# ZijiaLewisLu/CVPR2025-DeCafNet

Hardware: AMD Instinct MI355X
Metric: clips/sec (grounding fwd, T=16384 D=1024) (higher is better)
Workload: dtype f32; 1 GPU; BASELINE configs[2]: T=16384 D=1024 full multi-scale pyramid + sidekick top-k 30% + expert path, NQ=1 queries/video, 24 independent videos per step: 3 forwards in flight on 3 HIP streams x 8 videos per forward, one replica of this per GPU; T=16384, vid_len=16384, D=1024, E=256, TE=256, levels=8, win=9, heads=4, fusion_layers=2, sn=60, msf=True, norm=True, Lq=32, nq=1, max_batch=8, forwards_in_flight=3

## Files before the change

### cvpr2025-decafnet_amd/_lib.py

```python
import ctypes
import os

_HERE = os.path.dirname(os.path.abspath(__file__))
SO_PATH = os.environ.get('DCF_LIB_PATH') or os.path.join(_HERE, 'libdecafnet_hip.so')
_LIB = None

c_f32p = ctypes.c_void_p
c_u8p = ctypes.c_void_p
c_i32p = ctypes.c_void_p
c_i64p = ctypes.c_void_p
i32, i64, f32, f64 = ctypes.c_int32, ctypes.c_int64, ctypes.c_float, ctypes.c_double
vp = ctypes.c_void_p


class DcfConfig(ctypes.Structure):
    _fields_ = [(n, i32) for n in ('D', 'E', 'TE', 'vid_heads', 'fusion_heads', 'fusion_layers', 'n_embd_convs',
                                   'n_stem', 'n_levels', 'win', 'head_layers', 'sn')] + \
               [('sratio', f32)] + [(n, i32) for n in ('msf', 'norm', 'use_abs_pe', 'max_batch', 'gemm_mode', 'model_kind', 'second_fusion',
                                                      'text_in', 'text_layers', 'text_heads', 'text_abs_pe', 'text_bkgd',
                                                      'scat', 'sfonly', 'text_kind', 'xattn_affine', 'vid_stride', 'pool_only', 'attn_mode')]


SIGNATURES = {
    'dcf_last_error': (ctypes.c_char_p, []),
    'dcf_abi_version': (i32, []),
    'dcf_model_create': (i32, [ctypes.POINTER(DcfConfig), ctypes.POINTER(vp)]),
    'dcf_model_destroy': (None, [vp]),
    'dcf_model_bind': (i32, [vp, ctypes.c_char_p, c_f32p, ctypes.POINTER(i64), i32]),
    'dcf_model_set_pe': (i32, [vp, c_f32p, i64]),
    'dcf_model_set_text_pe': (i32, [vp, c_f32p, i64]),
    'dcf_text_encode': (i32, [vp, c_f32p, c_u8p, i32, c_f32p, c_u8p, vp]),
    'dcf_model_finalize': (i32, [vp, vp]),
    'dcf_numerics_status': (i32, [vp, i32, vp]),
    'dcf_numerics_status_async': (i32, [vp, vp, vp]),
    'dcf_points_per_query': (i64, [vp, i64]),
    'dcf_forward_eval': (i32, [vp, c_f32p, c_f32p, c_u8p, i64, i32, ctypes.POINTER(vp), ctypes.POINTER(vp),
                               ctypes.POINTER(i32), c_f32p, c_f32p, c_f32p, c_u8p, vp]),
    'dcf_forward_eval_videos': (i32, [vp, i32, ctypes.POINTER(vp), ctypes.POINTER(vp), ctypes.POINTER(vp), i64, ctypes.POINTER(i32),
                                      ctypes.POINTER(vp), ctypes.POINTER(vp), ctypes.POINTER(i32), ctypes.POINTER(vp),
                                      c_f32p, c_f32p, c_u8p, vp]),
    'dcf_forward_train_videos': (i32, [vp, i32, ctypes.POINTER(vp), ctypes.POINTER(vp), ctypes.POINTER(vp), i64, ctypes.POINTER(i32),
                                       ctypes.POINTER(vp), ctypes.POINTER(vp), ctypes.POINTER(i32), ctypes.POINTER(vp),
                                       c_f32p, c_f32p, c_f32p, c_u8p, vp]),
    'dcf_model_set_dropout': (i32, [vp, f32, f32, f32, f32, f32, i64]),
    'dcf_debug_dropout_keep': (i32, [i64, i32, i64, i64, f32, c_u8p, vp]),
    'dcf_sigmoid_focal_loss': (i32, [c_f32p, c_f32p, c_u8p, i64, f32, f32, i32, c_f32p, c_f32p, c_i32p, vp]),
    'dcf_ctr_iou_loss': (i32, [c_f32p, c_f32p, c_u8p, i64, i32, f32, c_f32p, c_f32p, c_i32p, vp]),
    'dcf_annotate_points': (i32, [c_f32p, i32, i64, i32, f64, f64, i32, i64, i32, f64, c_u8p, c_f32p, c_u8p, c_u8p, vp]),
    'dcf_point_objective': (i32, [c_f32p, c_f32p, c_f32p, c_u8p, c_f32p, i32, i64, i32, f64, f64, i32, i64, i32, f64, f32, f64, i32, f32,
                                  c_f32p, f32, f32, c_f32p, c_f32p, vp]),
    'dcf_sigmoid_focal_loss_grad': (i32, [c_f32p, c_f32p, c_u8p, i64, f32, f32, i32, c_f32p, c_f32p, c_i32p, c_f32p, vp]),
    'dcf_ctr_iou_loss_grad': (i32, [c_f32p, c_f32p, c_u8p, i64, i32, f32, c_f32p, c_f32p, c_i32p, c_f32p, vp]),
    'dcf_point_objective_grad': (i32, [c_f32p, c_f32p, c_f32p, c_u8p, c_f32p, i32, i64, i32, f64, f64, i32, i64, i32, f64, f32, f64, i32, f32,
                                       c_f32p, f32, f32, c_f32p, c_f32p, c_f32p, c_f32p, c_f32p, i32, c_f32p, c_f32p, vp]),
    'dcf_forward_eval_gated': (i32, [vp, c_f32p, c_f32p, c_u8p, i64, i32, ctypes.POINTER(vp), ctypes.POINTER(vp),
                                     ctypes.POINTER(i32), c_f32p, c_f32p, c_f32p, c_u8p, vp]),
    'dcf_hybrid_phase1': (i32, [vp, i32, c_f32p, c_f32p, c_u8p, i64, i64, i32, ctypes.POINTER(vp), ctypes.POINTER(vp), ctypes.POINTER(i32),
                                c_f32p, c_f32p, vp]),
    'dcf_hybrid_phase2': (i32, [vp, c_f32p, c_u8p, i64, c_f32p, vp]),
    'dcf_hybrid_phase3': (i32, [vp, c_f32p, c_f32p, c_f32p, c_u8p, c_f32p, c_f32p, c_u8p, vp]),
    'dcf_debug_copy': (i32, [vp, i32, c_f32p, i64, vp]),
    'dcf_graph_active': (i32, [vp]),
    'dcf_debug_set_option': (i32, [ctypes.c_char_p, i32]),
    'dcf_calib_mfma_rate': (i32, [i32, i32, ctypes.POINTER(i32), ctypes.POINTER(f32)]),
    'dcf_model_set_graph_mode': (i32, [vp, i32]),
    'dcf_model_set_ln_carry': (i32, [vp, i32]),
    'dcf_profile_enable': (i32, [i32]),
    'dcf_profile_report': (i64, [ctypes.c_char_p, i64]),
    'dcf_collect_segments': (i32, [c_f32p, c_f32p, c_u8p, i32, i64, i32, f32, i32, f32, c_f32p, c_f32p, c_i32p, vp]),
    'dcf_collect_segments_ext': (i32, [c_f32p, c_f32p, c_u8p, c_f32p, i32, i64, i32, f32, i32, f32, c_f32p, c_f32p, c_i32p, vp]),
    'dcf_nms_1d': (i32, [c_f32p, c_f32p, c_i32p, i32, i32, i32, f32, c_i64p, c_i32p, vp]),
    'dcf_softnms_1d': (i32, [c_f32p, c_f32p, c_i32p, i32, i32, i32, f32, f32, f32, i32, i32, c_f32p, c_i64p, c_i32p, vp]),
    'dcf_segment_voting': (i32, [c_f32p, i32, c_i32p, i32, i32, c_f32p, c_f32p, c_i32p, i32, i32, f32, i32, c_f32p, vp]),
    'dcf_op_linear': (i32, [c_f32p, c_f32p, c_f32p, c_f32p, i32, i32, i32, i32, vp]),
    'dcf_op_linear_split': (i32, [c_f32p, c_f32p, c_f32p, c_f32p, i32, i32, i32, i32, i32, vp]),
    'dcf_op_linear_cm': (i32, [c_f32p, c_f32p, c_f32p, c_f32p, i32, i32, i32, vp]),
    'dcf_op_linear_ln': (i32, [c_f32p, c_f32p, c_f32p, c_f32p, c_f32p, c_f32p, c_f32p, i32, i32, i32, i32, i32, vp]),
    'dcf_op_linear_ln_carry': (i32, [c_f32p, c_f32p, c_f32p, c_f32p, c_f32p, c_f32p, c_f32p, c_f32p, c_f32p, c_f32p, i32, i32, i32, i32, i32, i32, vp]),
    'dcf_op_ffn': (i32, [c_f32p, c_f32p, c_f32p, c_f32p, c_f32p, c_f32p, c_f32p, c_f32p, c_u8p, c_f32p, c_f32p, i32, i32, i32, vp]),
    'dcf_op_linear_cm_split': (i32, [c_f32p, c_f32p, c_f32p, c_f32p, i32, i32, i32, i32, vp]),
    'dcf_op_head': (i32, [c_f32p, c_u8p, c_f32p, c_f32p, c_f32p, c_f32p, c_f32p, c_f32p, c_f32p, c_f32p, c_f32p, i32, i32, i32, i32, f32, i32, vp]),
    'dcf_op_conv3': (i32, [c_f32p, c_u8p, c_f32p, c_f32p, i32, i32, i32, i32, vp]),
    'dcf_op_conv3_split': (i32, [c_f32p, c_u8p, c_f32p, c_f32p, i32, i32, i32, i32, i32, vp]),
    'dcf_op_layernorm': (i32, [c_f32p, c_f32p, c_f32p, c_f32p, i32, i32, i32, vp]),
    'dcf_op_xattn': (i32, [c_f32p, c_f32p, c_f32p, c_u8p, c_f32p, i32, i32, i32, i32, i32, vp]),
    'dcf_op_local_attn': (i32, [c_f32p, c_f32p, c_f32p, c_u8p, c_f32p, i32, i32, i32, i32, i32, vp]),
    'dcf_op_sidekick': (i32, [c_f32p, c_f32p, c_f32p, i32, i32, i32, i32, vp]),
    'dcf_op_gate': (i32, [c_f32p, c_u8p, c_f32p, c_u8p, i32, i32, i32, f64, i32, vp]),
    'dcf_op_encoder': (i32, [vp, ctypes.c_char_p, c_f32p, c_u8p, i32, i32, i32, c_f32p, c_u8p, vp]),
    'dcf_op_enc_pre': (i32, [vp, ctypes.c_char_p, c_f32p, c_u8p, i32, i32, i32, c_f32p, c_f32p, c_f32p, c_f32p, vp]),
    'dcf_op_decoder': (i32, [vp, ctypes.c_char_p, c_f32p, c_u8p, i32, i32, ctypes.POINTER(vp), ctypes.POINTER(vp), ctypes.POINTER(i32), vp]),
    'dcf_op_tcn': (i32, [vp, ctypes.c_char_p, c_f32p, c_u8p, i32, i32, i32, i32, c_f32p, vp]),
}


def lib():
    global _LIB
    if _LIB is None:
        import torch
        if not os.path.exists(SO_PATH):
            raise RuntimeError(f'{SO_PATH} is missing: build it with __graft_entry__.build() '
                               f'(there is no CPU fallback for the grounding path)')
        h = ctypes.CDLL(SO_PATH, mode=ctypes.RTLD_GLOBAL)
        for name, (res, args) in SIGNATURES.items():
            fn = getattr(h, name)
            fn.restype = res
            fn.argtypes = args
        _LIB = h
    return _LIB


def check(rc, what=''):
    if rc != 0:
        msg = lib().dcf_last_error().decode(errors='replace')
        raise RuntimeError(f'decafnet_hip {what} failed: {msg}')


def ptr(t):
    return None if t is None else ctypes.c_void_p(t.data_ptr())


def current_stream():
    import torch
    return ctypes.c_void_p(torch.cuda.current_stream().cuda_stream)
```

### cvpr2025-decafnet_amd/csrc/dec_chain.h

```cpp
#pragma once
#include <hip/hip_runtime.h>
#include <stdint.h>

namespace dcf {

struct DecChainArgs {
  const float* X;
  int64_t ldx;
  const uint8_t* mask;
  const float* ln_q_w; const float* ln_q_b;
  const float* dw;
  const float* qn_w; const float* qn_b;
  const unsigned short* Wq;
  const float* bq;
  const unsigned short* KV;
  const float* kmask;
  const unsigned short* Wp;
  const float* bp;
  float* Q3;
  int64_t ldq;
  float* stats_out;
  int stats_w;
  int B, T;
  int affine;
  int lk2;
  unsigned* status;
  int attn_single;
};

bool dec_chain_supports(int E, int heads, int Lk);
int launch_dec_chain(const DecChainArgs& a, hipStream_t stream);

size_t chain1_image_halfs(int N, int K);
int launch_split_chain1(const float* W, unsigned short* img, int N, int K, hipStream_t stream, unsigned* overflow = nullptr);

size_t kv_image_halfs(int lk2);
int launch_kv_image(const float* K, const float* V, const uint8_t* kvmask, int B, int Lk, int lk2, unsigned short* img, float* kmask,
                    hipStream_t stream);

}
```

### cvpr2025-decafnet_amd/csrc/dec_chain.hip

```cpp
#include "dec_chain.h"

#include <type_traits>

#include "chain_common.h"
#include "common.h"

namespace dcf {

namespace {

using namespace chain;

constexpr int DE = 256, DHEADS = 4, DHD = 64;
constexpr int STAGE = 65536;
constexpr int WGROWS = 128;
constexpr int P_LNW = 0, P_LNB = 256, P_QNW = 512, P_QNB = 768, P_DW = 1024, P_BQ = 1792, P_BP = 2048, P_MS = 2560, P_END = 2624;
constexpr int X_LAST = P_END;
constexpr int X_FIRST = X_LAST + 5 * 256;
constexpr int LDS_FLOATS = X_FIRST + 5 * 256;
constexpr int LDS_BYTES = 2 * STAGE + LDS_FLOATS * (int)sizeof(float);
#ifdef DCF_DC_STAMP
__device__ unsigned long long dcf_dc_stamps[16];
#endif
}

__global__ void k_split_chain1(const float* __restrict__ W, unsigned short* __restrict__ img, int N, int K, unsigned* __restrict__ overflow) {
  const int i = blockIdx.x * blockDim.x + threadIdx.x;
  if (i >= N * (K / 2)) return;
  const int n = i / (K / 2), k = (i - n * (K / 2)) * 2;
  const float w0 = W[(size_t)n * K + k], w1 = W[(size_t)n * K + k + 1];
  unsigned hi, lo;
  split2_f16(w0, w1, SW, hi, lo);
  if (!(__builtin_fabsf(w0) * SW <= 65504.f) || !(__builtin_fabsf(w1) * SW <= 65504.f)) {
    if (overflow) atomicOr(overflow, 1u);
  }
  const int n32 = n >> 5, rr = n & 31, kk = k >> 4, kr = k & 15;
  const int a = kr >> 3, h = (kr >> 2) & 1, ii = kr & 3, j = 4 * a + ii;
  const size_t o = ((size_t)(n32 * (K / 16) + kk) * 2) * 512 + (size_t)(h * 32 + rr) * 8 + j;
  *reinterpret_cast<unsigned*>(img + o) = hi;
  *reinterpret_cast<unsigned*>(img + o + 512) = lo;
}

__global__ void k_kv_image(const float* __restrict__ K, const float* __restrict__ V, const uint8_t* __restrict__ kvmask, int B, int Lk,
                           int lk2, unsigned short* __restrict__ img, float* __restrict__ kmask) {
  const int per_head = 16 * lk2 * 256;
  const int i = blockIdx.x * blockDim.x + threadIdx.x;
  if (i < B * 64) {
    const int b = i / 64, key = i % 64;
    kmask[i] = (key < Lk && kvmask[(size_t)b * Lk + key]) ? 0.f : -INFINITY;
  }
  if (i >= B * DHEADS * per_head) return;
  const int b = i / (DHEADS * per_head), rem = i - b * (DHEADS * per_head);
  const int hd = rem / per_head, rem2 = rem - hd * per_head;
  const int piece = rem2 >> 8, lane = (rem2 >> 2) & 63, jp = rem2 & 3;
  const int h = lane >> 5, r = lane & 31, plane = piece & 1, j = 2 * jp;
  const float scale = 1.0f / sqrtf(sqrtf((float)DHD));
  float v0 = 0.f, v1 = 0.f;
  if (piece < 8 * lk2) {
    const int ks = (piece >> 1) & 3, kt = piece >> 3;
    const int key = 32 * kt + r, ch = DHD * hd + 16 * ks + 8 * (j >> 2) + 4 * h + (j & 3);
    if (key < Lk) { v0 = K[((size_t)b * Lk + key) * DE + ch] * scale; v1 = K[((size_t)b * Lk + key) * DE + ch + 1] * scale; }
  } else {
    const int pv = piece - 8 * lk2;
    const int q = (pv >> 1) & 1, kt = (pv >> 2) % lk2, ct = (pv >> 2) / lk2;
    const int ch = DHD * hd + 32 * ct + r, key = 32 * kt + 16 * q + 8 * (j >> 2) + 4 * h + (j & 3);
    if (key < Lk) v0 = V[((size_t)b * Lk + key) * DE + ch];
    if (key + 1 < Lk) v1 = V[((size_t)b * Lk + key + 1) * DE + ch];
  }
  const f16x2 hh = __builtin_convertvector(f32x2{v0, v1}, f16x2);
  const f16x2 ll = __builtin_convertvector(f32x2{v0 - (float)hh[0], v1 - (float)hh[1]}, f16x2);
  const size_t o = (((size_t)b * DHEADS + hd) * 16 * lk2 + piece) * 512 + (size_t)lane * 8 + j;
  *reinterpret_cast<unsigned*>(img + o) = __builtin_bit_cast(unsigned, plane == 0 ? hh : ll);
}

template <int LK2, bool SINGLE = false>
__global__ __launch_bounds__(256, 1) void k_dec_chain(DecChainArgs p) {
  extern __shared__ __attribute__((aligned(16))) unsigned char lds[];
  float* ldf = reinterpret_cast<float*>(lds + 2 * STAGE);
  const int tid = threadIdx.x, lane = tid & 63, r = lane & 31, h = lane >> 5;
  const int w = __builtin_amdgcn_readfirstlane(tid >> 6);
  const unsigned lane16 = (unsigned)lane * 16u;
  const int wins = (p.T + WGROWS - 1) / WGROWS;
  const int b = (int)blockIdx.x / wins, t0 = ((int)blockIdx.x - b * wins) * WGROWS;
  const int t = t0 + w * 32 + r;
  const bool inseq = t < p.T;
  const int64_t row = (int64_t)b * p.T + (inseq ? t : p.T - 1);
  constexpr int KVP = 16 * LK2;

  const unsigned short* kv_b = p.KV + (size_t)b * DHEADS * KVP * 512;
  auto issue_piece = [&](int s, int i) __attribute__((always_inline)) {
    const bool kv = s < 8 && (s & 1);
    const int np = kv ? KVP : 64;
    int pc = w + 4 * i;
    pc = pc < np ? pc : np - 1;
    const unsigned short* src = s >= 8 ? p.Wp + (size_t)(s - 8) * 64 * 512 : (kv ? kv_b + (size_t)(s >> 1) * KVP * 512 : p.Wq + (size_t)(s >> 1) * 64 * 512);
    glds16(src + (size_t)pc * 512, lane16, (unsigned)(s & 1) * STAGE + (unsigned)pc * 1024u);
  };
#ifdef DCF_DC_STAMP
  unsigned long long acc_[16] = {0, 0, 0, 0, 0, 0, 0, 0, 0, 0, 0, 0, 0, 0, 0, 0}, last_ = dc_stamp();
#endif

  const float* px = p.X + row * p.ldx + 4 * h;
  const bool valid = inseq && p.mask[row] != 0;
  f32x4 xv[32];
#pragma unroll
  for (int i = 0; i < 32; ++i) xv[i] = *reinterpret_cast<const f32x4*>(px + 32 * (i >> 2) + 8 * (i & 3));
  const int te = w == 0 ? t0 - 1 : t0 + WGROWS;
  const bool edge_wave = w == 0 || w == 3;
  const bool evalid = edge_wave && te >= 0 && te < p.T && p.mask[(int64_t)b * p.T + (te >= 0 && te < p.T ? te : 0)] != 0;
  f32x4 ev = f32x4{0.f, 0.f, 0.f, 0.f};
  if (evalid) ev = *reinterpret_cast<const f32x4*>(p.X + ((int64_t)b * p.T + te) * p.ldx + 4 * lane);
#pragma unroll
  for (int i = 0; i < 16; ++i) issue_piece(0, i);

  {
    ldf[P_LNW + tid] = p.ln_q_w[tid]; ldf[P_LNB + tid] = p.ln_q_b[tid];
    ldf[P_QNW + tid] = p.qn_w[tid]; ldf[P_QNB + tid] = p.qn_b[tid];
    ldf[P_DW + tid] = p.dw[tid]; ldf[P_DW + 256 + tid] = p.dw[256 + tid]; ldf[P_DW + 512 + tid] = p.dw[512 + tid];
    ldf[P_BQ + tid] = p.bq[tid];
    ldf[P_BP + tid] = p.bp[tid]; ldf[P_BP + 256 + tid] = p.bp[256 + tid];
    if (tid < 64) ldf[P_MS + tid] = p.kmask[(size_t)b * 64 + tid];
  }


  if (!valid) {
#pragma unroll
    for (int i = 0; i < 32; ++i) xv[i] = f32x4{0.f, 0.f, 0.f, 0.f};
  }
  float mean1, rstd1;
  row_stats<DE>(xv, mean1, rstd1);
  STAMP(0);
  __syncthreads();
#pragma unroll
  for (int i = 0; i < 32; ++i) {
    const int c = 32 * (i >> 2) + 8 * (i & 3) + 4 * h;
    const f32x4 g = *reinterpret_cast<const f32x4*>(ldf + P_LNW + c), bb = *reinterpret_cast<const f32x4*>(ldf + P_LNB + c);
    f32x4 y = (xv[i] - mean1) * rstd1 * g + bb;
    if (!valid) y = f32x4{0.f, 0.f, 0.f, 0.f};
    xv[i] = y;
  }
  if (r == 31) {
#pragma unroll
    for (int i = 0; i < 32; ++i) *reinterpret_cast<f32x4*>(ldf + X_LAST + (w + 1) * 256 + 32 * (i >> 2) + 8 * (i & 3) + 4 * h) = xv[i];
  }
  if (r == 0) {
#pragma unroll
    for (int i = 0; i < 32; ++i) *reinterpret_cast<f32x4*>(ldf + X_FIRST + w * 256 + 32 * (i >> 2) + 8 * (i & 3) + 4 * h) = xv[i];
  }
  if (edge_wave) {
    f32x4 y = f32x4{0.f, 0.f, 0.f, 0.f};
    const float s = wave_sum((ev.x + ev.y) + (ev.z + ev.w));
    const float mean = s * (1.0f / DE);
    const f32x4 d = ev - mean;
    const float var = wave_sum((d.x * d.x + d.y * d.y) + (d.z * d.z + d.w * d.w)) * (1.0f / DE);
    const float rs = 1.0f / sqrtf(var + 1e-5f);
    if (evalid) y = d * rs * *reinterpret_cast<const f32x4*>(ldf + P_LNW + 4 * lane) + *reinterpret_cast<const f32x4*>(ldf + P_LNB + 4 * lane);
    *reinterpret_cast<f32x4*>(ldf + (w == 0 ? X_LAST : X_FIRST + 4 * 256) + 4 * lane) = y;
  }
  STAMP(1);
  __syncthreads();
  STAMP(2);
  {
    const bool is32 = lane == 32, is31 = lane == 31;
#pragma unroll
    for (int i = 0; i < 32; ++i) {
      const int c = 32 * (i >> 2) + 8 * (i & 3) + 4 * h;
      const f32x4 lastv = *reinterpret_cast<const f32x4*>(ldf + X_LAST + w * 256 + c);
      const f32x4 firstv = *reinterpret_cast<const f32x4*>(ldf + X_FIRST + (w + 1) * 256 + c);
      const f32x4 w0 = *reinterpret_cast<const f32x4*>(ldf + P_DW + c), w1 = *reinterpret_cast<const f32x4*>(ldf + P_DW + 256 + c),
                  w2 = *reinterpret_cast<const f32x4*>(ldf + P_DW + 512 + c);
      f32x4 pv, nv;
#pragma unroll
      for (int e = 0; e < 4; ++e) {
        const float sp = shr1(xv[i][e], lastv[e]), sn = shl1(xv[i][e], firstv[e]);
        pv[e] = is32 ? lastv[e] : sp;
        nv[e] = is31 ? firstv[e] : sn;
      }
      xv[i] = w0 * pv + w1 * xv[i] + w2 * nv;
    }
  }
  f16x8 qh[16], ql[16];
  {
    float mean2, rstd2;
    row_stats<DE>(xv, mean2, rstd2);
#pragma unroll
    for (int kk = 0; kk < 16; ++kk) {
      float v8[8];
#pragma unroll
      for (int u = 0; u < 2; ++u) {
        const int i = 2 * kk + u, c = 32 * (i >> 2) + 8 * (i & 3) + 4 * h;
        const f32x4 g = *reinterpret_cast<const f32x4*>(ldf + P_QNW + c), bb = *reinterpret_cast<const f32x4*>(ldf + P_QNB + c);
        const f32x4 y = (xv[i] - mean2) * rstd2 * g + bb;
        v8[4 * u] = y.x; v8[4 * u + 1] = y.y; v8[4 * u + 2] = y.z; v8[4 * u + 3] = y.w;
      }
      split8(v8, SA, qh[kk], ql[kk]);
    }
  }

  STAMP(3);
  f16x8 cth[16], ctl[16];
  const float qscale = 1.0f / sqrtf(sqrtf((float)DHD));
  auto stage_begin = [&](int s) __attribute__((always_inline)) {
    asm volatile("s_waitcnt vmcnt(0)" ::: "memory");
    STAMP(4);
    __syncthreads();
    STAMP(5);
  };
  auto gemm2 = [&](const unsigned char* buf, const f16x8 (&bh)[16], const f16x8 (&bl)[16], f32x16 (&acc)[2], auto&& dma, auto&& side)
                   __attribute__((always_inline)) {
    f16x8 fr[2][4];
    auto frags = [&](int kk, int set) __attribute__((always_inline)) {
      fr[set][0] = *reinterpret_cast<const f16x8*>(buf + ((0 * 16 + kk) * 2) * 1024);
      fr[set][1] = *reinterpret_cast<const f16x8*>(buf + ((0 * 16 + kk) * 2 + 1) * 1024);
      fr[set][2] = *reinterpret_cast<const f16x8*>(buf + ((1 * 16 + kk) * 2) * 1024);
      fr[set][3] = *reinterpret_cast<const f16x8*>(buf + ((1 * 16 + kk) * 2 + 1) * 1024);
    };
    frags(0, 0);
#pragma unroll
    for (int kk = 0; kk < 16; ++kk) {
      const int set = kk & 1;
      if (kk + 1 < 16) frags(kk + 1, set ^ 1);
      acc[0] = mma(fr[set][1], bh[kk], acc[0]);
      acc[1] = mma(fr[set][3], bh[kk], acc[1]);
      __builtin_amdgcn_sched_barrier(0);
      side(kk, 0);
      __builtin_amdgcn_sched_barrier(0);
      acc[0] = mma(fr[set][0], bl[kk], acc[0]);
      acc[1] = mma(fr[set][2], bl[kk], acc[1]);
      __builtin_amdgcn_sched_barrier(0);
      side(kk, 1);
      dma(kk);
      __builtin_amdgcn_sched_barrier(0);
      acc[0] = mma(fr[set][0], bh[kk], acc[0]);
      acc[1] = mma(fr[set][2], bh[kk], acc[1]);
      __builtin_amdgcn_sched_barrier(0);
    }
  };
  f32x16 O[2];
  u32x4 cx_h, cx_l;
  auto ctx_piece = [&](int hd, int u) __attribute__((always_inline)) {
    const int ct = u >> 3, q = (u >> 2) & 1, i = u & 3;
    unsigned hi, lo;
    split2_f16(O[ct][8 * q + 2 * i], O[ct][8 * q + 2 * i + 1], SA, hi, lo);
    cx_h[i] = hi; cx_l[i] = lo;
    if (i == 3) {
      cth[2 * (2 * hd + ct) + q] = __builtin_bit_cast(f16x8, cx_h);
      ctl[2 * (2 * hd + ct) + q] = __builtin_bit_cast(f16x8, cx_l);
    }
  };
#pragma unroll
  for (int hd = 0; hd < DHEADS; ++hd) {
    f32x16 QA[2];
    {
      stage_begin(2 * hd);
      const unsigned char* buf = lds + ((2 * hd) & 1) * STAGE + lane16;
#pragma unroll
      for (int t2 = 0; t2 < 2; ++t2)
#pragma unroll
        for (int e = 0; e < 16; ++e) QA[t2][e] = 0.f;
      gemm2(buf, qh, ql, QA,
            [&](int kk) __attribute__((always_inline)) {
              if (kk < KVP / 4) issue_piece(2 * hd + 1, kk);
            },
            [&](int kk, int slot) __attribute__((always_inline)) { if (hd > 0 && slot == 0) ctx_piece(hd - 1, kk); });
    }
    STAMP(6);
    f16x8 sh_[4], sl_[4];
#pragma unroll
    for (int t2 = 0; t2 < 2; ++t2)
#pragma unroll
      for (int q = 0; q < 2; ++q) {
        float v8[8];
#pragma unroll
        for (int u = 0; u < 2; ++u) {
          const int g = 2 * q + u;
          const f32x4 bq = *reinterpret_cast<const f32x4*>(ldf + P_BQ + DHD * hd + 32 * t2 + 8 * g + 4 * h);
#pragma unroll
          for (int e = 0; e < 4; ++e) v8[4 * u + e] = __builtin_fmaf(QA[t2][4 * g + e], UNSCALE, bq[e]) * qscale;
        }
        split8(v8, 1.f, sh_[2 * t2 + q], sl_[2 * t2 + q]);
      }
    STAMP(7);
    {
      stage_begin(2 * hd + 1);
      const unsigned char* buf = lds + ((2 * hd + 1) & 1) * STAGE + lane16;
      f32x16 S[LK2];
#pragma unroll
      for (int kt = 0; kt < LK2; ++kt)
#pragma unroll
        for (int e = 0; e < 16; ++e) S[kt][e] = 0.f;
      f16x8 kf[2][LK2][2];
      auto kfrags = [&](int ks, int set) __attribute__((always_inline)) {
#pragma unroll
        for (int kt = 0; kt < LK2; ++kt) {
          kf[set][kt][0] = *reinterpret_cast<const f16x8*>(buf + ((kt * 4 + ks) * 2) * 1024);
          kf[set][kt][1] = *reinterpret_cast<const f16x8*>(buf + ((kt * 4 + ks) * 2 + 1) * 1024);
        }
      };
      kfrags(0, 0);
#pragma unroll
      for (int ks = 0; ks < 4; ++ks) {
        const int set = ks & 1;
        if (ks + 1 < 4) kfrags(ks + 1, set ^ 1);
        issue_piece(2 * hd + 2, 2 * ks);
        issue_piece(2 * hd + 2, 2 * ks + 1);
        if constexpr (!SINGLE) {
#pragma unroll
          for (int kt = 0; kt < LK2; ++kt) S[kt] = mma(kf[set][kt][0], sl_[ks], S[kt]);
#pragma unroll
          for (int kt = 0; kt < LK2; ++kt) S[kt] = mma(kf[set][kt][1], sh_[ks], S[kt]);
        }
#pragma unroll
        for (int kt = 0; kt < LK2; ++kt) S[kt] = mma(kf[set][kt][0], sh_[ks], S[kt]);
        __builtin_amdgcn_sched_barrier(0);
      }
      STAMP(8);
      f16x8 vf[2][2][2];
      auto vfrags = [&](int st_, int set) __attribute__((always_inline)) {
#pragma unroll
        for (int ct = 0; ct < 2; ++ct) {
          const int pc = 8 * LK2 + ((ct * LK2 + (st_ >> 1)) * 2 + (st_ & 1)) * 2;
          vf[set][ct][0] = *reinterpret_cast<const f16x8*>(buf + pc * 1024);
          vf[set][ct][1] = *reinterpret_cast<const f16x8*>(buf + (pc + 1) * 1024);
        }
      };
      vfrags(0, 0);
      float mx = -INFINITY;
#pragma unroll
      for (int kt = 0; kt < LK2; ++kt)
#pragma unroll
        for (int g = 0; g < 4; ++g) {
          const f32x4 mk = *reinterpret_cast<const f32x4*>(ldf + P_MS + 32 * kt + 8 * g + 4 * h);
#pragma unroll
          for (int e = 0; e < 4; ++e) { S[kt][4 * g + e] += mk[e]; mx = fmaxf(mx, S[kt][4 * g + e]); }
        }
      mx = xor32_max(mx);
      float sum = 0.f;
#pragma unroll
      for (int kt = 0; kt < LK2; ++kt)
#pragma unroll
        for (int e = 0; e < 16; ++e) { S[kt][e] = fast_exp(S[kt][e] - mx); sum += S[kt][e]; }
      const float inv = 1.0f / xor32_sum(sum);
      f16x8 ph[LK2][2], pl[LK2][2];
#pragma unroll
      for (int kt = 0; kt < LK2; ++kt)
#pragma unroll
        for (int q = 0; q < 2; ++q) {
          float v8[8];
#pragma unroll
          for (int e = 0; e < 8; ++e) v8[e] = S[kt][8 * q + e] * inv;
          split8(v8, 1.f, ph[kt][q], pl[kt][q]);
        }
      STAMP(9);
#pragma unroll
      for (int ct = 0; ct < 2; ++ct)
#pragma unroll
        for (int e = 0; e < 16; ++e) O[ct][e] = 0.f;
#pragma unroll
      for (int st_ = 0; st_ < 2 * LK2; ++st_) {
        const int set = st_ & 1, kt = st_ >> 1, q = st_ & 1;
        if (st_ + 1 < 2 * LK2) vfrags(st_ + 1, set ^ 1);
#pragma unroll
        for (int i = 0; i < 8 / (2 * LK2); ++i) issue_piece(2 * hd + 2, 8 + st_ * (8 / (2 * LK2)) + i);
        if constexpr (!SINGLE) {
#pragma unroll
          for (int ct = 0; ct < 2; ++ct) O[ct] = mma(vf[set][ct][0], pl[kt][q], O[ct]);
#pragma unroll
          for (int ct = 0; ct < 2; ++ct) O[ct] = mma(vf[set][ct][1], ph[kt][q], O[ct]);
        }
#pragma unroll
        for (int ct = 0; ct < 2; ++ct) O[ct] = mma(vf[set][ct][0], ph[kt][q], O[ct]);
        __builtin_amdgcn_sched_barrier(0);
      }
      STAMP(10);
    }
  }

  float ps = 0.f, pss = 0.f;
  float* qout = p.Q3 + row * p.ldq + 4 * h;
  f32x16 A2[2][2];
  f32x4 xr[2][4];
  auto load_xr = [&](int j) __attribute__((always_inline)) {
#pragma unroll
    for (int g = 0; g < 4; ++g) xr[j & 1][g] = *reinterpret_cast<const f32x4*>(px + 32 * j + 8 * g);
  };
  f32x4 ep_sc, ep_sf;
  auto epilogue = [&](int j, int g, int half) __attribute__((always_inline)) {
    if (half == 0) {
      const f32x4 bs = *reinterpret_cast<const f32x4*>(ldf + P_BP + 64 * j + 8 * g + 4 * h);
      const f32x4 bh = *reinterpret_cast<const f32x4*>(ldf + P_BP + 64 * j + 32 + 8 * g + 4 * h);
#pragma unroll
      for (int e = 0; e < 4; ++e) {
        ep_sc[e] = __builtin_fmaf(A2[j & 1][0][4 * g + e], UNSCALE, bs[e]);
        ep_sf[e] = __builtin_fmaf(A2[j & 1][1][4 * g + e], UNSCALE, bh[e]);
      }
    } else {
      f32x4 xa = valid ? xr[j & 1][g] : f32x4{0.f, 0.f, 0.f, 0.f};
      if (!p.affine) xa = (xa - mean1) * rstd1;
      const f32x4 o = xa * ep_sc + ep_sf;
      if (inseq) *reinterpret_cast<f32x4*>(qout + 32 * j + 8 * g) = o;
      ps += (o.x + o.y) + (o.z + o.w);
      pss += __builtin_fmaf(o.x, o.x, o.y * o.y) + __builtin_fmaf(o.z, o.z, o.w * o.w);
    }
  };
#pragma unroll
  for (int j = 0; j < 8; ++j) {
    stage_begin(8 + j);
    const unsigned char* buf = lds + (j & 1) * STAGE + lane16;
    if (j > 0) asm volatile("" : "+v"(xr[(j - 1) & 1][0]), "+v"(xr[(j - 1) & 1][1]), "+v"(xr[(j - 1) & 1][2]), "+v"(xr[(j - 1) & 1][3]));
    load_xr(j);
#pragma unroll
    for (int t2 = 0; t2 < 2; ++t2)
#pragma unroll
      for (int e = 0; e < 16; ++e) A2[j & 1][t2][e] = 0.f;
    if (j == 0) {
      gemm2(buf, cth, ctl, A2[0],
            [&](int kk) __attribute__((always_inline)) {
              issue_piece(9, kk);
            },
            [&](int kk, int slot) __attribute__((always_inline)) { if (kk < 8) ctx_piece(DHEADS - 1, 2 * kk + slot); });
    } else {
      gemm2(buf, cth, ctl, A2[j & 1],
            [&](int kk) __attribute__((always_inline)) {
              if (j + 1 < 8) issue_piece(8 + j + 1, kk);
            },
            [&](int kk, int slot) __attribute__((always_inline)) { if ((kk & 3) == 0) epilogue(j - 1, kk >> 2, slot); });
    }
    STAMP(11);
  }
  asm volatile("s_waitcnt vmcnt(0)" ::: "memory");
  asm volatile("" : "+v"(xr[1][0]), "+v"(xr[1][1]), "+v"(xr[1][2]), "+v"(xr[1][3]));
#pragma unroll
  for (int g = 0; g < 4; ++g) { epilogue(7, g, 0); epilogue(7, g, 1); }
  STAMP(12);
  const float s1 = xor32_sum(ps), s2 = xor32_sum(pss);
  if (p.stats_out && inseq && h == 0) {
    const int slots = DE / p.stats_w;
    float* o = p.stats_out + row * slots * 2;
    o[0] = s1; o[1] = s2;
    for (int k = 1; k < slots; ++k) { o[2 * k] = 0.f; o[2 * k + 1] = 0.f; }
  }
  const bool bad = !(__builtin_fabsf(s1) <= 3.4028234664e38f) && inseq;
  if (bad && p.status) {
    bool anykey = false;
#pragma unroll
    for (int k = 0; k < 64; ++k) anykey = anykey || ldf[P_MS + k] == 0.f;
    if (anykey) atomicOr(p.status, 1u);
  }
#ifdef DCF_DC_STAMP
  STAMP(13);
  if (blockIdx.x == 1 && tid == 0)
    for (int i = 0; i < 16; ++i) dcf_dc_stamps[i] = acc_[i];
#endif
}

#ifdef DCF_DC_STAMP
}
extern "C" int dcf_debug_dc_stamps(unsigned long long* out) {
  return hipMemcpyFromSymbol(out, HIP_SYMBOL(dcf::dcf_dc_stamps), 16 * sizeof(unsigned long long)) == hipSuccess ? 0 : -1;
}
namespace dcf {
#endif

bool dec_chain_supports(int E, int heads, int Lk) { return E == DE && heads == DHEADS && Lk >= 1 && Lk <= 64; }

size_t chain1_image_halfs(int N, int K) { return (size_t)N * K * 2; }

int launch_split_chain1(const float* W, unsigned short* img, int N, int K, hipStream_t stream, unsigned* overflow) {
  DCF_CHECK(N % 32 == 0 && K % 16 == 0, "launch_split_chain1: N = %d, K = %d", N, K);
  const int n = N * (K / 2);
  hipLaunchKernelGGL(k_split_chain1, dim3((n + 255) / 256), dim3(256), 0, stream, W, img, N, K, overflow);
  DCF_HIP(hipGetLastError());
  return 0;
}

size_t kv_image_halfs(int lk2) { return (size_t)DHEADS * 16 * lk2 * 512; }

int launch_kv_image(const float* K, const float* V, const uint8_t* kvmask, int B, int Lk, int lk2, unsigned short* img, float* kmask,
                    hipStream_t stream) {
  DCF_CHECK(B > 0 && Lk >= 1 && Lk <= 32 * lk2 && (lk2 == 1 || lk2 == 2), "launch_kv_image: Lk = %d, lk2 = %d", Lk, lk2);
  const int n = B * DHEADS * 16 * lk2 * 256;
  hipLaunchKernelGGL(k_kv_image, dim3((n + 255) / 256), dim3(256), 0, stream, K, V, kvmask, B, Lk, lk2, img, kmask);
  DCF_HIP(hipGetLastError());
  return 0;
}

int launch_dec_chain(const DecChainArgs& a, hipStream_t stream) {
  DCF_CHECK(a.B > 0 && a.T > 0 && a.X && a.mask && a.Wq && a.KV && a.kmask && a.Wp && a.Q3, "launch_dec_chain: null argument");
  DCF_CHECK(a.lk2 == 1 || a.lk2 == 2, "launch_dec_chain: lk2 = %d", a.lk2);
  DCF_CHECK(!a.stats_out || (a.stats_w > 0 && DE % a.stats_w == 0), "launch_dec_chain: stats_out needs a slot width dividing %d", DE);
  auto al16 = [](const void* q) { return (reinterpret_cast<uintptr_t>(q) & 15) == 0; };
  DCF_CHECK(al16(a.X) && al16(a.Q3) && al16(a.Wq) && al16(a.Wp) && al16(a.KV) && a.ldx % 4 == 0 && a.ldq % 4 == 0,
            "launch_dec_chain: operands must be 16-byte aligned with row pitches that are multiples of 4");
  static bool attr_set[64] = {};
  int dev = 0;
  DCF_HIP(hipGetDevice(&dev));
  if (dev >= 0 && dev < 64 && !attr_set[dev]) {
    DCF_HIP(hipFuncSetAttribute(reinterpret_cast<const void*>(&k_dec_chain<1>), hipFuncAttributeMaxDynamicSharedMemorySize, LDS_BYTES));
    DCF_HIP(hipFuncSetAttribute(reinterpret_cast<const void*>(&k_dec_chain<2>), hipFuncAttributeMaxDynamicSharedMemorySize, LDS_BYTES));
    DCF_HIP(hipFuncSetAttribute(reinterpret_cast<const void*>(&k_dec_chain<1, true>), hipFuncAttributeMaxDynamicSharedMemorySize, LDS_BYTES));
    DCF_HIP(hipFuncSetAttribute(reinterpret_cast<const void*>(&k_dec_chain<2, true>), hipFuncAttributeMaxDynamicSharedMemorySize, LDS_BYTES));
    attr_set[dev] = true;
  }
  const unsigned grid = (unsigned)(a.B * ((a.T + WGROWS - 1) / WGROWS));
  if (a.attn_single) {
    if (a.lk2 == 1) hipLaunchKernelGGL((k_dec_chain<1, true>), dim3(grid), dim3(256), LDS_BYTES, stream, a);
    else hipLaunchKernelGGL((k_dec_chain<2, true>), dim3(grid), dim3(256), LDS_BYTES, stream, a);
  } else if (a.lk2 == 1) hipLaunchKernelGGL(k_dec_chain<1>, dim3(grid), dim3(256), LDS_BYTES, stream, a);
  else hipLaunchKernelGGL(k_dec_chain<2>, dim3(grid), dim3(256), LDS_BYTES, stream, a);
  DCF_HIP(hipGetLastError());
  return 0;
}

}
```

### cvpr2025-decafnet_amd/csrc/engine.hip

```cpp
#include <cstdarg>
#include <cstdio>
#include <cstdlib>
#include <algorithm>
#include <cstring>
#include <string>
#include <atomic>
#include <mutex>
#include <unordered_map>
#include <vector>

#include "../../include/decafnet_hip.h"
#include "attn.h"
#include "common.h"
#include "dec_chain.h"
#include "dropout.h"
#include "enc_chain.h"
#include "ffn_chain.h"
#include "gemm.h"
#include "head_chain.h"
#include "heads.h"
#include "postproc.h"
#include "rowops.h"
#include "score.h"

namespace dcf {

static thread_local std::string g_err;
void set_error(const char* fmt, ...) {
  char buf[1024];
  va_list ap;
  va_start(ap, fmt);
  vsnprintf(buf, sizeof(buf), fmt, ap);
  va_end(ap);
  g_err = buf;
}

static std::unordered_map<std::string, int>& debug_options() {
  static std::unordered_map<std::string, int> o;
  return o;
}
static std::mutex& debug_options_mutex() {
  static std::mutex mu;
  return mu;
}
static std::atomic<int> g_option_epoch{0};
static int debug_option(const char* name, int dflt) {
  std::lock_guard<std::mutex> lock(debug_options_mutex());
  auto& o = debug_options();
  auto it = o.find(name);
  return it == o.end() ? dflt : it->second;
}

struct ProfRec { std::string name; hipEvent_t a, b; double flops, bytes; };
static bool g_prof_on = false;
static std::vector<ProfRec> g_recs;

ProfScope::ProfScope(const char* name, hipStream_t s, double flops, double bytes) : idx(-1), st(s) {
  if (!g_prof_on) return;
  ProfRec r{name, nullptr, nullptr, flops, bytes};
  if (hipEventCreate(&r.a) != hipSuccess || hipEventCreate(&r.b) != hipSuccess) return;
  (void)hipEventRecord(r.a, st);
  g_recs.push_back(r);
  idx = (int)g_recs.size() - 1;
}
ProfScope::~ProfScope() {
  if (idx >= 0) (void)hipEventRecord(g_recs[idx].b, st);
}

__global__ void k_permute3(const float* __restrict__ src, float* __restrict__ dst, int d0, int d1, int d2, int p0, int p1,
                           int p2) {
  const int n = d0 * d1 * d2;
  const int i = blockIdx.x * blockDim.x + threadIdx.x;
  if (i >= n) return;
  int idx[3];
  idx[0] = i / (d1 * d2);
  idx[1] = (i / d2) % d1;
  idx[2] = i % d2;
  const int dims[3] = {d0, d1, d2};
  const int perm[3] = {p0, p1, p2};
  const int o = (idx[perm[0]] * dims[perm[1]] + idx[perm[1]]) * dims[perm[2]] + idx[perm[2]];
  dst[o] = src[i];
}

__global__ void k_masks_out(const uint8_t* __restrict__ mask_all, uint8_t* __restrict__ out, const LevelTable* lt,
                            const unsigned* __restrict__ status, float* __restrict__ logits) {
  const int r = blockIdx.x * blockDim.x + threadIdx.x;
  const int total = lt->start[lt->n_levels];
  if (r >= total) return;
  int l = 0;
  while (l + 1 < lt->n_levels && r >= lt->start[l + 1]) ++l;
  const int rel = r - lt->start[l];
  const int b = rel / lt->T[l], t = rel - b * lt->T[l];
  const int64_t o = (int64_t)b * lt->S + lt->off[l] + t;
  out[o] = mask_all[r];
  if (status && (status[0] & 3u)) logits[o] = __uint_as_float(0x7fc00000u);
}

__global__ void k_points_out(const float* __restrict__ rows, float* __restrict__ out, const LevelTable* lt) {
  const int r = blockIdx.x * blockDim.x + threadIdx.x;
  const int total = lt->start[lt->n_levels];
  if (r >= total) return;
  int l = 0;
  while (l + 1 < lt->n_levels && r >= lt->start[l + 1]) ++l;
  const int rel = r - lt->start[l];
  const int b = rel / lt->T[l], t = rel - b * lt->T[l];
  out[(int64_t)b * lt->S + lt->off[l] + t] = rows[r];
}

__global__ void k_apply_gate(const float* __restrict__ gate_in, const uint8_t* __restrict__ vid_mask, float* __restrict__ gate,
                             uint8_t* __restrict__ mask_out, int T, int rows, int msf) {
  const int r = blockIdx.x * blockDim.x + threadIdx.x;
  if (r >= rows) return;
  const int t = r % T;
  const float g = gate_in[r];
  const bool m = vid_mask[t] != 0;
  gate[r] = g;
  mask_out[r] = msf ? m : (m && g != 0.f);
}

__global__ __launch_bounds__(64) void k_fold_ln(const float* __restrict__ W, const float* __restrict__ bias, const float* __restrict__ g,
                                                const float* __restrict__ beta, float* __restrict__ Wf, float* __restrict__ s,
                                                float* __restrict__ c, int K) {
  const int n = blockIdx.x, lane = threadIdx.x;
  float a1 = 0.f, a2 = 0.f;
  for (int k = lane; k < K; k += 64) {
    const float w = W[(int64_t)n * K + k];
    const float wf = w * g[k];
    Wf[(int64_t)n * K + k] = wf;
    a1 += wf;
    a2 += beta[k] * w;
  }
  a1 = wave_sum(a1);
  a2 = wave_sum(a2);
  if (lane == 0) { s[n] = a1; c[n] = (bias ? bias[n] : 0.f) + a2; }
}

struct Bound {
  const float* p = nullptr;
  std::vector<int64_t> shape;
  int64_t numel() const {
    int64_t n = 1;
    for (auto s : shape) n *= s;
    return n;
  }
};

struct EncW {
  const float *ln_attn_w, *ln_attn_b, *dw_q, *dw_k, *dw_v, *qn_w, *qn_b, *kn_w, *kn_b, *vn_w, *vn_b;
  const float *wq, *bq, *wk, *bk, *wv, *bv, *wp, *bp, *ls_attn;
  const float *ln_ffn_w, *ln_ffn_b, *fc_w, *fc_b, *pj_w, *pj_b, *ls_ffn;
  const float *fc_wf, *fc_s, *fc_c;
  const unsigned short* qkv_chain[3];
  const float *qkv_s[3], *qkv_c[3];
  const unsigned short* wp_chain;
};
struct DecW {
  const float *ln_q_w, *ln_q_b, *ln_kv_w, *ln_kv_b, *dw, *qn_w, *qn_b;
  const float *wq, *bq, *wk, *bk, *wv, *bv, *wp, *bp;
  const float *wp_il, *bp_il;
  const float *ln_ffn_w, *ln_ffn_b, *fc_w, *fc_b, *pj_w, *pj_b, *ls_ffn;
  const float *fc_wf, *fc_s, *fc_c;
  const unsigned short *wq_chain, *wp_chain;
};
struct TextEncW {
  const float *ln_attn_w, *ln_attn_b, *wq, *bq, *wk, *bk, *wv, *bv, *wp, *bp, *ls_attn;
  const float *ln_ffn_w, *ln_ffn_b, *fc_w, *fc_b, *pj_w, *pj_b, *ls_ffn;
};
struct HeadW {
  std::vector<const float*> conv;
  std::vector<const float*> ln_w, ln_b;
  const float* out_w;
  const float* out_b;
  const unsigned short* chain[2] = {nullptr, nullptr};
};

static inline int vid_stride_of(const dcf_config& c) { return c.vid_stride > 1 ? c.vid_stride : 1; }

struct Plan {
  int T0 = 0, B = 0, L = 0;
  LevelTable lt{};
  LevelTable* d_lt = nullptr;
};

}

using namespace dcf;

namespace dcf { struct HybridState; }
using dcf::HybridState;

struct dcf_model {
  dcf_config cfg{};
  std::unordered_map<std::string, Bound> bound;
  std::vector<float*> owned;
  std::unordered_map<const float*, const unsigned short*> wsplit;
  std::unordered_map<const float*, int64_t> wsplit_ldw;
  std::unordered_map<const float*, int> wsplit_terms;
  int gemm_terms = 16;
  bool force_x6 = false;
  bool no_ln_carry = false;
  int option_epoch = 0;
  unsigned* status = nullptr;
  bool finalized = false;
  const float* pe = nullptr;
  int64_t pe_T = 0;

  const float *vid_map_w = nullptr, *vid_map_b = nullptr;
  const float *vid_w1 = nullptr, *vid_w2 = nullptr, *vid_w3 = nullptr;
  int64_t vid_ldw = 0;
  std::vector<DecW> dec;
  const float *fus_out_w = nullptr, *fus_out_b = nullptr;
  const float *embd_fc_w = nullptr, *embd_fc_b = nullptr;
  const float *embd_fc_wf = nullptr, *embd_fc_s = nullptr, *embd_fc_c = nullptr;
  std::vector<const float*> embd_conv, embd_ln_w, embd_ln_b;
  std::vector<EncW> stem, branch;
  std::vector<const float*> pool_w;
  HeadW cls1, cls2, reg;
  std::vector<float> reg_scales;
  const float *tcn_in_w = nullptr, *tcn_in_b = nullptr, *tcn_out_w = nullptr, *tcn_out_b = nullptr;
  std::vector<const float*> tcn_wd, tcn_bd, tcn_wp, tcn_bp, tcn_lnw, tcn_lnb;
  std::vector<const unsigned short*> tcn_frag;
  const float *text_embd_w = nullptr, *text_embd_b = nullptr, *text_bkgd = nullptr;
  TextEncW text_pool{};
  std::vector<TextEncW> text_enc;
  const float* text_pe = nullptr;
  int64_t text_pe_L = 0;
  char* text_ws = nullptr;
  size_t text_ws_bytes = 0;

  char* arena = nullptr;
  size_t arena_bytes = 0;
  std::vector<Plan> plans;
  std::vector<uint64_t> last_key, graph_key;
  hipGraph_t graph = nullptr;
  hipGraphExec_t graph_exec = nullptr;
  bool capturing = false;
  int graph_mode = 0;
  std::vector<uint64_t> nocapture_key;
  int last_launch = 0;
  hipStream_t own = nullptr;
  hipEvent_t ev_in = nullptr, ev_out = nullptr;
  struct {
    float *correl = nullptr, *gate = nullptr, *vidmap = nullptr, *fused = nullptr, *F = nullptr;
    int nq = 0, T0 = 0, B = 0, S = 0;
  } dbg;
  struct HybridState* hyb = nullptr;
  int hyb_levels = 0;
  size_t hyb_extra = 0;
  char* hyb_extra_ptr = nullptr;
  float* hyb_feat_out = nullptr;
  float* dbg_vidmap = nullptr;
  float* dbg_fused = nullptr;
  int64_t dbg_cap = 0;
  bool keep_debug = false;
  struct DropState {
    float p[5] = {0.f, 0.f, 0.f, 0.f, 0.f};
    float scale[5] = {1.f, 1.f, 1.f, 1.f, 1.f};
    uint64_t seed = 0;
    bool active = false;
    int b0 = 0;
  } drop_state;
  DropState* drop = nullptr;
};

namespace dcf {

static void free_hybrid(dcf_model* m);

static void drop_graph(dcf_model* m, bool keep_last_key = false) {
  if (m->graph_exec) (void)hipGraphExecDestroy(m->graph_exec);
  if (m->graph) (void)hipGraphDestroy(m->graph);
  m->graph_exec = nullptr;
  m->graph = nullptr;
  m->graph_key.clear();
  if (!keep_last_key) m->last_key.clear();
}

static int free_model(dcf_model* m) {
  drop_graph(m);
  if (m->status) (void)hipFree(m->status);
  m->status = nullptr;
  for (float* p : m->owned) (void)hipFree(p);
  m->owned.clear();
  m->wsplit.clear();
  m->wsplit_ldw.clear();
  m->wsplit_terms.clear();
  for (auto& pl : m->plans) if (pl.d_lt) (void)hipFree(pl.d_lt);
  m->plans.clear();
  free_hybrid(m);
  if (m->arena) (void)hipFree(m->arena);
  if (m->text_ws) (void)hipFree(m->text_ws);
  if (m->ev_in) (void)hipEventDestroy(m->ev_in);
  if (m->ev_out) (void)hipEventDestroy(m->ev_out);
  if (m->own) (void)hipStreamDestroy(m->own);
  return 0;
}

static int get(dcf_model* m, const std::string& name, std::initializer_list<int64_t> shape, const float** out) {
  auto it = m->bound.find(name);
  DCF_CHECK(it != m->bound.end(), "parameter '%s' is not bound", name.c_str());
  const Bound& b = it->second;
  int64_t want = 1;
  for (auto s : shape) want *= s;
  DCF_CHECK(b.numel() == want, "parameter '%s' has %lld elements, expected %lld", name.c_str(), (long long)b.numel(),
            (long long)want);
  *out = b.p;
  return 0;
}

static int pack3(dcf_model* m, const float* src, int d0, int d1, int d2, int p0, int p1, int p2, hipStream_t st,
                 const float** out) {
  float* dst = nullptr;
  const size_t n = (size_t)d0 * d1 * d2;
  DCF_HIP(hipMalloc(&dst, n * sizeof(float)));
  m->owned.push_back(dst);
  hipLaunchKernelGGL(k_permute3, dim3((unsigned)((n + 255) / 256)), dim3(256), 0, st, src, dst, d0, d1, d2, p0, p1, p2);
  DCF_HIP(hipGetLastError());
  *out = dst;
  return 0;
}

static int split_weight(dcf_model* m, const float* W, int N, int K, hipStream_t st, int64_t ldw = 0, int terms = 0) {
  if (m->gemm_terms == 0 || m->wsplit.count(W)) return 0;
  if (!terms) terms = m->gemm_terms;
  unsigned short* planes = nullptr;
  DCF_HIP(hipMalloc(&planes, (size_t)3 * N * K * sizeof(unsigned short)));
  m->owned.push_back(reinterpret_cast<float*>(planes));
  if (launch_split_planes(W, planes, N, K, ldw ? ldw : K, st, terms, m->status ? m->status + 1 : nullptr)) return -1;
  m->wsplit[W] = planes;
  m->wsplit_ldw[W] = ldw ? ldw : K;
  m->wsplit_terms[W] = terms;
  return 0;
}
#define SPLIT(W, N, K) do { if (split_weight(m, (W), (N), (K), st)) return -1; } while (0)

static int fold_ln(dcf_model* m, const float* W, const float* bias, const float* g, const float* beta, int N, int K, hipStream_t st,
                   const float** wf, const float** s_out, const float** c_out) {
  float* buf = nullptr;
  DCF_HIP(hipMalloc(&buf, ((size_t)N * K + 2 * (size_t)N) * sizeof(float)));
  m->owned.push_back(buf);
  float* sv = buf + (size_t)N * K;
  hipLaunchKernelGGL(k_fold_ln, dim3(N), dim3(64), 0, st, W, bias, g, beta, buf, sv, sv + N, K);
  DCF_HIP(hipGetLastError());
  *wf = buf; *s_out = sv; *c_out = sv + N;
  return split_weight(m, buf, N, K, st);
}

#define GET(name, shape, dst) do { if (get(m, (name), shape, &(dst))) return -1; } while (0)
#define SH(...) std::initializer_list<int64_t>{__VA_ARGS__}

static int resolve_encoder(dcf_model* m, const std::string& p, int E, hipStream_t st, EncW& w) {
  const float* t;
  GET(p + ".ln_attn.weight", SH(E), w.ln_attn_w); GET(p + ".ln_attn.bias", SH(E), w.ln_attn_b);
  GET(p + ".attn.q_conv.conv.weight", SH(E, 3), t); if (pack3(m, t, 1, E, 3, 0, 2, 1, st, &w.dw_q)) return -1;
  GET(p + ".attn.k_conv.conv.weight", SH(E, 3), t); if (pack3(m, t, 1, E, 3, 0, 2, 1, st, &w.dw_k)) return -1;
  GET(p + ".attn.v_conv.conv.weight", SH(E, 3), t); if (pack3(m, t, 1, E, 3, 0, 2, 1, st, &w.dw_v)) return -1;
  GET(p + ".attn.q_norm.weight", SH(E), w.qn_w); GET(p + ".attn.q_norm.bias", SH(E), w.qn_b);
  GET(p + ".attn.k_norm.weight", SH(E), w.kn_w); GET(p + ".attn.k_norm.bias", SH(E), w.kn_b);
  GET(p + ".attn.v_norm.weight", SH(E), w.vn_w); GET(p + ".attn.v_norm.bias", SH(E), w.vn_b);
  GET(p + ".attn.attn.query.weight", SH(E, E), w.wq); GET(p + ".attn.attn.query.bias", SH(E), w.bq);
  GET(p + ".attn.attn.key.weight", SH(E, E), w.wk); GET(p + ".attn.attn.key.bias", SH(E), w.bk);
  GET(p + ".attn.attn.value.weight", SH(E, E), w.wv); GET(p + ".attn.attn.value.bias", SH(E), w.bv);
  GET(p + ".attn.attn.proj.weight", SH(E, E), w.wp); GET(p + ".attn.attn.proj.bias", SH(E), w.bp);
  GET(p + ".drop_path_attn.scale", SH(E), w.ls_attn);
  GET(p + ".ln_ffn.weight", SH(E), w.ln_ffn_w); GET(p + ".ln_ffn.bias", SH(E), w.ln_ffn_b);
  GET(p + ".ffn.fc.weight", SH(4 * E, E), w.fc_w); GET(p + ".ffn.fc.bias", SH(4 * E), w.fc_b);
  GET(p + ".ffn.proj.weight", SH(E, 4 * E), w.pj_w); GET(p + ".ffn.proj.bias", SH(E), w.pj_b);
  GET(p + ".drop_path_ffn.scale", SH(E), w.ls_ffn);
  SPLIT(w.wq, E, E); SPLIT(w.wk, E, E); SPLIT(w.wv, E, E); SPLIT(w.wp, E, E);
  SPLIT(w.fc_w, 4 * E, E); SPLIT(w.pj_w, E, 4 * E);
  w.fc_wf = w.fc_s = w.fc_c = nullptr;
  if (m->gemm_terms != 0 && E % 64 == 0 && fold_ln(m, w.fc_w, w.fc_b, w.ln_ffn_w, w.ln_ffn_b, 4 * E, E, st, &w.fc_wf, &w.fc_s, &w.fc_c)) return -1;
  for (int i = 0; i < 3; ++i) { w.qkv_chain[i] = nullptr; w.qkv_s[i] = w.qkv_c[i] = nullptr; }
  w.wp_chain = nullptr;
  if (m->gemm_terms == GEMM_F16X3 && enc_chain_supports(E, m->cfg.vid_heads, m->cfg.win > 0 ? m->cfg.win : 99)) {
    {
      unsigned short* img = nullptr;
      DCF_HIP(hipMalloc(&img, chain1_image_halfs(E, E) * sizeof(unsigned short)));
      m->owned.push_back(reinterpret_cast<float*>(img));
      if (launch_split_chain1(w.wp, img, E, E, st, nullptr)) return -1;
      w.wp_chain = img;
    }
    const float* W3[3] = {w.wq, w.wk, w.wv};
    const float* B3[3] = {w.bq, w.bk, w.bv};
    const float* G3[3] = {w.qn_w, w.kn_w, w.vn_w};
    const float* H3[3] = {w.qn_b, w.kn_b, w.vn_b};
    for (int i = 0; i < 3; ++i) {
      const float* wf;
      if (fold_ln(m, W3[i], B3[i], G3[i], H3[i], E, E, st, &wf, &w.qkv_s[i], &w.qkv_c[i])) return -1;
      unsigned short* img = nullptr;
      DCF_HIP(hipMalloc(&img, chain1_image_halfs(E, E) * sizeof(unsigned short)));
      m->owned.push_back(reinterpret_cast<float*>(img));
      if (launch_split_chain1(wf, img, E, E, st, m->status ? m->status + 1 : nullptr)) return -1;
      w.qkv_chain[i] = img;
    }
  }
  return 0;
}

static int resolve_decoder(dcf_model* m, const std::string& p, int E, int TE, hipStream_t st, DecW& w) {
  const float* t;
  GET(p + ".ln_xattn_q.weight", SH(E), w.ln_q_w); GET(p + ".ln_xattn_q.bias", SH(E), w.ln_q_b);
  GET(p + ".ln_xattn_kv.weight", SH(TE), w.ln_kv_w); GET(p + ".ln_xattn_kv.bias", SH(TE), w.ln_kv_b);
  GET(p + ".xattn.q_conv.conv.weight", SH(E, 3), t); if (pack3(m, t, 1, E, 3, 0, 2, 1, st, &w.dw)) return -1;
  GET(p + ".xattn.q_norm.weight", SH(E), w.qn_w); GET(p + ".xattn.q_norm.bias", SH(E), w.qn_b);
  GET(p + ".xattn.xattn.query.weight", SH(E, E), w.wq); GET(p + ".xattn.xattn.query.bias", SH(E), w.bq);
  GET(p + ".xattn.xattn.key.weight", SH(E, TE), w.wk); GET(p + ".xattn.xattn.key.bias", SH(E), w.bk);
  GET(p + ".xattn.xattn.value.weight", SH(E, TE), w.wv); GET(p + ".xattn.xattn.value.bias", SH(E), w.bv);
  GET(p + ".xattn.xattn.proj.weight", SH(2 * E, E), w.wp); GET(p + ".xattn.xattn.proj.bias", SH(2 * E), w.bp);
  GET(p + ".ln_ffn.weight", SH(E), w.ln_ffn_w); GET(p + ".ln_ffn.bias", SH(E), w.ln_ffn_b);
  GET(p + ".ffn.fc.weight", SH(4 * E, E), w.fc_w); GET(p + ".ffn.fc.bias", SH(4 * E), w.fc_b);
  GET(p + ".ffn.proj.weight", SH(E, 4 * E), w.pj_w); GET(p + ".ffn.proj.bias", SH(E), w.pj_b);
  GET(p + ".drop_path_ffn.scale", SH(E), w.ls_ffn);
  SPLIT(w.wq, E, E); SPLIT(w.wk, E, TE); SPLIT(w.wv, E, TE); SPLIT(w.wp, 2 * E, E);
  SPLIT(w.fc_w, 4 * E, E); SPLIT(w.pj_w, E, 4 * E);
  w.fc_wf = w.fc_s = w.fc_c = nullptr;
  if (m->gemm_terms != 0 && E % 128 == 0 && fold_ln(m, w.fc_w, w.fc_b, w.ln_ffn_w, w.ln_ffn_b, 4 * E, E, st, &w.fc_wf, &w.fc_s, &w.fc_c)) return -1;
  w.wp_il = w.bp_il = nullptr;
  if (E % 32 == 0) {
    if (pack3(m, w.wp, 2, E / 32, 32 * E, 1, 0, 2, st, &w.wp_il)) return -1;
    if (pack3(m, w.bp, 2, E / 32, 32, 1, 0, 2, st, &w.bp_il)) return -1;
    SPLIT(w.wp_il, 2 * E, E);
  }
  w.wq_chain = w.wp_chain = nullptr;
  if (m->gemm_terms == GEMM_F16X3 && w.wp_il && dec_chain_supports(E, m->cfg.fusion_heads, 1)) {
    unsigned short *iq = nullptr, *ip = nullptr;
    DCF_HIP(hipMalloc(&iq, chain1_image_halfs(E, E) * sizeof(unsigned short)));
    m->owned.push_back(reinterpret_cast<float*>(iq));
    DCF_HIP(hipMalloc(&ip, chain1_image_halfs(2 * E, E) * sizeof(unsigned short)));
    m->owned.push_back(reinterpret_cast<float*>(ip));
    if (launch_split_chain1(w.wq, iq, E, E, st, nullptr)) return -1;
    if (launch_split_chain1(w.wp_il, ip, 2 * E, E, st, nullptr)) return -1;
    w.wq_chain = iq; w.wp_chain = ip;
  }
  return 0;
}

static int resolve_tcn(dcf_model* m, const std::string& pre, int n_in, int n_layers, hipStream_t st) {
  const float* t;
  m->tcn_wd.clear(); m->tcn_bd.clear(); m->tcn_wp.clear(); m->tcn_bp.clear(); m->tcn_lnw.clear(); m->tcn_lnb.clear();
  GET(pre + ".conv_1x1.weight", SH(TCN_HID, n_in), t); if (pack3(m, t, 1, TCN_HID, n_in, 0, 2, 1, st, &m->tcn_in_w)) return -1;
  GET(pre + ".conv_1x1.bias", SH(TCN_HID), m->tcn_in_b);
  for (int i = 0; i < n_layers; ++i) {
    const std::string p = pre + ".layers." + std::to_string(i);
    const float* pk;
    GET(p + ".conv_dilated.weight", SH(TCN_HID, TCN_HID, 3), t);
    if (pack3(m, t, TCN_HID, TCN_HID, 3, 2, 1, 0, st, &pk)) return -1;
    m->tcn_wd.push_back(pk);
    GET(p + ".conv_dilated.bias", SH(TCN_HID), t); m->tcn_bd.push_back(t);
    GET(p + ".conv_1x1.weight", SH(TCN_HID, TCN_HID), t);
    if (pack3(m, t, 1, TCN_HID, TCN_HID, 0, 2, 1, st, &pk)) return -1;
    m->tcn_wp.push_back(pk);
    if (m->gemm_terms == GEMM_F16X3) {
      if (launch_f16_weight_range(m->tcn_wd.back(), 3 * TCN_HID * TCN_HID, m->status ? m->status + 1 : nullptr, st)) return -1;
      if (launch_f16_weight_range(m->tcn_wp.back(), TCN_HID * TCN_HID, m->status ? m->status + 1 : nullptr, st)) return -1;
    }
    GET(p + ".conv_1x1.bias", SH(TCN_HID), t); m->tcn_bp.push_back(t);
    GET(p + ".norm.weight", SH(TCN_HID), t); m->tcn_lnw.push_back(t);
    GET(p + ".norm.bias", SH(TCN_HID), t); m->tcn_lnb.push_back(t);
  }
  GET(pre + ".conv_out.weight", SH(TCN_HID, TCN_HID), t);
  if (pack3(m, t, 1, TCN_HID, TCN_HID, 0, 2, 1, st, &m->tcn_out_w)) return -1;
  if (m->gemm_terms == GEMM_F16X3 && launch_f16_weight_range(m->tcn_out_w, TCN_HID * TCN_HID, m->status ? m->status + 1 : nullptr, st)) return -1;
  GET(pre + ".conv_out.bias", SH(TCN_HID), m->tcn_out_b);
  m->tcn_frag.clear();
  if (m->gemm_terms == GEMM_F16X3) {
    for (int i = 0; i < n_layers; ++i) {
      unsigned short* img = nullptr;
      DCF_HIP(hipMalloc(&img, (size_t)TCN_FRAG_HALFS * sizeof(unsigned short)));
      m->owned.push_back(reinterpret_cast<float*>(img));
      if (launch_tcn_frag_image(m->tcn_wd[i], m->tcn_wp[i], i + 1 == n_layers ? m->tcn_out_w : nullptr, img, st)) return -1;
      m->tcn_frag.push_back(img);
    }
  }
  return 0;
}

static int init_gemm_mode(dcf_model* m, hipStream_t st) {
  const int gm = m->cfg.gemm_mode;
  DCF_CHECK(gm == 0 || gm == 1 || gm == 6 || gm == 16, "gemm_mode %d: use 0 / 16 (f16x3), 6 (bf16x6) or 1 (fp32); the bf16x3 mode was replaced by f16x3", gm);
  m->gemm_terms = gm == 1 ? 0 : (gm == 6 ? GEMM_BF16X6 : GEMM_F16X3);
  if (m->force_x6 && m->gemm_terms == GEMM_F16X3) m->gemm_terms = GEMM_BF16X6;
  if (!m->status) DCF_HIP(hipMalloc(&m->status, 2 * sizeof(unsigned)));
  DCF_HIP(hipMemsetAsync(m->status, 0, 2 * sizeof(unsigned), st));
  return 0;
}

static int resolve_head(dcf_model* m, const std::string& p, const std::string& out_name, int C, int NO, int layers,
                        hipStream_t st, HeadW& h) {
  const float* t;
  for (int i = 0; i < layers; ++i) {
    const std::string s = std::to_string(i);
    GET(p + ".convs." + s + ".conv.weight", SH(C, C, 3), t);
    const float* pk;
    if (pack3(m, t, C, C, 3, 0, 2, 1, st, &pk)) return -1;
    SPLIT(pk, C, 3 * C);
    h.conv.push_back(pk);
    const float *lw, *lb;
    GET(p + ".norms." + s + ".weight", SH(C), lw); GET(p + ".norms." + s + ".bias", SH(C), lb);
    h.ln_w.push_back(lw); h.ln_b.push_back(lb);
  }
  GET(p + "." + out_name + ".conv.weight", SH(NO, C, 3), t);
  if (pack3(m, t, NO, C, 3, 0, 2, 1, st, &h.out_w)) return -1;
  GET(p + "." + out_name + ".conv.bias", SH(NO), h.out_b);
  h.chain[0] = h.chain[1] = nullptr;
  if (m->gemm_terms == GEMM_F16X3 && layers == 2 && head_chain_supports(C, NO)) {
    for (int i = 0; i < 2; ++i) {
      unsigned short* img = nullptr;
      DCF_HIP(hipMalloc(&img, head_chain_image_halfs(C) * sizeof(unsigned short)));
      m->owned.push_back(reinterpret_cast<float*>(img));
      if (launch_split_chain3(h.conv[i], img, C, st, nullptr)) return -1;
      h.chain[i] = img;
    }
  }
  return 0;
}

static inline bool vidmap_sfonly(const dcf_config& c) { return c.model_kind == 0 && c.msf && c.sfonly; }
static inline int vidmap_in_dim(const dcf_config& c) {
  return ((c.msf && !vidmap_sfonly(c)) ? 2 * c.D : c.D) + (c.scat ? 1 : 0);
}

static int finalize(dcf_model* m, hipStream_t st) {
  const dcf_config& c = m->cfg;
  const int E = c.E, D = c.D, TE = c.TE, L = c.n_levels;
  const bool sfonly = vidmap_sfonly(c);
  const int Din = vidmap_in_dim(c);
  for (float* p : m->owned) (void)hipFree(p);
  m->owned.clear();
  m->wsplit.clear();
  m->wsplit_ldw.clear();
  m->wsplit_terms.clear();
  if (init_gemm_mode(m, st)) return -1;
  m->dec.clear(); m->stem.clear(); m->branch.clear();
  m->embd_conv.clear(); m->embd_ln_w.clear(); m->embd_ln_b.clear();
  m->cls1 = HeadW(); m->cls2 = HeadW(); m->reg = HeadW();
  m->tcn_wd.clear(); m->tcn_bd.clear(); m->tcn_wp.clear(); m->tcn_bp.clear(); m->tcn_lnw.clear(); m->tcn_lnb.clear();
  const float* t;

  m->text_enc.clear();
  m->text_embd_w = m->text_embd_b = m->text_bkgd = nullptr;
  m->text_pool = TextEncW();
  if (c.text_kind == 1) {
    DCF_CHECK(c.text_in > 0 && c.text_heads >= 1 && TE % c.text_heads == 0, "text_net (identity): in_dim=%d heads=%d do not fit TE=%d", c.text_in, c.text_heads, TE);
    if (m->bound.count("text_net.embd_fc.conv.weight")) {
      GET("text_net.embd_fc.conv.weight", SH(TE, c.text_in), m->text_embd_w); GET("text_net.embd_fc.conv.bias", SH(TE), m->text_embd_b);
    } else {
      DCF_CHECK(c.text_in == TE, "text_net (identity) without embd_fc needs in_dim == embd_dim (%d vs %d)", c.text_in, TE);
    }
    if (c.text_bkgd) {
      TextEncW& w = m->text_pool;
      const std::string p = "text_net.attn_pool.attn";
      GET(p + ".query.weight", SH(TE, TE), w.wq); GET(p + ".query.bias", SH(TE), w.bq);
      GET(p + ".key.weight", SH(TE, TE), w.wk); GET(p + ".key.bias", SH(TE), w.bk);
      GET(p + ".value.weight", SH(TE, TE), w.wv); GET(p + ".value.bias", SH(TE), w.bv);
      GET(p + ".proj.weight", SH(TE, TE), w.wp); GET(p + ".proj.bias", SH(TE), w.bp);
      SPLIT(w.wq, TE, TE); SPLIT(w.wk, TE, TE); SPLIT(w.wv, TE, TE); SPLIT(w.wp, TE, TE);
    }
  } else
  if (c.text_layers > 0 || c.text_in > 0) {
    DCF_CHECK(c.text_in > 0 && c.text_layers >= 0 && c.text_heads >= 1 && TE % c.text_heads == 0,
              "text_net: in_dim=%d layers=%d heads=%d do not fit TE=%d", c.text_in, c.text_layers, c.text_heads, TE);
    GET("text_net.embd_fc.conv.weight", SH(TE, c.text_in), m->text_embd_w); GET("text_net.embd_fc.conv.bias", SH(TE), m->text_embd_b);
    if (c.text_bkgd) GET("text_net.bkgd_token", SH(TE), m->text_bkgd);
    for (int i = 0; i < c.text_layers; ++i) {
      const std::string p = "text_net.transformer." + std::to_string(i);
      TextEncW w{};
      GET(p + ".ln_attn.weight", SH(TE), w.ln_attn_w); GET(p + ".ln_attn.bias", SH(TE), w.ln_attn_b);
      GET(p + ".attn.attn.query.weight", SH(TE, TE), w.wq); GET(p + ".attn.attn.query.bias", SH(TE), w.bq);
      GET(p + ".attn.attn.key.weight", SH(TE, TE), w.wk); GET(p + ".attn.attn.key.bias", SH(TE), w.bk);
      GET(p + ".attn.attn.value.weight", SH(TE, TE), w.wv); GET(p + ".attn.attn.value.bias", SH(TE), w.bv);
      GET(p + ".attn.attn.proj.weight", SH(TE, TE), w.wp); GET(p + ".attn.attn.proj.bias", SH(TE), w.bp);
      GET(p + ".drop_path_attn.scale", SH(TE), w.ls_attn);
      GET(p + ".ln_ffn.weight", SH(TE), w.ln_ffn_w); GET(p + ".ln_ffn.bias", SH(TE), w.ln_ffn_b);
      GET(p + ".ffn.fc.weight", SH(4 * TE, TE), w.fc_w); GET(p + ".ffn.fc.bias", SH(4 * TE), w.fc_b);
      GET(p + ".ffn.proj.weight", SH(TE, 4 * TE), w.pj_w); GET(p + ".ffn.proj.bias", SH(TE), w.pj_b);
      GET(p + ".drop_path_ffn.scale", SH(TE), w.ls_ffn);
      SPLIT(w.wq, TE, TE); SPLIT(w.wk, TE, TE); SPLIT(w.wv, TE, TE); SPLIT(w.wp, TE, TE);
      SPLIT(w.fc_w, 4 * TE, TE); SPLIT(w.pj_w, TE, 4 * TE);
      m->text_enc.push_back(w);
    }
  }

  if (c.model_kind == 1) {
    GET("vid_net.embd_fc.conv.weight", SH(E, Din), m->vid_map_w); GET("vid_net.embd_fc.conv.bias", SH(E), m->vid_map_b);
  } else {
    GET("vid_map.conv.weight", SH(E, Din), m->vid_map_w); GET("vid_map.conv.bias", SH(E), m->vid_map_b);
  }
  m->vid_w1 = (c.msf && sfonly) ? nullptr : m->vid_map_w;
  m->vid_w2 = c.msf ? (sfonly ? m->vid_map_w : m->vid_map_w + D) : nullptr;
  m->vid_w3 = nullptr;
  m->vid_ldw = Din;
  if (c.scat) {
    float* blk[3] = {nullptr, nullptr, nullptr};
    const float* src[3] = {m->vid_w1, m->vid_w2, m->vid_map_w + (Din - 1)};
    const int wid[3] = {D, D, 1};
    for (int i = 0; i < 3; ++i) {
      if (!src[i]) continue;
      DCF_HIP(hipMalloc(&blk[i], (size_t)E * wid[i] * sizeof(float)));
      m->owned.push_back(blk[i]);
      DCF_HIP(hipMemcpy2DAsync(blk[i], (size_t)wid[i] * 4, src[i], (size_t)Din * 4, (size_t)wid[i] * 4, E, hipMemcpyDeviceToDevice, st));
    }
    m->vid_w1 = blk[0]; m->vid_w2 = blk[1]; m->vid_w3 = blk[2];
    m->vid_ldw = D;
  }
  if (D % 32 == 0 && E % 32 == 0) {
    if (m->vid_w1 && split_weight(m, m->vid_w1, E, D, st, m->vid_ldw)) return -1;
    if (m->vid_w2 && split_weight(m, m->vid_w2, E, D, st, m->vid_ldw)) return -1;
  }
  for (int i = 0; i < c.fusion_layers; ++i) {
    DecW w{};
    if (resolve_decoder(m, "fusion.layers." + std::to_string(i), E, TE, st, w)) return -1;
    m->dec.push_back(w);
  }
  GET("fusion.ln_out.weight", SH(E), m->fus_out_w); GET("fusion.ln_out.bias", SH(E), m->fus_out_b);
  if (c.model_kind != 1) {
    GET("vid_net.embd_fc.conv.weight", SH(E, E), m->embd_fc_w); GET("vid_net.embd_fc.conv.bias", SH(E), m->embd_fc_b);
    SPLIT(m->embd_fc_w, E, E);
    m->embd_fc_wf = m->embd_fc_s = m->embd_fc_c = nullptr;
    if (m->gemm_terms != 0 && E % 64 == 0 && c.fusion_layers > 0 &&
        fold_ln(m, m->embd_fc_w, m->embd_fc_b, m->fus_out_w, m->fus_out_b, E, E, st, &m->embd_fc_wf, &m->embd_fc_s, &m->embd_fc_c)) return -1;
  }
  for (int i = 0, sv = vid_stride_of(c); i < c.n_embd_convs; ++i, sv = std::max(sv / 2, 1)) {
    const std::string s = std::to_string(i);
    const int taps = sv > 1 ? 5 : 3;
    GET("vid_net.embd_convs." + s + ".conv.weight", SH(E, E, taps), t);
    const float* pk;
    if (pack3(m, t, E, E, taps, 0, 2, 1, st, &pk)) return -1;
    SPLIT(pk, E, taps * E);
    m->embd_conv.push_back(pk);
    const float *lw, *lb;
    GET("vid_net.embd_norms." + s + ".weight", SH(E), lw); GET("vid_net.embd_norms." + s + ".bias", SH(E), lb);
    m->embd_ln_w.push_back(lw); m->embd_ln_b.push_back(lb);
  }
  for (int i = 0; i < c.n_stem; ++i) {
    EncW w{};
    if (resolve_encoder(m, "vid_net.stem." + std::to_string(i), E, st, w)) return -1;
    m->stem.push_back(w);
  }
  m->pool_w.clear();
  for (int i = 0; i < L; ++i) {
    if (c.pool_only) {
      const float* pk;
      GET("vid_net.branch." + std::to_string(i) + ".conv.weight", SH(E, 3), t);
      if (pack3(m, t, 1, E, 3, 0, 2, 1, st, &pk)) return -1;
      m->pool_w.push_back(pk);
      continue;
    }
    EncW w{};
    if (resolve_encoder(m, "vid_net.branch." + std::to_string(i), E, st, w)) return -1;
    m->branch.push_back(w);
  }
  if (resolve_head(m, "cls_head", "cls_head", E, 1, c.head_layers, st, m->cls1)) return -1;
  const int EH = c.model_kind == 0 ? E + TCN_HID : E;
  if (c.model_kind == 0 && resolve_head(m, "cls_head2", "cls_head", EH, 1, c.head_layers, st, m->cls2)) return -1;
  if (resolve_head(m, "reg_head", "reg_head", EH, 2, c.head_layers, st, m->reg)) return -1;
  m->reg_scales.assign(L, 1.f);
  for (int l = 0; l < L; ++l) {
    GET("reg_head.scales." + std::to_string(l) + ".scale", SH(1), t);
    DCF_HIP(hipMemcpyAsync(&m->reg_scales[l], t, sizeof(float), hipMemcpyDeviceToHost, st));
  }
  if (c.model_kind == 0 && resolve_tcn(m, "refine", L, L, st)) return -1;
  DCF_HIP(hipStreamSynchronize(st));
  for (auto& pl : m->plans) if (pl.d_lt) (void)hipFree(pl.d_lt);
  m->plans.clear();
  free_hybrid(m);
  drop_graph(m);
  if (m->gemm_terms == GEMM_F16X3) {
    unsigned flags[2] = {0u, 0u};
    DCF_HIP(hipMemcpyAsync(flags, m->status, sizeof(flags), hipMemcpyDeviceToHost, st));
    DCF_HIP(hipStreamSynchronize(st));
    if (flags[1]) {
      m->force_x6 = true;
      return finalize(m, st);
    }
  }
  m->finalized = true;
  return 0;
}

struct Arena {
  char* base;
  size_t off = 0, cap;
  bool dry;
  template <typename T>
  T* take(size_t n) {
    off = (off + 255) & ~(size_t)255;
    T* p = dry ? nullptr : reinterpret_cast<T*>(base + off);
    off += n * sizeof(T);
    return p;
  }
};

struct Buffers {
  float *P1, *P2, *tn, *partial, *correl, *gate;
  uint8_t *mask_all, *nbr_all, *kvmask, *maskv;
  uint8_t* tile_flags;
  uint8_t *mask_pre, *nbr_pre;
  float* col5;
  float *X, *R[7], *H2, *HID, *F, *HA, *HB, *HC, *HD, *logits1, *tcnA, *tcnB, *kvn, *Kt, *Vt;
  unsigned short* kvimg;
  float* kmadd;
  float* stats;
  float* hstats[2];
};

static void carve(Arena& a, const dcf_config& c, int T0, int B, int nq, int S, int Lk, int nvid, Buffers& b) {
  const size_t rows0 = (size_t)B * T0, rowsAll = (size_t)B * S;
  const size_t rowsF = std::max(rows0, (c.model_kind == 1 || c.second_fusion) ? rowsAll : (size_t)0);
  const bool strided = vid_stride_of(c) > 1;
  const int E = c.E, EH = c.E + TCN_HID;
  b.P1 = a.take<float>((size_t)nvid * T0 * E);
  b.P2 = a.take<float>((size_t)nvid * T0 * E);
  b.maskv = a.take<uint8_t>(nvid > 1 ? (size_t)nvid * T0 : 0);
  b.tn = a.take<float>((size_t)nq * c.D);
  b.partial = a.take<float>((size_t)SCORE_SLICES * (nq + nvid) * T0);
  b.correl = a.take<float>((size_t)nq * T0);
  b.gate = a.take<float>(rows0);
  b.tile_flags = a.take<uint8_t>((size_t)B * ((T0 + 63) / 64));
  b.mask_all = a.take<uint8_t>(rowsAll);
  b.nbr_all = a.take<uint8_t>(rowsAll);
  b.mask_pre = a.take<uint8_t>(strided ? 2 * rows0 : 0);
  b.nbr_pre = a.take<uint8_t>(strided ? 2 * rows0 : 0);
  b.col5 = a.take<float>(strided ? rows0 / 2 * 5 * E : 0);
  b.kvmask = a.take<uint8_t>((size_t)B * Lk);
  b.X = a.take<float>(rows0 * E);
  for (int i = 0; i < 7; ++i) b.R[i] = a.take<float>((i < 3 ? rowsF : rows0) * E);
  b.stats = a.take<float>(rowsF * (size_t)((E + 63) / 64) * 2);
  for (int i = 0; i < 2; ++i) b.hstats[i] = a.take<float>(rowsAll * (size_t)((EH + 63) / 64) * 2);
  b.H2 = a.take<float>(rowsF * 2 * E);
  b.HID = a.take<float>(rowsF * 4 * E);
  b.F = a.take<float>(rowsAll * EH);
  b.HA = a.take<float>(rowsAll * EH);
  b.HB = a.take<float>(rowsAll * EH);
  b.HC = a.take<float>(rowsAll * EH);
  b.HD = a.take<float>(rowsAll * EH);
  b.logits1 = a.take<float>(rowsAll);
  b.tcnA = a.take<float>(rows0 * TCN_HID);
  b.tcnB = a.take<float>(rows0 * TCN_HID);
  b.kvn = a.take<float>((size_t)B * Lk * c.TE);
  b.Kt = a.take<float>((size_t)B * Lk * E);
  b.Vt = a.take<float>((size_t)B * Lk * E);
  b.kvimg = a.take<unsigned short>((size_t)B * kv_image_halfs(2));
  b.kmadd = a.take<float>((size_t)B * 64);
}

static int get_plan(dcf_model* m, int T0, int B, int L, hipStream_t st, Plan** out) {
  for (auto& p : m->plans)
    if (p.T0 == T0 && p.B == B && p.L == L) { *out = &p; return 0; }
  Plan p;
  p.T0 = T0; p.B = B; p.L = L;
  LevelTable& lt = p.lt;
  lt.n_levels = L; lt.B = B;
  int acc = 0;
  for (int l = 0; l < lt.n_levels; ++l) {
    lt.T[l] = T0 >> l;
    lt.off[l] = acc;
    lt.start[l] = B * acc;
    lt.scale[l] = m->reg_scales[l];
    acc += lt.T[l];
  }
  lt.S = acc;
  lt.start[lt.n_levels] = B * acc;
  DCF_HIP(hipMalloc(&p.d_lt, sizeof(LevelTable)));
  DCF_HIP(hipMemcpyAsync(p.d_lt, &p.lt, sizeof(LevelTable), hipMemcpyHostToDevice, st));
  DCF_HIP(hipStreamSynchronize(st));
  m->plans.push_back(p);
  *out = &m->plans.back();
  return 0;
}

static GemmArgs gemm(const float* A, int64_t lda, const float* W, const float* bias, float* C, int64_t ldc, int M, int N,
                     int K) {
  GemmArgs g{};
  g.A = A; g.lda = lda; g.W = W; g.ldw = 0; g.bias = bias; g.C = C; g.ldc = ldc; g.M = M; g.N = N; g.K = K;
  return g;
}

#define TRY(x) do { if ((x) != 0) return -1; } while (0)

static int run_gemm(dcf_model* m, GemmArgs* g, int count, GemmAMode mode, hipStream_t st) {
  bool split = m->gemm_terms != 0;
  int terms = 0;
  for (int i = 0; i < count && split; ++i) {
    auto it = m->wsplit.find(g[i].W);
    if (it == m->wsplit.end() || (g[i].ldw ? g[i].ldw : g[i].K) != m->wsplit_ldw[g[i].W]) { split = false; break; }
    const int t = m->wsplit_terms[g[i].W];
    if (terms && t != terms) { split = false; break; }
    terms = t;
    g[i].Ws = it->second;
    g[i].status = m->status;
  }
  if (split && mode == A_CHANMAJOR && (g[0].N % 128 != 0 || g[0].M % 4 != 0)) split = false;
  for (int i = 0; i < count; ++i) DCF_CHECK(split || !(g[i].flags & G_ADALN), "internal: G_ADALN needs the split-operand GEMM");
  for (int i = 0; i < count; ++i) DCF_CHECK(split || !g[i].score_out, "internal: scores on the side need the split-operand GEMM");
  return split ? launch_gemm_split(g, count, mode, terms, st) : launch_gemm(g, count, mode, st);
}

constexpr int STATS_W = 64;
constexpr int FFN_CHAIN_MIN_ROWS = 16384;
static bool g_no_ffn_chain();
static bool can_chain_ffn_rows(dcf_model* m, int rows, int E) {
  return !g_no_ffn_chain() && E == 256 && rows >= FFN_CHAIN_MIN_ROWS && m->gemm_terms == GEMM_F16X3;
}
static bool g_no_ffn_chain() {
  static const bool off = getenv("DCF_NO_FFN_CHAIN") != nullptr;
  return off;
}
static bool can_chain_ffn(dcf_model* m, const float* fc_w, const GemmArgs& go, int rows, int E) {
  if (g_no_ffn_chain() || E != 256 || rows < FFN_CHAIN_MIN_ROWS || m->gemm_terms != GEMM_F16X3) return false;
  if (!m->wsplit.count(fc_w) || !m->wsplit.count(go.W) || m->wsplit_terms[fc_w] != GEMM_F16X3 || m->wsplit_terms[go.W] != GEMM_F16X3) return false;
  if (m->wsplit_ldw[fc_w] != E || m->wsplit_ldw[go.W] != 4 * E) return false;
  if (go.ln_w || !(go.flags & G_RES) || (go.flags & ~(G_RES | G_OUT_MASK)) || !go.R || !go.bias || go.a_scale > 0.f) return false;
  return true;
}
static int run_ffn_chain(dcf_model* m, const float* X, const float* fc_w, const float* fc_b, const GemmArgs& go, int rows, int E,
                         hipStream_t st, const float* stats, const float* ln_s) {
  FfnChainArgs a{};
  a.X = X; a.ldx = E; a.W1s = m->wsplit[fc_w]; a.b1 = fc_b; a.ln_s = ln_s; a.stats = stats; a.stats_slots = E / 64;
  a.W2s = m->wsplit[go.W]; a.b2 = go.bias; a.ls = go.ls; a.R = go.R; a.ldr = go.ldr;
  a.rowmask = (go.flags & G_OUT_MASK) ? go.rowmask : nullptr; a.C = go.C; a.ldc = go.ldc;
  a.stats_out = go.stats_out; a.stats_w = go.stats_w; a.status = m->status; a.M = rows;
  ProfScope prof("gemm_f16x3<ffn_chain>", st, 2.0 * rows * E * 4.0 * E * 2.0, (double)rows * E * 4.0 * 3.0);
  return launch_ffn_chain(a, st);
}

static int run_ffn(dcf_model* m, const float* X, const float* fc_w, const float* fc_b, GemmArgs go, float* HID, int rows, int E,
                   hipStream_t st, const float* stats = nullptr, const float* ln_s = nullptr) {
  if (can_chain_ffn(m, fc_w, go, rows, E)) return run_ffn_chain(m, X, fc_w, fc_b, go, rows, E, st, stats, ln_s);
  GemmArgs gf = gemm(X, E, fc_w, fc_b, HID, 4 * E, rows, 4 * E, E);
  gf.flags = G_GELU;
  if (stats) { gf.stats_in = stats; gf.ln_s = ln_s; gf.stats_slots = E / STATS_W; gf.stats_w = STATS_W; }
  TRY(run_gemm(m, &gf, 1, A_ROWS, st));
  return run_gemm(m, &go, 1, A_ROWS, st);
}

static bool g_no_carry_env() {
  static const bool off = getenv("DCF_NO_LN_CARRY") != nullptr;
  return off;
}
#define g_no_carry() (g_no_carry_env() || m->no_ln_carry)
static bool can_carry_ln(dcf_model* m, const float* prod_w, const float* fc_wf, int rows, int n_prod, int k_prod, int E) {
  if (g_no_carry() || !fc_wf || !prod_w || m->gemm_terms == 0 || !m->wsplit.count(fc_wf) || !m->wsplit.count(prod_w)) return false;
  return gemm_can_carry_stats(rows, n_prod, k_prod, 1, m->wsplit_terms[prod_w]) &&
         gemm_can_carry_stats(rows, 4 * E, E, 1, m->wsplit_terms[fc_wf]);
}

static bool can_fuse_ln(dcf_model* m, const float* W, int M, int N, int K, GemmAMode mode) {
  if (M >= 65536) return false;
  return m->gemm_terms != 0 && m->wsplit.count(W) && m->wsplit_ldw[W] == K && K >= 512 && gemm_can_fuse_ln(M, N, K, mode);
}

static bool can_norm_a(dcf_model* m, const float* W1, const float* W2, int M, int C, int* stats_w) {
  if (g_no_carry() || m->gemm_terms == 0 || !m->wsplit.count(W1) || !m->wsplit.count(W2)) return false;
  const int t1 = m->wsplit_terms[W1], t2 = m->wsplit_terms[W2];
  return t1 == t2 && gemm_can_norm_a(M, C, 3 * C, t1, stats_w) && !can_fuse_ln(m, W1, M, C, 3 * C, A_ROWS_TAP3);
}
static void norm_a(GemmArgs& g, const float* stats, int C, int stats_w, const float* ln_g, const float* ln_b) {
  g.a_stats = stats; g.a_stats_slots = C / stats_w; g.a_ln_g = ln_g; g.a_ln_b = ln_b;
}

static int enc_chain_min_rows() {
  const int o = debug_option("enc_chain_min_rows", -1);
  if (o >= 0) return o;
  static const int v = getenv("DCF_ENC_CHAIN_MIN_ROWS") ? atoi(getenv("DCF_ENC_CHAIN_MIN_ROWS")) : 32768;
  return v;
}
static bool can_chain_enc(dcf_model* m, const EncW& w, int rows, int stride, int64_t ldx) {
  static const bool off = getenv("DCF_NO_ENC_CHAIN") != nullptr;
  const dcf_config& c = m->cfg;
  return !off && !m->no_ln_carry && m->gemm_terms == GEMM_F16X3 && w.qkv_chain[0] && w.qkv_chain[1] && w.qkv_chain[2] && stride == 1 &&
         enc_chain_supports(c.E, c.vid_heads, c.win > 0 ? c.win : 99) && rows >= enc_chain_min_rows() && ldx % 4 == 0;
}

static bool fuse_scores_on() {
  static const bool off = getenv("DCF_NO_FUSE_SCORES") != nullptr;
  return !off && debug_option("fuse_scores", 1) != 0;
}
static int enc_attn_min_rows() {
  const int o = debug_option("enc_attn_min_rows", -1);
  if (o >= 0) return o;
  static const int v = getenv("DCF_ENC_ATTN_MIN_ROWS") ? atoi(getenv("DCF_ENC_ATTN_MIN_ROWS")) : 32768;
  return v;
}
static bool can_chain_enc_attn(dcf_model* m, const EncW& w, int rows, int64_t ldr) {
  static const bool off = getenv("DCF_NO_ENC_ATTN") != nullptr;
  const dcf_config& c = m->cfg;
  return !off && m->gemm_terms == GEMM_F16X3 && w.wp_chain && c.win > 0 && (c.win & 1) && enc_chain_supports(c.E, c.vid_heads, c.win) &&
         rows >= enc_attn_min_rows() && ldr % 4 == 0;
}

static int run_encoder(dcf_model* m, const EncW& w, Buffers& b, const float* Xin, int64_t ldx, const uint8_t* mask_in,
                       const uint8_t* mask_out, int B, int T_in, int stride, float* Xout, int64_t ldo, hipStream_t st) {
  const dcf_config& c = m->cfg;
  const int E = c.E, To = T_in / stride, rows = B * To;
  if (can_chain_enc(m, w, rows, stride, ldx)) {
    EncQkvArgs ea{};
    ea.X = Xin; ea.ldx = ldx; ea.mask_in = mask_in; ea.ln_w = w.ln_attn_w; ea.ln_b = w.ln_attn_b;
    ea.dw[0] = w.dw_q; ea.dw[1] = w.dw_k; ea.dw[2] = w.dw_v;
    for (int i = 0; i < 3; ++i) { ea.W[i] = w.qkv_chain[i]; ea.fs[i] = w.qkv_s[i]; ea.fc[i] = w.qkv_c[i]; ea.out[i] = b.R[4 + i]; }
    ea.B = B; ea.T_in = T_in; ea.status = m->status;
    ProfScope prof("gemm_f16x3<enc_qkv>", st, 2.0 * rows * E * 3.0 * E, (double)rows * E * 4.0 * 4.0);
    TRY(launch_enc_qkv(ea, st));
  } else {
  EncPreArgs ep{};
  ep.X = Xin; ep.ldx = ldx; ep.mask_in = mask_in; ep.ln_w = w.ln_attn_w; ep.ln_b = w.ln_attn_b;
  ep.dw_q = w.dw_q; ep.dw_k = w.dw_k; ep.dw_v = w.dw_v;
  ep.qn_w = w.qn_w; ep.qn_b = w.qn_b; ep.kn_w = w.kn_w; ep.kn_b = w.kn_b; ep.vn_w = w.vn_w; ep.vn_b = w.vn_b;
  ep.Qc = b.R[0]; ep.Kc = b.R[1]; ep.Vc = b.R[2]; ep.Skip = stride == 2 ? b.R[3] : nullptr;
  ep.B = B; ep.T_in = T_in; ep.C = E;
  TRY(launch_enc_pre(ep, stride, st));
  GemmArgs g3[3] = {gemm(b.R[0], E, w.wq, w.bq, b.R[4], E, rows, E, E), gemm(b.R[1], E, w.wk, w.bk, b.R[5], E, rows, E, E),
                    gemm(b.R[2], E, w.wv, w.bv, b.R[6], E, rows, E, E)};
  TRY(run_gemm(m, g3, 3, A_ROWS, st));
  }
  if (can_chain_enc_attn(m, w, rows, stride == 2 ? (int64_t)E : ldx)) {
    const bool carry = w.fc_wf && m->wsplit.count(w.fc_wf) && !g_no_carry() &&
                       (can_chain_ffn_rows(m, rows, E) || gemm_can_carry_stats(rows, 4 * E, E, 1, m->wsplit_terms[w.fc_wf]));
    EncAttnArgs aa{};
    aa.Q = b.R[4]; aa.K = b.R[5]; aa.V = b.R[6]; aa.mask = mask_out; aa.Wp = w.wp_chain; aa.bp = w.bp; aa.ls = w.ls_attn;
    if (stride == 2) { aa.R = b.R[3]; aa.ldr = E; } else { aa.R = Xin; aa.ldr = ldx; }
    aa.Y = b.R[1]; aa.ldy = E; aa.stats_out = carry ? b.stats : nullptr; aa.stats_w = STATS_W; aa.B = B; aa.T = To; aa.win = c.win; aa.status = m->status; aa.attn_single = c.attn_mode == 1;
    {
      ProfScope prof("gemm_f16x3<enc_attn>", st, 2.0 * rows * E * E + 4.0 * rows * E * c.win, (double)rows * E * 4.0 * 5.0);
      TRY(launch_enc_attn(aa, st));
    }
    GemmArgs go = gemm(b.HID, 4 * E, w.pj_w, w.pj_b, Xout, ldo, rows, E, 4 * E);
    go.flags = G_RES | G_OUT_MASK; go.rowmask = mask_out; go.ls = w.ls_ffn; go.R = b.R[1]; go.ldr = E;
    if (carry) return run_ffn(m, b.R[1], w.fc_wf, w.fc_c, go, b.HID, rows, E, st, b.stats, w.fc_s);
    LnArgs ln{}; ln.X = b.R[1]; ln.ldx = E; ln.Y = b.R[2]; ln.ldy = E; ln.w = w.ln_ffn_w; ln.b = w.ln_ffn_b; ln.rows = rows; ln.C = E;
    TRY(launch_ln(ln, st));
    return run_ffn(m, b.R[2], w.fc_w, w.fc_b, go, b.HID, rows, E, st);
  }
  if (c.win > 0) {
    LocalAttnArgs la{b.R[4], b.R[5], b.R[6], mask_out, b.R[0], B, To, E, c.vid_heads, c.win};
    TRY(launch_local_attn(la, st));
  } else {
    GlobalAttnArgs ga{b.R[4], b.R[5], b.R[6], mask_out, b.R[0], B, To, E, c.vid_heads};
    TRY(launch_global_attn(ga, st));
  }
  GemmArgs gp = gemm(b.R[0], E, w.wp, w.bp, b.R[1], E, rows, E, E);
  gp.flags = G_RES | G_RES_MASK; gp.rowmask = mask_out; gp.ls = w.ls_attn;
  if (stride == 2) { gp.R = b.R[3]; gp.ldr = E; } else { gp.R = Xin; gp.ldr = ldx; }
  GemmArgs go = gemm(b.HID, 4 * E, w.pj_w, w.pj_b, Xout, ldo, rows, E, 4 * E);
  go.flags = G_RES | G_OUT_MASK; go.rowmask = mask_out; go.ls = w.ls_ffn; go.R = b.R[1]; go.ldr = E;
  if (can_fuse_ln(m, w.wp, rows, E, E, A_ROWS)) {
    gp.ln_w = w.ln_ffn_w; gp.ln_b = w.ln_ffn_b; gp.Y = b.R[2]; gp.ldy = E;
    TRY(run_gemm(m, &gp, 1, A_ROWS, st));
  } else if (can_carry_ln(m, w.wp, w.fc_wf, rows, E, E, E)) {
    gp.stats_out = b.stats; gp.stats_w = STATS_W;
    TRY(run_gemm(m, &gp, 1, A_ROWS, st));
    return run_ffn(m, b.R[1], w.fc_wf, w.fc_c, go, b.HID, rows, E, st, b.stats, w.fc_s);
  } else {
    TRY(run_gemm(m, &gp, 1, A_ROWS, st));
    LnArgs ln{}; ln.X = b.R[1]; ln.ldx = E; ln.Y = b.R[2]; ln.ldy = E; ln.w = w.ln_ffn_w; ln.b = w.ln_ffn_b; ln.rows = rows; ln.C = E;
    TRY(launch_ln(ln, st));
  }
  TRY(run_ffn(m, b.R[2], w.fc_w, w.fc_b, go, b.HID, rows, E, st));
  return 0;
}

static int head_chain_min_rows() {
  static const int v = getenv("DCF_HEAD_CHAIN_MIN_ROWS") ? atoi(getenv("DCF_HEAD_CHAIN_MIN_ROWS")) : 30000;
  return v;
}
static bool g_no_head_chain() {
  static const bool off = getenv("DCF_NO_HEAD_CHAIN") != nullptr;
  return off;
}
static bool can_chain_head(dcf_model* m, const HeadW& h, int rows, int Cin, int NO) {
  if (g_no_head_chain() || rows < head_chain_min_rows() || m->gemm_terms != GEMM_F16X3 || !h.chain[0] || !h.chain[1]) return false;
  if (h.conv.size() != 2 || !head_chain_supports(Cin, NO)) return false;
  for (int i = 0; i < 2; ++i)
    if (!m->wsplit.count(h.conv[i]) || m->wsplit_terms[h.conv[i]] != GEMM_F16X3) return false;
  return true;
}
static HeadChainArgs head_chain_args(dcf_model* m, const HeadW& h, Buffers& b, const Plan& pl, int NO, int mode, int query_major, float* out) {
  HeadChainArgs a{};
  a.X = b.F; a.ldx = m->cfg.E + TCN_HID; a.nbr = b.nbr_all; a.W1c = h.chain[0]; a.W2c = h.chain[1];
  a.ln1_w = h.ln_w[0]; a.ln1_b = h.ln_b[0]; a.ln2_w = h.ln_w[1]; a.ln2_b = h.ln_b[1];
  a.Wout = h.out_w; a.bout = h.out_b; a.lt = pl.d_lt; a.out = out; a.rows = pl.B * pl.lt.S; a.NO = NO; a.mode = mode;
  a.query_major = query_major; a.status = m->status;
  return a;
}
static int run_head_chain(dcf_model* m, const HeadChainArgs* a, int count, int Cin, hipStream_t st) {
  double flops = 0., bytes = 0.;
  for (int i = 0; i < count; ++i) {
    flops += 2.0 * a[i].rows * Cin * 3.0 * Cin * 2.0 + 2.0 * a[i].rows * 3.0 * Cin * a[i].NO;
    bytes += (double)a[i].rows * (Cin + a[i].NO) * 4.0;
  }
  ProfScope prof("gemm_f16x3<head_chain>", st, flops, bytes);
  return launch_head_chain(a, count, Cin, st);
}

static int run_head(dcf_model* m, const HeadW& h, Buffers& b, const Plan& pl, int Cin, int NO, int mode, int query_major,
                    float* out, hipStream_t st, int row0 = 0, int rows = -1) {
  if (row0 == 0 && rows < 0 && can_chain_head(m, h, pl.B * pl.lt.S, Cin, NO)) {
    const HeadChainArgs a = head_chain_args(m, h, b, pl, NO, mode, query_major, out);
    return run_head_chain(m, &a, 1, Cin, st);
  }
  const int rowsAll = rows >= 0 ? rows : pl.B * pl.lt.S;
  const int ldf = m->cfg.E + TCN_HID;
  const float* in = b.F + (int64_t)row0 * ldf;
  int64_t ldin = ldf;
  float* HA = b.HA + (int64_t)row0 * Cin;
  float* HB = b.HB + (int64_t)row0 * Cin;
  const uint8_t* nbr = b.nbr_all + row0;
  const float *last_ln_w = nullptr, *last_ln_b = nullptr;
  float* hst = b.hstats[0] + (int64_t)row0 * ((Cin + 63) / 64) * 2;
  int pending = -1, pend_w = 0;
  for (size_t i = 0; i < h.conv.size(); ++i) {
    GemmArgs g = gemm(in, ldin, h.conv[i], nullptr, HA, Cin, rowsAll, Cin, 3 * Cin);
    g.cin = Cin; g.nbr = nbr;
    float* outp = (in == HB) ? HA : HB;
    if (pending >= 0) { norm_a(g, hst, Cin, pend_w, h.ln_w[pending], h.ln_b[pending]); pending = -1; }
    int sw = 0;
    if (can_fuse_ln(m, h.conv[i], rowsAll, Cin, 3 * Cin, A_ROWS_TAP3) && !g.a_stats) {
      g.C = nullptr; g.ln_w = h.ln_w[i]; g.ln_b = h.ln_b[i]; g.Y = outp; g.ldy = Cin; g.ln_relu = 1;
      TRY(run_gemm(m, &g, 1, A_ROWS_TAP3, st));
    } else if (i + 1 < h.conv.size() && !g.a_stats && can_norm_a(m, h.conv[i], h.conv[i + 1], rowsAll, Cin, &sw)) {
      g.C = outp; g.stats_out = hst; g.stats_w = sw;
      TRY(run_gemm(m, &g, 1, A_ROWS_TAP3, st));
      pending = (int)i; pend_w = sw;
    } else {
      g.C = outp;
      TRY(run_gemm(m, &g, 1, A_ROWS_TAP3, st));
      if (i + 1 == h.conv.size()) {
        last_ln_w = h.ln_w[i]; last_ln_b = h.ln_b[i];
      } else {
        LnArgs ln{}; ln.X = outp; ln.ldx = Cin; ln.Y = outp; ln.ldy = Cin; ln.w = h.ln_w[i]; ln.b = h.ln_b[i];
        ln.rows = rowsAll; ln.C = Cin; ln.relu = 1;
        TRY(launch_ln(ln, st));
      }
    }
    in = outp; ldin = Cin;
  }
  ConvOutArgs co{};
  co.ln_w = last_ln_w; co.ln_b = last_ln_b;
  co.X = in; co.ldx = ldin; co.nbr = nbr; co.W = h.out_w; co.bias = h.out_b; co.lt = pl.d_lt;
  co.out = query_major ? out : out + row0;
  co.rows = rowsAll; co.C = Cin; co.NO = NO; co.row0 = row0; co.mode = mode; co.query_major = query_major;
  TRY(launch_conv_out(co, st));
  return 0;
}

static int run_head_pair(dcf_model* m, const HeadW& h1, const HeadW& h2, Buffers& b, const Plan& pl, int Cin, int NO1, int mode1,
                         float* out1, int NO2, int mode2, float* out2, hipStream_t st) {
  const int rowsAll = pl.B * pl.lt.S;
  if (can_chain_head(m, h1, rowsAll, Cin, NO1) && can_chain_head(m, h2, rowsAll, Cin, NO2)) {
    const HeadChainArgs a[2] = {head_chain_args(m, h1, b, pl, NO1, mode1, 1, out1), head_chain_args(m, h2, b, pl, NO2, mode2, 1, out2)};
    return run_head_chain(m, a, 2, Cin, st);
  }
  bool pair = h1.conv.size() == h2.conv.size() && !h1.conv.empty() && m->gemm_terms != 0;
  for (size_t i = 0; pair && i < h1.conv.size(); ++i)
    pair = !can_fuse_ln(m, h1.conv[i], rowsAll, Cin, 3 * Cin, A_ROWS_TAP3) && m->wsplit.count(h1.conv[i]) && m->wsplit.count(h2.conv[i]);
  if (!pair) {
    TRY(run_head(m, h1, b, pl, Cin, NO1, mode1, 1, out1, st));
    return run_head(m, h2, b, pl, Cin, NO2, mode2, 1, out2, st);
  }
  const int ldf = m->cfg.E + TCN_HID;
  const float* in[2] = {b.F, b.F};
  int64_t ldin = ldf;
  float* buf[2][2] = {{b.HA, b.HB}, {b.HC, b.HD}};
  const HeadW* hs[2] = {&h1, &h2};
  int pending = -1, pend_w = 0;
  for (size_t i = 0; i < h1.conv.size(); ++i) {
    float* outp[2] = {buf[0][i & 1], buf[1][i & 1]};
    GemmArgs g[2];
    for (int k = 0; k < 2; ++k) {
      g[k] = gemm(in[k], ldin, hs[k]->conv[i], nullptr, outp[k], Cin, rowsAll, Cin, 3 * Cin);
      g[k].cin = Cin; g[k].nbr = b.nbr_all;
      if (pending >= 0) norm_a(g[k], b.hstats[k], Cin, pend_w, hs[k]->ln_w[pending], hs[k]->ln_b[pending]);
    }
    const bool was_pending = pending >= 0;
    pending = -1;
    int sw = 0;
    const bool carry = !was_pending && i + 1 < h1.conv.size() && can_norm_a(m, h1.conv[i], h1.conv[i + 1], rowsAll, Cin, &sw) &&
                       can_norm_a(m, h2.conv[i], h2.conv[i + 1], rowsAll, Cin, &sw);
    if (carry)
      for (int k = 0; k < 2; ++k) { g[k].stats_out = b.hstats[k]; g[k].stats_w = sw; }
    TRY(run_gemm(m, g, 2, A_ROWS_TAP3, st));
    if (carry) { pending = (int)i; pend_w = sw; }
    for (int k = 0; k < 2; ++k) {
      if (i + 1 < h1.conv.size() && !carry) {
        LnArgs ln{}; ln.X = outp[k]; ln.ldx = Cin; ln.Y = outp[k]; ln.ldy = Cin; ln.w = hs[k]->ln_w[i]; ln.b = hs[k]->ln_b[i];
        ln.rows = rowsAll; ln.C = Cin; ln.relu = 1;
        TRY(launch_ln(ln, st));
      }
      in[k] = outp[k];
    }
    ldin = Cin;
  }
  const int NOs[2] = {NO1, NO2}, modes[2] = {mode1, mode2};
  float* outs[2] = {out1, out2};
  for (int k = 0; k < 2; ++k) {
    ConvOutArgs co{};
    co.X = in[k]; co.ldx = ldin; co.nbr = b.nbr_all; co.W = hs[k]->out_w; co.bias = hs[k]->out_b; co.lt = pl.d_lt;
    co.out = outs[k]; co.rows = rowsAll; co.C = Cin; co.NO = NOs[k]; co.row0 = 0; co.mode = modes[k]; co.query_major = 1;
    co.ln_w = hs[k]->ln_w.back(); co.ln_b = hs[k]->ln_b.back();
    TRY(launch_conv_out(co, st));
  }
  return 0;
}

static int dec_chain_min_rows() {
  const int o = debug_option("dec_chain_min_rows", -1);
  if (o >= 0) return o;
  static const int v = getenv("DCF_DEC_CHAIN_MIN_ROWS") ? atoi(getenv("DCF_DEC_CHAIN_MIN_ROWS")) : 16384;
  return v;
}
static bool can_chain_dec(dcf_model* m, const DecW& w, const LevelTable* lt, int rows, int64_t ldx, int Lk) {
  static const bool off = getenv("DCF_NO_DEC_CHAIN") != nullptr;
  const dcf_config& c = m->cfg;
  return !off && !lt && m->gemm_terms == GEMM_F16X3 && w.wq_chain && w.wp_chain && dec_chain_supports(c.E, c.fusion_heads, Lk) &&
         c.TE % 32 == 0 && rows >= dec_chain_min_rows() && ldx % 4 == 0;
}

static int run_fusion(dcf_model* m, Buffers& b, float* X, int64_t ldx, int B, int T, const LevelTable* lt, const uint8_t* mask,
                      const uint8_t* nbr, const TextMeta* dm, int Lk, float* out, int64_t ld_out, hipStream_t st,
                      bool* carry_out = nullptr) {
  if (carry_out) *carry_out = false;
  const dcf_config& c = m->cfg;
  const int E = c.E;
  const int rows = lt ? lt->start[lt->n_levels] : B * T;
  for (size_t li = 0; li < m->dec.size(); ++li) {
    const DecW& w = m->dec[li];
    bool carry = false;
    const bool chain = can_chain_dec(m, w, lt, rows, ldx, Lk);
    TextLnArgs tl{*dm, b.kvn, b.kvmask, w.ln_kv_w, w.ln_kv_b, Lk, c.TE};
    TRY(launch_text_ln(tl, B, st));
    GemmArgs gkv[2] = {gemm(b.kvn, c.TE, w.wk, w.bk, b.Kt, E, B * Lk, E, c.TE), gemm(b.kvn, c.TE, w.wv, w.bv, b.Vt, E, B * Lk, E, c.TE)};
    TRY(run_gemm(m, gkv, 2, A_ROWS, st));
    if (chain) {
      const int lk2 = Lk <= 32 ? 1 : 2;
      TRY(launch_kv_image(b.Kt, b.Vt, b.kvmask, B, Lk, lk2, b.kvimg, b.kmadd, st));
      carry = !g_no_carry() && w.fc_wf && m->wsplit.count(w.fc_wf) &&
              (can_chain_ffn_rows(m, rows, E) || gemm_can_carry_stats(rows, 4 * E, E, 1, m->wsplit_terms[w.fc_wf]));
      DecChainArgs da{};
      da.X = X; da.ldx = ldx; da.mask = mask; da.ln_q_w = w.ln_q_w; da.ln_q_b = w.ln_q_b; da.dw = w.dw; da.qn_w = w.qn_w; da.qn_b = w.qn_b;
      da.Wq = w.wq_chain; da.bq = w.bq; da.KV = b.kvimg; da.kmask = b.kmadd; da.Wp = w.wp_chain; da.bp = w.bp_il;
      da.Q3 = b.R[2]; da.ldq = E; da.stats_out = carry ? b.stats : nullptr; da.stats_w = STATS_W;
      da.B = B; da.T = T; da.affine = c.xattn_affine; da.lk2 = lk2; da.status = m->status; da.attn_single = c.attn_mode == 1;
      {
        ProfScope prof("gemm_f16x3<dec_chain>", st, 2.0 * rows * E * 3.0 * E + 4.0 * rows * E * Lk, (double)rows * E * 4.0 * 2.0);
        TRY(launch_dec_chain(da, st));
      }
      if (!carry) {
        LnArgs ln{}; ln.X = b.R[2]; ln.ldx = E; ln.Y = b.R[0]; ln.ldy = E; ln.w = w.ln_ffn_w; ln.b = w.ln_ffn_b; ln.rows = rows; ln.C = E;
        TRY(launch_ln(ln, st));
      }
    } else {
    DecPreArgs dp{X, ldx, mask, w.ln_q_w, w.ln_q_b, w.dw, w.qn_w, w.qn_b, b.R[0], b.R[1], lt ? 1 : B, lt ? rows : T, E};
    dp.nbr = lt ? nbr : nullptr;
    dp.affine = c.xattn_affine;
    TRY(launch_dec_pre(dp, st));
    GemmArgs gq = gemm(b.R[0], E, w.wq, w.bq, b.R[2], E, rows, E, E);
    TRY(run_gemm(m, &gq, 1, A_ROWS, st));
    if (lt) {
      for (int l = 0; l < lt->n_levels; ++l) {
        XAttnArgs xa{b.R[2] + (int64_t)lt->start[l] * E, b.Kt, b.Vt, b.kvmask, b.R[0] + (int64_t)lt->start[l] * E, B, lt->T[l], Lk, E, c.fusion_heads, m->status, c.attn_mode == 1};
        TRY(launch_xattn(xa, st));
      }
    } else {
      XAttnArgs xa{b.R[2], b.Kt, b.Vt, b.kvmask, b.R[0], B, T, Lk, E, c.fusion_heads, m->status, c.attn_mode == 1};
      TRY(launch_xattn(xa, st));
    }
    if (m->gemm_terms != 0 && w.wp_il && m->wsplit.count(w.wp_il) && gemm_can_fuse_adaln(rows, 2 * E, E)) {
      GemmArgs gh = gemm(b.R[0], E, w.wp_il, w.bp_il, b.R[2], E, rows, 2 * E, E);
      gh.flags = G_ADALN; gh.R = b.R[1]; gh.ldr = E;
      carry = can_carry_ln(m, w.wp_il, w.fc_wf, rows, 2 * E, E, E);
      if (carry) { gh.stats_out = b.stats; gh.stats_w = STATS_W; }
      TRY(run_gemm(m, &gh, 1, A_ROWS, st));
      if (!carry) {
        LnArgs ln{}; ln.X = b.R[2]; ln.ldx = E; ln.Y = b.R[0]; ln.ldy = E; ln.w = w.ln_ffn_w; ln.b = w.ln_ffn_b; ln.rows = rows; ln.C = E;
        TRY(launch_ln(ln, st));
      }
    } else {
      GemmArgs gh = gemm(b.R[0], E, w.wp, w.bp, b.H2, 2 * E, rows, 2 * E, E);
      TRY(run_gemm(m, &gh, 1, A_ROWS, st));
      TRY(launch_dec_mid(b.R[1], b.H2, w.ln_ffn_w, w.ln_ffn_b, b.R[2], b.R[0], rows, E, st));
    }
    }
    GemmArgs go = gemm(b.HID, 4 * E, w.pj_w, w.pj_b, X, ldx, rows, E, 4 * E);
    go.flags = G_RES | G_OUT_MASK; go.rowmask = mask; go.ls = w.ls_ffn; go.R = b.R[2]; go.ldr = E;
    const float* fc_in = carry ? b.R[2] : b.R[0];
    const float *fc_w = carry ? w.fc_wf : w.fc_w, *fc_b = carry ? w.fc_c : w.fc_b;
    if (li + 1 == m->dec.size() && m->fus_out_w && can_fuse_ln(m, w.pj_w, rows, E, 4 * E, A_ROWS)) {
      GemmArgs gf = gemm(fc_in, E, fc_w, fc_b, b.HID, 4 * E, rows, 4 * E, E);
      gf.flags = G_GELU;
      if (carry) { gf.stats_in = b.stats; gf.ln_s = w.fc_s; gf.stats_slots = E / STATS_W; gf.stats_w = STATS_W; }
      TRY(run_gemm(m, &gf, 1, A_ROWS, st));
      go.C = nullptr; go.ln_w = m->fus_out_w; go.ln_b = m->fus_out_b; go.Y = out; go.ldy = ld_out;
      TRY(run_gemm(m, &go, 1, A_ROWS, st));
      return 0;
    }
    if (li + 1 == m->dec.size() && carry_out && m->fus_out_w && ldx == E &&
        m->embd_fc_wf && m->wsplit.count(m->embd_fc_wf) && !g_no_carry() &&
        m->wsplit.count(w.pj_w) && gemm_can_carry_stats(rows, E, 4 * E, 1, m->wsplit_terms[w.pj_w]) &&
        gemm_can_carry_stats(rows, E, E, 1, m->wsplit_terms[m->embd_fc_wf])) {
      go.stats_out = b.stats; go.stats_w = STATS_W;
      TRY(run_ffn(m, fc_in, fc_w, fc_b, go, b.HID, rows, E, st, carry ? b.stats : nullptr, w.fc_s));
      *carry_out = true;
      return 0;
    }
    TRY(run_ffn(m, fc_in, fc_w, fc_b, go, b.HID, rows, E, st, carry ? b.stats : nullptr, w.fc_s));
  }
  if (!m->fus_out_w) return 0;
  LnArgs ln{}; ln.X = X; ln.ldx = ldx; ln.Y = out; ln.ldy = ld_out; ln.w = m->fus_out_w; ln.b = m->fus_out_b; ln.rows = rows; ln.C = E;
  TRY(launch_ln(ln, st));
  return 0;
}

enum { DROP_R_VPROJ = 0, DROP_R_VPATH, DROP_R_FPROJ, DROP_R_FPATH, DROP_R_REFINE };
static DropSite drop_at(const dcf_model* m, int rate, uint32_t site) {
  DropSite d;
  d.site = site; d.p = m->drop->p[rate]; d.scale = m->drop->scale[rate];
  return d;
}

static int run_encoder_drop(dcf_model* m, const EncW& w, Buffers& b, const float* Xin, int64_t ldx, const uint8_t* mask_in,
                            const uint8_t* mask_out, int B, int T_in, int stride, float* Xout, int64_t ldo, uint32_t site0,
                            hipStream_t st) {
  const dcf_config& c = m->cfg;
  const int E = c.E, To = T_in / stride, rows = B * To;
  const auto& d = *m->drop;
  EncPreArgs ep{};
  ep.X = Xin; ep.ldx = ldx; ep.mask_in = mask_in; ep.ln_w = w.ln_attn_w; ep.ln_b = w.ln_attn_b;
  ep.dw_q = w.dw_q; ep.dw_k = w.dw_k; ep.dw_v = w.dw_v;
  ep.qn_w = w.qn_w; ep.qn_b = w.qn_b; ep.kn_w = w.kn_w; ep.kn_b = w.kn_b; ep.vn_w = w.vn_w; ep.vn_b = w.vn_b;
  ep.Qc = b.R[0]; ep.Kc = b.R[1]; ep.Vc = b.R[2]; ep.Skip = stride == 2 ? b.R[3] : nullptr;
  ep.B = B; ep.T_in = T_in; ep.C = E;
  TRY(launch_enc_pre(ep, stride, st));
  GemmArgs g3[3] = {gemm(b.R[0], E, w.wq, w.bq, b.R[4], E, rows, E, E), gemm(b.R[1], E, w.wk, w.bk, b.R[5], E, rows, E, E),
                    gemm(b.R[2], E, w.wv, w.bv, b.R[6], E, rows, E, E)};
  TRY(run_gemm(m, g3, 3, A_ROWS, st));
  if (c.win > 0) {
    LocalAttnArgs la{b.R[4], b.R[5], b.R[6], mask_out, b.R[0], B, To, E, c.vid_heads, c.win};
    TRY(launch_local_attn(la, st));
  } else {
    GlobalAttnArgs ga{b.R[4], b.R[5], b.R[6], mask_out, b.R[0], B, To, E, c.vid_heads};
    TRY(launch_global_attn(ga, st));
  }
  GemmArgs gp = gemm(b.R[0], E, w.wp, w.bp, b.R[4], E, rows, E, E);
  TRY(run_gemm(m, &gp, 1, A_ROWS, st));
  DropResArgs ra{};
  ra.out = b.R[1]; ra.ldo = E;
  if (stride == 2) { ra.R = b.R[3]; ra.ldr = E; } else { ra.R = Xin; ra.ldr = ldx; }
  ra.H = b.R[4]; ra.ldh = E; ra.rowmask = mask_out; ra.res_mask = 1; ra.out_mask = 0; ra.ls = w.ls_attn;
  ra.rows = rows; ra.C = E; ra.T = To; ra.b0 = d.b0; ra.seed = d.seed;
  ra.drop = drop_at(m, DROP_R_VPROJ, site0 | DROP_PROJ); ra.path = drop_at(m, DROP_R_VPATH, site0 | DROP_PATH_ATTN);
  TRY(launch_drop_residual(ra, st));
  LnArgs ln{}; ln.X = b.R[1]; ln.ldx = E; ln.Y = b.R[2]; ln.ldy = E; ln.w = w.ln_ffn_w; ln.b = w.ln_ffn_b; ln.rows = rows; ln.C = E;
  TRY(launch_ln(ln, st));
  GemmArgs gf = gemm(b.R[2], E, w.fc_w, w.fc_b, b.HID, 4 * E, rows, 4 * E, E);
  gf.flags = G_GELU;
  TRY(run_gemm(m, &gf, 1, A_ROWS, st));
  TRY(launch_dropout(b.HID, 4 * E, rows, 4 * E, To, d.b0, d.seed, drop_at(m, DROP_R_VPROJ, site0 | DROP_FFN_HID), st));
  GemmArgs go = gemm(b.HID, 4 * E, w.pj_w, w.pj_b, b.R[4], E, rows, E, 4 * E);
  TRY(run_gemm(m, &go, 1, A_ROWS, st));
  ra.out = Xout; ra.ldo = ldo; ra.R = b.R[1]; ra.ldr = E; ra.res_mask = 0; ra.out_mask = 1; ra.ls = w.ls_ffn;
  ra.drop = drop_at(m, DROP_R_VPROJ, site0 | DROP_FFN_OUT); ra.path = drop_at(m, DROP_R_VPATH, site0 | DROP_PATH_FFN);
  return launch_drop_residual(ra, st);
}

static int run_fusion_drop(dcf_model* m, Buffers& b, float* X, int64_t ldx, int B, int T, const uint8_t* mask, const TextMeta* dm,
                           int Lk, float* out, int64_t ld_out, hipStream_t st) {
  const dcf_config& c = m->cfg;
  const int E = c.E, rows = B * T;
  const auto& d = *m->drop;
  for (size_t li = 0; li < m->dec.size(); ++li) {
    const DecW& w = m->dec[li];
    const uint32_t site0 = drop_site(DROP_G_FUSION, (uint32_t)li, 0);
    TextLnArgs tl{*dm, b.kvn, b.kvmask, w.ln_kv_w, w.ln_kv_b, Lk, c.TE};
    TRY(launch_text_ln(tl, B, st));
    GemmArgs gkv[2] = {gemm(b.kvn, c.TE, w.wk, w.bk, b.Kt, E, B * Lk, E, c.TE), gemm(b.kvn, c.TE, w.wv, w.bv, b.Vt, E, B * Lk, E, c.TE)};
    TRY(run_gemm(m, gkv, 2, A_ROWS, st));
    DecPreArgs dp{X, ldx, mask, w.ln_q_w, w.ln_q_b, w.dw, w.qn_w, w.qn_b, b.R[0], b.R[1], B, T, E};
    dp.nbr = nullptr;
    dp.affine = c.xattn_affine;
    TRY(launch_dec_pre(dp, st));
    GemmArgs gq = gemm(b.R[0], E, w.wq, w.bq, b.R[2], E, rows, E, E);
    TRY(run_gemm(m, &gq, 1, A_ROWS, st));
    XAttnArgs xa{b.R[2], b.Kt, b.Vt, b.kvmask, b.R[0], B, T, Lk, E, c.fusion_heads, m->status, c.attn_mode == 1};
    TRY(launch_xattn(xa, st));
    GemmArgs gh = gemm(b.R[0], E, w.wp, w.bp, b.H2, 2 * E, rows, 2 * E, E);
    TRY(run_gemm(m, &gh, 1, A_ROWS, st));
    TRY(launch_dropout(b.H2, 2 * E, rows, 2 * E, T, d.b0, d.seed, drop_at(m, DROP_R_FPROJ, site0 | DROP_PROJ), st));
    TRY(launch_dec_mid(b.R[1], b.H2, w.ln_ffn_w, w.ln_ffn_b, b.R[2], b.R[0], rows, E, st));
    GemmArgs gf = gemm(b.R[0], E, w.fc_w, w.fc_b, b.HID, 4 * E, rows, 4 * E, E);
    gf.flags = G_GELU;
    TRY(run_gemm(m, &gf, 1, A_ROWS, st));
    TRY(launch_dropout(b.HID, 4 * E, rows, 4 * E, T, d.b0, d.seed, drop_at(m, DROP_R_FPROJ, site0 | DROP_FFN_HID), st));
    GemmArgs go = gemm(b.HID, 4 * E, w.pj_w, w.pj_b, b.R[1], E, rows, E, 4 * E);
    TRY(run_gemm(m, &go, 1, A_ROWS, st));
    DropResArgs ra{};
    ra.out = X; ra.ldo = ldx; ra.R = b.R[2]; ra.ldr = E; ra.H = b.R[1]; ra.ldh = E; ra.rowmask = mask; ra.res_mask = 0; ra.out_mask = 1;
    ra.ls = w.ls_ffn; ra.rows = rows; ra.C = E; ra.T = T; ra.b0 = d.b0; ra.seed = d.seed;
    ra.drop = drop_at(m, DROP_R_FPROJ, site0 | DROP_FFN_OUT); ra.path = drop_at(m, DROP_R_FPATH, site0 | DROP_PATH_FFN);
    TRY(launch_drop_residual(ra, st));
  }
  LnArgs ln{}; ln.X = X; ln.ldx = ldx; ln.Y = out; ln.ldy = ld_out; ln.w = m->fus_out_w; ln.b = m->fus_out_b; ln.rows = rows; ln.C = E;
  return launch_ln(ln, st);
}

constexpr int DCF_MAX_VIDEOS = 16;
struct VideoSet {
  int nvid = 0;
  const float* vid[DCF_MAX_VIDEOS];
  const float* shallow[DCF_MAX_VIDEOS];
  const uint8_t* mask[DCF_MAX_VIDEOS];
  const float* text_cls[DCF_MAX_VIDEOS];
  int nq[DCF_MAX_VIDEOS];
  float* logits1_out = nullptr;
};

struct MaskPtrs { const uint8_t* p[DCF_MAX_VIDEOS]; };
__global__ void k_gather_masks(MaskPtrs mp, uint8_t* __restrict__ dst, int T0) {
  const int t = blockIdx.x * blockDim.x + threadIdx.x;
  if (t < T0) dst[(size_t)blockIdx.y * T0 + t] = mp.p[blockIdx.y][t];
}


struct HybridState {
  bool valid = false;
  int k = 0, Tn = 0, Tc = 0, B = 0, Lk = 0;
  Buffers bn{};
  Plan pn{}, pc{}, pch{};
  float *Fc = nullptr, *logits1c = nullptr, *stacked = nullptr;
  uint8_t *maskc = nullptr, *nbrc = nullptr;
};

static void free_hybrid(dcf_model* m) {
  if (!m->hyb) return;
  for (Plan* p : {&m->hyb->pn, &m->hyb->pc, &m->hyb->pch}) if (p->d_lt) (void)hipFree(p->d_lt);
  delete m->hyb;
  m->hyb = nullptr;
}

static int make_plan(dcf_model* m, Plan& p, const int* Tl, int n, int B, const float* scales, hipStream_t st) {
  p.T0 = Tl[0]; p.B = B; p.L = n;
  LevelTable& lt = p.lt;
  lt = LevelTable{};
  lt.n_levels = n; lt.B = B;
  int acc = 0;
  for (int l = 0; l < n; ++l) {
    lt.T[l] = Tl[l]; lt.off[l] = acc; lt.start[l] = B * acc; lt.scale[l] = scales ? scales[l] : 1.f;
    acc += Tl[l];
  }
  lt.S = acc; lt.start[n] = B * acc;
  if (!p.d_lt) DCF_HIP(hipMalloc(&p.d_lt, sizeof(LevelTable)));
  DCF_HIP(hipMemcpyAsync(p.d_lt, &p.lt, sizeof(LevelTable), hipMemcpyHostToDevice, st));
  DCF_HIP(hipStreamSynchronize(st));
  (void)m;
  return 0;
}

static size_t hybrid_extra_bytes(const dcf_config& c, int B, int Tc, int LC, int Tn, int L) {
  size_t rows = 0;
  for (int j = 0; j < LC; ++j) rows += (size_t)B * (Tc >> j);
  const size_t EH = c.E + TCN_HID;
  return rows * EH * 4 + 2 * (rows + 256) + rows * 4 + (size_t)B * Tn * L * 4 + 8 * 256;
}

static int hybrid_take(dcf_model* m, const Buffers& b, const Plan& pl, int B, int Lk, hipStream_t st) {
  HybridState& h = *m->hyb;
  const dcf_config& c = m->cfg;
  const int E = c.E, ldf = E + TCN_HID, k = h.k;
  h.bn = b; h.B = B; h.Lk = Lk;
  h.pn.lt = pl.lt; h.pn.T0 = pl.T0; h.pn.B = pl.B; h.pn.L = pl.L;
  if (!h.pn.d_lt) DCF_HIP(hipMalloc(&h.pn.d_lt, sizeof(LevelTable)));
  DCF_HIP(hipMemcpyAsync(h.pn.d_lt, pl.d_lt, sizeof(LevelTable), hipMemcpyDeviceToDevice, st));
  const int LC = c.n_levels - k;
  Arena a{m->hyb_extra_ptr, 0, m->hyb_extra, false};
  size_t rows = 0;
  for (int j = 0; j < LC; ++j) rows += (size_t)B * (h.Tc >> j);
  h.Fc = a.take<float>(rows * ldf);
  h.maskc = a.take<uint8_t>(rows);
  h.nbrc = a.take<uint8_t>(rows);
  h.logits1c = a.take<float>(rows);
  h.stacked = a.take<float>((size_t)B * h.Tn * c.n_levels);
  DCF_CHECK(a.off <= m->hyb_extra, "internal: hybrid workspace");
  DCF_HIP(hipMemcpy2DAsync(m->hyb_feat_out, (size_t)E * 4, b.F + (int64_t)pl.lt.start[k] * ldf, (size_t)ldf * 4, (size_t)E * 4,
                           (size_t)B * pl.lt.T[k], hipMemcpyDeviceToDevice, st));
  h.valid = true;
  return 0;
}

__global__ void k_hybrid_stack(const float* __restrict__ l1n, const LevelTable* __restrict__ ltn, const float* __restrict__ l1c,
                               const LevelTable* __restrict__ ltc, const uint8_t* __restrict__ mask0, float* __restrict__ out,
                               int B, int Tn, int k, int L, int off_k) {
  const int r = blockIdx.x * blockDim.x + threadIdx.x;
  if (r >= B * Tn) return;
  const int b = r / Tn, t = r - b * Tn;
  const float m0 = mask0[r] ? 1.f : 0.f;
  for (int l = 0; l < L; ++l) {
    float u;
    if (l <= k) u = l1n[ltn->start[l] + b * ltn->T[l] + (t >> l)];
    else {
      const int j = l - k - 1;
      int i = ((t >> k) + off_k) >> (j + 1);
      i = i < 0 ? 0 : (i < ltc->T[j] ? i : ltc->T[j] - 1);
      u = l1c[ltc->start[j] + b * ltc->T[j] + i];
    }
    out[(int64_t)r * L + l] = l > 0 ? u * m0 : u;
  }
}

static int tcn_stack_env() {
  static const int v = getenv("DCF_TCN_STACK") ? atoi(getenv("DCF_TCN_STACK")) : -1;
  return v;
}
static RefineArgs refine_args(dcf_model* m) {
  RefineArgs ra{};
  ra.w_in = m->tcn_in_w; ra.b_in = m->tcn_in_b;
  ra.host_w_dil = m->tcn_wd.data(); ra.host_b_dil = m->tcn_bd.data(); ra.host_w_pw = m->tcn_wp.data();
  ra.host_b_pw = m->tcn_bp.data(); ra.host_ln_w = m->tcn_lnw.data(); ra.host_ln_b = m->tcn_lnb.data();
  ra.w_out = m->tcn_out_w; ra.b_out = m->tcn_out_b;
  ra.host_frag = (!m->tcn_frag.empty() && debug_option("tcn_frag", 1) != 0) ? m->tcn_frag.data() : nullptr;
  ra.stack_layers = debug_option("tcn_stack", tcn_stack_env());
  ra.f16 = m->gemm_terms == GEMM_F16X3; ra.status = m->status;
  return ra;
}

static Buffers hybrid_coarse_heads(const HybridState& h, int ldf) {
  Buffers bc = h.bn;
  const int s1 = h.pc.lt.start[1];
  bc.F = h.Fc + (int64_t)s1 * ldf; bc.mask_all = h.maskc + s1; bc.nbr_all = h.nbrc + s1; bc.logits1 = h.logits1c;
  return bc;
}

static int hybrid_phase2(dcf_model* m, const float* featk_c, const uint8_t* maskk_c, int off_k, float* refk_out, hipStream_t st) {
  HybridState& h = *m->hyb;
  const dcf_config& c = m->cfg;
  const int E = c.E, ldf = E + TCN_HID, k = h.k, L = c.n_levels, LC = L - k, B = h.B;
  DCF_HIP(hipMemcpy2DAsync(h.Fc, (size_t)ldf * 4, featk_c, (size_t)E * 4, (size_t)E * 4, (size_t)B * h.Tc, hipMemcpyDeviceToDevice, st));
  for (int b = 0; b < B; ++b) DCF_HIP(hipMemcpyAsync(h.maskc + (size_t)b * h.Tc, maskk_c, (size_t)h.Tc, hipMemcpyDeviceToDevice, st));
  TRY(launch_pyramid_masks(h.maskc, h.nbrc, B, h.Tc, LC, h.pc.lt.start[LC], st));
  const LevelTable& lc = h.pc.lt;
  for (int j = 1; j < LC; ++j) {
    const float* xin = h.Fc + (int64_t)lc.start[j - 1] * ldf;
    float* xo = h.Fc + (int64_t)lc.start[j] * ldf;
    if (c.pool_only) TRY(launch_dwconv3(xin, ldf, h.maskc + lc.start[j - 1], m->pool_w[k + j], xo, ldf, B, lc.T[j - 1], 2, E, st));
    else TRY(run_encoder(m, m->branch[k + j], h.bn, xin, ldf, h.maskc + lc.start[j - 1], h.maskc + lc.start[j], B, lc.T[j - 1], 2, xo, ldf, st));
  }
  TRY(run_head(m, m->cls1, h.bn, h.pn, E, 1, 0, 0, h.bn.logits1, st));
  Buffers bc = hybrid_coarse_heads(h, ldf);
  if (LC > 1) TRY(run_head(m, m->cls1, bc, h.pch, E, 1, 0, 0, h.logits1c, st));
// ... 926 lines not shown
  dcf::VotingArgs a{nms_segs, nms_ld, n1_counts, n1_max, n1_stride, all_segs, all_scores, n2_counts, n2_max, n2_stride,
                    iou_thresh, out};
  return dcf::launch_voting(a, nq, (hipStream_t)stream);
}

int dcf_op_linear(const float* A, const float* W, const float* bias, float* C, int32_t M, int32_t N, int32_t K,
                  int32_t act, void* stream) {
  dcf::GemmArgs g = dcf::gemm(A, K, W, bias, C, N, M, N, K);
  g.flags = act == 1 ? dcf::G_GELU : act == 2 ? dcf::G_RELU : 0;
  return dcf::launch_gemm(&g, 1, dcf::A_ROWS, (hipStream_t)stream);
}

int dcf_op_linear_split(const float* A, const float* W, const float* bias, float* C, int32_t M, int32_t N, int32_t K,
                        int32_t act, int32_t nterms, void* stream) {
  hipStream_t st = (hipStream_t)stream;
  unsigned short* planes = nullptr;
  DCF_HIP(hipMallocAsync((void**)&planes, (size_t)3 * N * K * sizeof(unsigned short), st));
  int rc = dcf::launch_split_planes(W, planes, N, K, K, st, nterms);
  if (rc == 0) {
    dcf::GemmArgs g = dcf::gemm(A, K, W, bias, C, N, M, N, K);
    g.Ws = planes;
    g.flags = act == 1 ? dcf::G_GELU : act == 2 ? dcf::G_RELU : 0;
    rc = dcf::launch_gemm_split(&g, 1, dcf::A_ROWS, nterms, st);
  }
  DCF_HIP(hipFreeAsync(planes, st));
  return rc;
}

int dcf_op_linear_cm(const float* A_cm, const float* W, const float* bias, float* C, int32_t M, int32_t N, int32_t K,
                     void* stream) {
  dcf::GemmArgs g = dcf::gemm(A_cm, M, W, bias, C, N, M, N, K);
  return dcf::launch_gemm(&g, 1, dcf::A_CHANMAJOR, (hipStream_t)stream);
}

int dcf_op_linear_ln(const float* A, const float* W, const float* bias, const float* ln_w, const float* ln_b, float* C, float* Y,
                     int32_t M, int32_t N, int32_t K, int32_t relu, int32_t nterms, void* stream) {
  hipStream_t st = (hipStream_t)stream;
  DCF_CHECK(dcf::gemm_can_fuse_ln(M, N, K, dcf::A_ROWS), "dcf_op_linear_ln: %dx%dx%d cannot carry a fused LayerNorm (N = 256, M >= 28672)", M, N, K);
  unsigned short* planes = nullptr;
  DCF_HIP(hipMallocAsync((void**)&planes, (size_t)3 * N * K * sizeof(unsigned short), st));
  int rc = dcf::launch_split_planes(W, planes, N, K, K, st, nterms);
  if (rc == 0) {
    dcf::GemmArgs g = dcf::gemm(A, K, W, bias, C, N, M, N, K);
    g.Ws = planes;
    g.ln_w = ln_w; g.ln_b = ln_b; g.Y = Y; g.ldy = N; g.ln_relu = relu;
    rc = dcf::launch_gemm_split(&g, 1, dcf::A_ROWS, nterms, st);
  }
  DCF_HIP(hipFreeAsync(planes, st));
  return rc;
}

int dcf_op_linear_ln_carry(const float* A, const float* W1, const float* b1, const float* R, const float* ln_w, const float* ln_b,
                           const float* W2, const float* b2, float* X, float* Y, int32_t M, int32_t N1, int32_t K1, int32_t N2,
                           int32_t gelu, int32_t nterms, void* stream) {
  hipStream_t st = (hipStream_t)stream;
  DCF_CHECK(A && W1 && ln_w && ln_b && W2 && X && Y, "dcf_op_linear_ln_carry: null argument");
  DCF_CHECK(N1 % 64 == 0 && dcf::gemm_can_carry_stats(M, N1, K1, 1, nterms) && dcf::gemm_can_carry_stats(M, N2, N1, 1, nterms),
            "dcf_op_linear_ln_carry: %dx%dx%d -> %d runs on the k-sliced kernel (no row statistics there)", M, N1, K1, N2);
  unsigned short *p1 = nullptr, *p2 = nullptr;
  float *wf = nullptr, *stats = nullptr;
  DCF_HIP(hipMallocAsync((void**)&p1, (size_t)3 * N1 * K1 * sizeof(unsigned short), st));
  DCF_HIP(hipMallocAsync((void**)&p2, (size_t)3 * N2 * N1 * sizeof(unsigned short), st));
  DCF_HIP(hipMallocAsync((void**)&wf, ((size_t)N2 * N1 + 2 * (size_t)N2) * sizeof(float), st));
  DCF_HIP(hipMallocAsync((void**)&stats, (size_t)M * (N1 / 64) * 2 * sizeof(float), st));
  float* sv = wf + (size_t)N2 * N1;
  hipLaunchKernelGGL(dcf::k_fold_ln, dim3(N2), dim3(64), 0, st, W2, b2, ln_w, ln_b, wf, sv, sv + N2, N1);
  int rc = dcf::launch_split_planes(W1, p1, N1, K1, K1, st, nterms);
  if (rc == 0) rc = dcf::launch_split_planes(wf, p2, N2, N1, N1, st, nterms);
  if (rc == 0) {
    dcf::GemmArgs g = dcf::gemm(A, K1, W1, b1, X, N1, M, N1, K1);
    g.Ws = p1; g.stats_out = stats; g.stats_w = 64;
    if (R) { g.flags = dcf::G_RES; g.R = R; g.ldr = N1; }
    rc = dcf::launch_gemm_split(&g, 1, dcf::A_ROWS, nterms, st);
  }
  if (rc == 0) {
    dcf::GemmArgs g = dcf::gemm(X, N1, wf, sv + N2, Y, N2, M, N2, N1);
    g.Ws = p2; g.flags = gelu ? dcf::G_GELU : 0;
    g.stats_in = stats; g.ln_s = sv; g.stats_slots = N1 / 64; g.stats_w = 64;
    rc = dcf::launch_gemm_split(&g, 1, dcf::A_ROWS, nterms, st);
  }
  DCF_HIP(hipFreeAsync(p1, st)); DCF_HIP(hipFreeAsync(p2, st)); DCF_HIP(hipFreeAsync(wf, st)); DCF_HIP(hipFreeAsync(stats, st));
  return rc;
}

int dcf_op_ffn(const float* X, const float* ln_w, const float* ln_b, const float* W1, const float* b1, const float* W2, const float* b2,
               const float* ls, const uint8_t* mask, float* C, float* stats_out, int32_t M, int32_t E, int32_t chain, void* stream) {
  hipStream_t st = (hipStream_t)stream;
  DCF_CHECK(X && W1 && b1 && W2 && b2 && C && M > 0 && E % 64 == 0, "dcf_op_ffn: bad argument");
  DCF_CHECK(!chain || E == 256, "dcf_op_ffn: the one-kernel form exists for E = 256 only");
  DCF_CHECK(chain >= 0 && chain <= 3, "dcf_op_ffn: chain = %d (0 .. 3)", chain);
  DCF_CHECK(C != X, "dcf_op_ffn: C must not alias X");
  DCF_CHECK(!stats_out || chain || dcf::gemm_can_carry_stats(M, E, 4 * E, 1, dcf::GEMM_F16X3), "dcf_op_ffn: %d rows run on a kernel without row statistics", M);
  const int H = 4 * E, nterms = dcf::GEMM_F16X3;
  unsigned short *p1 = nullptr, *p2 = nullptr;
  float *wf = nullptr, *stats = nullptr, *xn = nullptr, *hid = nullptr;
  DCF_HIP(hipMallocAsync((void**)&p1, (size_t)3 * H * E * sizeof(unsigned short), st));
  DCF_HIP(hipMallocAsync((void**)&p2, (size_t)3 * H * E * sizeof(unsigned short), st));
  const float *fc_w = W1, *fc_b = b1, *fc_s = nullptr, *fc_in = X;
  int rc = 0;
  if (ln_w && chain) {
    DCF_HIP(hipMallocAsync((void**)&wf, ((size_t)H * E + 2 * (size_t)H) * sizeof(float), st));
    DCF_HIP(hipMallocAsync((void**)&stats, (size_t)M * (E / 64) * 2 * sizeof(float), st));
    float* sv = wf + (size_t)H * E;
    hipLaunchKernelGGL(dcf::k_fold_ln, dim3(H), dim3(64), 0, st, W1, b1, ln_w, ln_b, wf, sv, sv + H, E);
    rc = dcf::launch_row_stats(X, E, stats, M, E, 64, st);
    fc_w = wf; fc_s = sv; fc_b = sv + H;
  } else if (ln_w) {
    DCF_HIP(hipMallocAsync((void**)&xn, (size_t)M * E * sizeof(float), st));
    dcf::LnArgs ln{}; ln.X = X; ln.ldx = E; ln.Y = xn; ln.ldy = E; ln.w = ln_w; ln.b = ln_b; ln.rows = M; ln.C = E;
    rc = dcf::launch_ln(ln, st);
    fc_in = xn;
  }
  if (rc == 0) rc = dcf::launch_split_planes(fc_w, p1, H, E, E, st, nterms);
  if (rc == 0) rc = dcf::launch_split_planes(W2, p2, E, H, H, st, nterms);
  if (rc == 0 && chain) {
    dcf::FfnChainArgs a{};
    a.X = X; a.ldx = E; a.W1s = p1; a.b1 = fc_b; a.ln_s = fc_s; a.stats = stats; a.stats_slots = E / 64; a.W2s = p2; a.b2 = b2; a.ls = ls;
    a.R = X; a.ldr = E; a.rowmask = mask; a.C = C; a.ldc = E; a.stats_out = stats_out; a.stats_w = 64; a.M = M;
    a.variant = chain == 1 ? 0 : chain - 1;
    unsigned* word = nullptr;
    unsigned flag = 0u;
    if (ln_w) {
      if (hipMallocAsync((void**)&word, sizeof(unsigned), st) != hipSuccess) { word = nullptr; rc = -1; dcf::set_error("dcf_op_ffn: hipMallocAsync failed"); }
      if (rc == 0 && hipMemsetAsync(word, 0, sizeof(unsigned), st) != hipSuccess) { rc = -1; dcf::set_error("dcf_op_ffn: hipMemsetAsync failed"); }
    }
    a.status = word;
    if (rc == 0) rc = dcf::launch_ffn_chain(a, st);
    if (rc == 0 && word) {
      if (hipMemcpyAsync(&flag, word, sizeof(flag), hipMemcpyDeviceToHost, st) != hipSuccess || hipStreamSynchronize(st) != hipSuccess) {
        rc = -1; dcf::set_error("dcf_op_ffn: reading the numerics word failed");
      }
    }
    if (word) (void)hipFreeAsync(word, st);
    if (rc == 0 && ln_w && (flag & 2u)) {
      DCF_HIP(hipMallocAsync((void**)&xn, (size_t)M * E * sizeof(float), st));
      dcf::LnArgs ln{}; ln.X = X; ln.ldx = E; ln.Y = xn; ln.ldy = E; ln.w = ln_w; ln.b = ln_b; ln.rows = M; ln.C = E;
      rc = dcf::launch_ln(ln, st);
      if (rc == 0) rc = dcf::launch_split_planes(W1, p1, H, E, E, st, nterms);
      a.X = xn; a.b1 = b1; a.ln_s = nullptr; a.stats = nullptr; a.status = nullptr;
      if (rc == 0) rc = dcf::launch_ffn_chain(a, st);
    }
  } else if (rc == 0) {
    DCF_HIP(hipMallocAsync((void**)&hid, (size_t)M * H * sizeof(float), st));
    dcf::GemmArgs gf = dcf::gemm(fc_in, E, fc_w, fc_b, hid, H, M, H, E);
    gf.Ws = p1; gf.flags = dcf::G_GELU;
    rc = dcf::launch_gemm_split(&gf, 1, dcf::A_ROWS, nterms, st);
    if (rc == 0) {
      dcf::GemmArgs go = dcf::gemm(hid, H, W2, b2, C, E, M, E, H);
      go.Ws = p2; go.flags = dcf::G_RES | (mask ? dcf::G_OUT_MASK : 0); go.rowmask = mask; go.ls = ls; go.R = X; go.ldr = E;
      if (stats_out) { go.stats_out = stats_out; go.stats_w = 64; }
      rc = dcf::launch_gemm_split(&go, 1, dcf::A_ROWS, nterms, st);
    }
  }
  DCF_HIP(hipFreeAsync(p1, st)); DCF_HIP(hipFreeAsync(p2, st));
  if (wf) DCF_HIP(hipFreeAsync(wf, st));
  if (stats) DCF_HIP(hipFreeAsync(stats, st));
  if (xn) DCF_HIP(hipFreeAsync(xn, st));
  if (hid) DCF_HIP(hipFreeAsync(hid, st));
  return rc;
}

int dcf_op_linear_cm_split(const float* A_cm, const float* W, const float* bias, float* C, int32_t M, int32_t N, int32_t K,
                           int32_t nterms, void* stream) {
  hipStream_t st = (hipStream_t)stream;
  unsigned short* planes = nullptr;
  DCF_HIP(hipMallocAsync((void**)&planes, (size_t)3 * N * K * sizeof(unsigned short), st));
  int rc = dcf::launch_split_planes(W, planes, N, K, K, st, nterms);
  if (rc == 0) {
    dcf::GemmArgs g = dcf::gemm(A_cm, M, W, bias, C, N, M, N, K);
    g.Ws = planes;
    rc = dcf::launch_gemm_split(&g, 1, dcf::A_CHANMAJOR, nterms, st);
  }
  DCF_HIP(hipFreeAsync(planes, st));
  return rc;
}

int dcf_op_conv3(const float* X, const uint8_t* mask, const float* W_ock, float* Y, int32_t B, int32_t T, int32_t Cin,
                 int32_t N, void* stream) {
  hipStream_t st = (hipStream_t)stream;
  const int rows = B * T;
  float* wp = nullptr;
  uint8_t* nbr = nullptr;
  DCF_HIP(hipMallocAsync((void**)&wp, (size_t)N * Cin * 3 * sizeof(float), st));
  DCF_HIP(hipMallocAsync((void**)&nbr, (size_t)rows, st));
  const int n = N * Cin * 3;
  hipLaunchKernelGGL(dcf::k_permute3, dim3((n + 255) / 256), dim3(256), 0, st, W_ock, wp, N, Cin, 3, 0, 2, 1);
  int rc = dcf::launch_rowflags(mask, nbr, T, rows, st);
  if (rc == 0) {
    dcf::GemmArgs g = dcf::gemm(X, Cin, wp, nullptr, Y, N, rows, N, 3 * Cin);
    g.cin = Cin; g.nbr = nbr;
    rc = dcf::launch_gemm(&g, 1, dcf::A_ROWS_TAP3, st);
  }
  DCF_HIP(hipFreeAsync(wp, st));
  DCF_HIP(hipFreeAsync(nbr, st));
  return rc;
}

int dcf_op_conv3_split(const float* X, const uint8_t* mask, const float* W_ock, float* Y, int32_t B, int32_t T, int32_t Cin,
                       int32_t N, int32_t nterms, void* stream) {
  hipStream_t st = (hipStream_t)stream;
  const int rows = B * T;
  float* wp = nullptr;
  uint8_t* nbr = nullptr;
  unsigned short* planes = nullptr;
  DCF_HIP(hipMallocAsync((void**)&wp, (size_t)N * Cin * 3 * sizeof(float), st));
  DCF_HIP(hipMallocAsync((void**)&nbr, (size_t)rows, st));
  DCF_HIP(hipMallocAsync((void**)&planes, (size_t)3 * N * Cin * 3 * sizeof(unsigned short), st));
  const int n = N * Cin * 3;
  hipLaunchKernelGGL(dcf::k_permute3, dim3((n + 255) / 256), dim3(256), 0, st, W_ock, wp, N, Cin, 3, 0, 2, 1);
  int rc = dcf::launch_rowflags(mask, nbr, T, rows, st);
  if (rc == 0) rc = dcf::launch_split_planes(wp, planes, N, 3 * Cin, 3 * Cin, st, nterms);
  if (rc == 0) {
    dcf::GemmArgs g = dcf::gemm(X, Cin, wp, nullptr, Y, N, rows, N, 3 * Cin);
    g.cin = Cin; g.nbr = nbr; g.Ws = planes;
    rc = dcf::launch_gemm_split(&g, 1, dcf::A_ROWS_TAP3, nterms, st);
  }
  DCF_HIP(hipFreeAsync(wp, st));
  DCF_HIP(hipFreeAsync(nbr, st));
  DCF_HIP(hipFreeAsync(planes, st));
  return rc;
}

int dcf_op_head(const float* X, const uint8_t* mask, const float* W1, const float* ln1_w, const float* ln1_b, const float* W2,
                const float* ln2_w, const float* ln2_b, const float* Wout, const float* bout, float* out, int32_t B, int32_t T,
                int32_t C, int32_t NO, float scale, int32_t chain, void* stream) {
  hipStream_t st = (hipStream_t)stream;
  DCF_CHECK(X && mask && W1 && ln1_w && ln1_b && W2 && ln2_w && ln2_b && Wout && bout && out && B > 0 && T > 0, "dcf_op_head: null argument");
  DCF_CHECK((NO == 1 || NO == 2) && C % 32 == 0, "dcf_op_head: NO = %d, C = %d", NO, C);
  DCF_CHECK(!chain || dcf::head_chain_supports(C, NO), "dcf_op_head: the one-kernel form exists for C = 256 / 288 only");
  const int rows = B * T, nterms = dcf::GEMM_F16X3;
  float *wp[2] = {nullptr, nullptr}, *wo = nullptr, *ha = nullptr, *hb = nullptr;
  uint8_t* nbr = nullptr;
  unsigned short* img[2] = {nullptr, nullptr};
  dcf::LevelTable lt{}, *d_lt = nullptr;
  lt.n_levels = 1; lt.B = B; lt.S = T; lt.T[0] = T; lt.start[0] = 0; lt.start[1] = rows; lt.off[0] = 0; lt.scale[0] = scale;
  DCF_HIP(hipMallocAsync((void**)&d_lt, sizeof(lt), st));
  DCF_HIP(hipMemcpyAsync(d_lt, &lt, sizeof(lt), hipMemcpyHostToDevice, st));
  DCF_HIP(hipStreamSynchronize(st));
  DCF_HIP(hipMallocAsync((void**)&nbr, (size_t)rows, st));
  DCF_HIP(hipMallocAsync((void**)&wo, (size_t)NO * C * 3 * sizeof(float), st));
  const size_t img_halfs = chain ? dcf::head_chain_image_halfs(C) : (size_t)3 * C * C * 3;
  const float* Ws[2] = {W1, W2};
  int rc = dcf::launch_rowflags(mask, nbr, T, rows, st);
  for (int i = 0; i < 2 && rc == 0; ++i) {
    DCF_HIP(hipMallocAsync((void**)&wp[i], (size_t)C * C * 3 * sizeof(float), st));
    DCF_HIP(hipMallocAsync((void**)&img[i], img_halfs * sizeof(unsigned short), st));
    const int n = C * C * 3;
    hipLaunchKernelGGL(dcf::k_permute3, dim3((n + 255) / 256), dim3(256), 0, st, Ws[i], wp[i], C, C, 3, 0, 2, 1);
    rc = chain ? dcf::launch_split_chain3(wp[i], img[i], C, st) : dcf::launch_split_planes(wp[i], img[i], C, 3 * C, 3 * C, st, nterms);
  }
  {
    const int n = NO * C * 3;
    hipLaunchKernelGGL(dcf::k_permute3, dim3((n + 255) / 256), dim3(256), 0, st, Wout, wo, NO, C, 3, 0, 2, 1);
  }
  const int mode = scale != 0.f ? 1 : 0;
  if (rc == 0 && chain) {
    dcf::HeadChainArgs a{};
    a.X = X; a.ldx = C; a.nbr = nbr; a.W1c = img[0]; a.W2c = img[1]; a.ln1_w = ln1_w; a.ln1_b = ln1_b; a.ln2_w = ln2_w; a.ln2_b = ln2_b;
    a.Wout = wo; a.bout = bout; a.lt = d_lt; a.out = out; a.rows = rows; a.NO = NO; a.mode = mode; a.query_major = 0;
    rc = dcf::launch_head_chain(&a, 1, C, st);
  } else if (rc == 0) {
    DCF_HIP(hipMallocAsync((void**)&ha, (size_t)rows * C * sizeof(float), st));
    DCF_HIP(hipMallocAsync((void**)&hb, (size_t)rows * C * sizeof(float), st));
    const float* in = X;
    float* bufs[2] = {ha, hb};
    const float *lw[2] = {ln1_w, ln2_w}, *lb[2] = {ln1_b, ln2_b};
    for (int i = 0; i < 2 && rc == 0; ++i) {
      dcf::GemmArgs g = dcf::gemm(in, C, wp[i], nullptr, bufs[i], C, rows, C, 3 * C);
      g.cin = C; g.nbr = nbr; g.Ws = img[i];
      rc = dcf::launch_gemm_split(&g, 1, dcf::A_ROWS_TAP3, nterms, st);
      if (rc == 0) {
        dcf::LnArgs ln{}; ln.X = bufs[i]; ln.ldx = C; ln.Y = bufs[i]; ln.ldy = C; ln.w = lw[i]; ln.b = lb[i]; ln.rows = rows; ln.C = C; ln.relu = 1;
        rc = dcf::launch_ln(ln, st);
      }
      in = bufs[i];
    }
    if (rc == 0) {
      dcf::ConvOutArgs co{};
      co.X = in; co.ldx = C; co.nbr = nbr; co.W = wo; co.bias = bout; co.lt = d_lt; co.out = out; co.rows = rows; co.C = C; co.NO = NO;
      co.row0 = 0; co.mode = mode; co.query_major = 0;
      rc = dcf::launch_conv_out(co, st);
    }
  }
  for (int i = 0; i < 2; ++i) { if (wp[i]) DCF_HIP(hipFreeAsync(wp[i], st)); if (img[i]) DCF_HIP(hipFreeAsync(img[i], st)); }
  if (ha) DCF_HIP(hipFreeAsync(ha, st));
  if (hb) DCF_HIP(hipFreeAsync(hb, st));
  DCF_HIP(hipFreeAsync(wo, st)); DCF_HIP(hipFreeAsync(nbr, st)); DCF_HIP(hipFreeAsync(d_lt, st));
  return rc;
}

int dcf_op_layernorm(const float* X, const float* w, const float* b, float* Y, int32_t rows, int32_t C, int32_t relu,
                     void* stream) {
  dcf::LnArgs a{};
  a.X = X; a.ldx = C; a.Y = Y; a.ldy = C; a.w = w; a.b = b; a.rows = rows; a.C = C; a.relu = relu;
  return dcf::launch_ln(a, (hipStream_t)stream);
}

int dcf_op_xattn(const float* Q, const float* K, const float* V, const uint8_t* kvmask, float* O, int32_t B, int32_t T,
                 int32_t Lk, int32_t C, int32_t heads, void* stream) {
  dcf::XAttnArgs a{Q, K, V, kvmask, O, B, T, Lk, C, heads};
  return dcf::launch_xattn(a, (hipStream_t)stream);
}

int dcf_op_local_attn(const float* Q, const float* K, const float* V, const uint8_t* mask, float* O, int32_t B, int32_t T,
                      int32_t C, int32_t heads, int32_t window, void* stream) {
  if (window == 0) {
    dcf::GlobalAttnArgs g{Q, K, V, mask, O, B, T, C, heads};
    return dcf::launch_global_attn(g, (hipStream_t)stream);
  }
  dcf::LocalAttnArgs a{Q, K, V, mask, O, B, T, C, heads, window};
  return dcf::launch_local_attn(a, (hipStream_t)stream);
}

int dcf_op_sidekick(const float* shallow, const float* text_cls, float* correl, int32_t D, int32_t T, int32_t nq,
                    int32_t norm, void* stream) {
  hipStream_t st = (hipStream_t)stream;
  float *tn = nullptr, *partial = nullptr;
  DCF_HIP(hipMallocAsync((void**)&tn, (size_t)nq * D * sizeof(float), st));
  DCF_HIP(hipMallocAsync((void**)&partial, (size_t)dcf::SCORE_SLICES * (nq + 1) * T * sizeof(float), st));
  int rc = dcf::launch_sidekick(dcf::score_args(shallow, text_cls, tn, partial, correl, D, T, nq, norm), st);
  DCF_HIP(hipFreeAsync(tn, st));
  DCF_HIP(hipFreeAsync(partial, st));
  return rc;
}

int dcf_op_gate(const float* correl, const uint8_t* vid_mask, float* gate, uint8_t* mask_out, int32_t T, int32_t nq,
                int32_t sn, double sratio, int32_t msf, void* stream) {
  dcf::GateArgs a{correl, vid_mask, gate, mask_out, T, nq, 0, sn, msf, sratio};
  return dcf::launch_gate(a, (hipStream_t)stream);
}

namespace dcf {
static int scratch_begin(dcf_model* m, const char* what, hipStream_t st) {
  DCF_CHECK(m && !m->finalized, "%s: needs a scratch model (dcf_model_create + dcf_model_bind of the block's parameters, not finalized)", what);
  return init_gemm_mode(m, st);
}
static int scratch_end(dcf_model* m, hipStream_t st, int rc) {
  (void)hipStreamSynchronize(st);
  for (float* p : m->owned) (void)hipFree(p);
  m->owned.clear();
  m->wsplit.clear(); m->wsplit_ldw.clear(); m->wsplit_terms.clear();
  m->dec.clear();
  m->fus_out_w = m->fus_out_b = nullptr;
  return rc;
}
struct ScratchArena {
  char* base = nullptr;
  ~ScratchArena() { if (base) (void)hipFree(base); }
};
}

int dcf_op_encoder(dcf_model* m, const char* prefix, const float* X, const uint8_t* mask, int32_t B, int32_t T, int32_t stride,
                   float* Y, uint8_t* mask_out, void* stream) {
  using namespace dcf;
  hipStream_t st = (hipStream_t)stream;
  DCF_CHECK(prefix && X && mask && Y && mask_out && B >= 1 && T >= 1 && (stride == 1 || stride == 2) && T % stride == 0, "dcf_op_encoder: bad arguments");
  if (scratch_begin(m, "dcf_op_encoder", st)) return -1;
  const dcf_config& c = m->cfg;
  const int half = c.win / 2;
  DCF_CHECK(half == 0 || (T / stride) % half == 0, "dcf_op_encoder: T / stride = %d must be a multiple of win//2 = %d (blocks.py:216)", T / stride, half);
  EncW w{};
  int rc = resolve_encoder(m, prefix, c.E, st, w);
  ScratchArena sa;
  if (rc == 0) {
    Buffers b{};
    Arena dry{nullptr, 0, 0, true};
    carve(dry, c, T, B, B, T, 1, 1, b);
    if (hipMalloc(&sa.base, dry.off) != hipSuccess) { set_error("dcf_op_encoder: out of memory"); rc = -1; }
    if (rc == 0) {
      Arena real{sa.base, 0, dry.off, false};
      carve(real, c, T, B, B, T, 1, 1, b);
      if (stride == 2) rc = launch_mask_down(mask, mask_out, B * T / 2, st);
      else if (hipMemcpyAsync(mask_out, mask, (size_t)B * T, hipMemcpyDeviceToDevice, st) != hipSuccess) rc = -1;
      if (rc == 0) rc = run_encoder(m, w, b, X, c.E, mask, mask_out, B, T, stride, Y, c.E, st);
    }
  }
  return scratch_end(m, st, rc);
}

int dcf_op_enc_pre(dcf_model* m, const char* prefix, const float* X, const uint8_t* mask, int32_t B, int32_t T, int32_t stride,
                   float* Qc, float* Kc, float* Vc, float* Skip, void* stream) {
  using namespace dcf;
  hipStream_t st = (hipStream_t)stream;
  DCF_CHECK(prefix && X && mask && Qc && Kc && Vc && B >= 1 && T >= 1 && (stride == 1 || (stride == 2 && Skip)) && T % stride == 0, "dcf_op_enc_pre: bad arguments");
  if (scratch_begin(m, "dcf_op_enc_pre", st)) return -1;
  EncW w{};
  int rc = resolve_encoder(m, prefix, m->cfg.E, st, w);
  if (rc == 0) {
    EncPreArgs ep{};
    ep.X = X; ep.ldx = m->cfg.E; ep.mask_in = mask; ep.ln_w = w.ln_attn_w; ep.ln_b = w.ln_attn_b;
    ep.dw_q = w.dw_q; ep.dw_k = w.dw_k; ep.dw_v = w.dw_v;
    ep.qn_w = w.qn_w; ep.qn_b = w.qn_b; ep.kn_w = w.kn_w; ep.kn_b = w.kn_b; ep.vn_w = w.vn_w; ep.vn_b = w.vn_b;
    ep.Qc = Qc; ep.Kc = Kc; ep.Vc = Vc; ep.Skip = stride == 2 ? Skip : nullptr;
    ep.B = B; ep.T_in = T; ep.C = m->cfg.E;
    rc = launch_enc_pre(ep, stride, st);
  }
  return scratch_end(m, st, rc);
}

int dcf_op_decoder(dcf_model* m, const char* prefix, float* X, const uint8_t* mask, int32_t B, int32_t T,
                   const float* const* text, const uint8_t* const* text_mask, const int32_t* text_len, void* stream) {
  using namespace dcf;
  hipStream_t st = (hipStream_t)stream;
  DCF_CHECK(prefix && X && mask && text && text_len && B >= 1 && B <= DCF_MAX_BATCH && T >= 1, "dcf_op_decoder: bad arguments");
  if (scratch_begin(m, "dcf_op_decoder", st)) return -1;
  const dcf_config& c = m->cfg;
  DecW w{};
  int rc = resolve_decoder(m, prefix, c.E, c.TE, st, w);
  ScratchArena sa;
  if (rc == 0) {
    m->dec.assign(1, w);
    m->fus_out_w = m->fus_out_b = nullptr;
    int Lk = 1;
    TextMeta tm{};
    for (int i = 0; i < B; ++i) {
      tm.text[i] = text[i]; tm.text_mask[i] = text_mask ? text_mask[i] : nullptr; tm.len[i] = text_len[i];
      Lk = std::max(Lk, (int)text_len[i]);
    }
    Buffers b{};
    Arena dry{nullptr, 0, 0, true};
    carve(dry, c, T, B, B, T, Lk, 1, b);
    if (hipMalloc(&sa.base, dry.off) != hipSuccess) { set_error("dcf_op_decoder: out of memory"); rc = -1; }
    if (rc == 0) {
      Arena real{sa.base, 0, dry.off, false};
      carve(real, c, T, B, B, T, Lk, 1, b);
      rc = run_fusion(m, b, X, c.E, B, T, nullptr, mask, nullptr, &tm, Lk, X, c.E, st);
    }
  }
  return scratch_end(m, st, rc);
}

int dcf_op_tcn(dcf_model* m, const char* prefix, const float* x, const uint8_t* mask, int32_t B, int32_t T, int32_t n_in,
               int32_t n_layers, float* Y, void* stream) {
  using namespace dcf;
  hipStream_t st = (hipStream_t)stream;
  DCF_CHECK(prefix && x && mask && Y && B >= 1 && T >= 1 && n_in >= 1 && n_in <= DCF_MAX_LEVELS && n_layers >= 0, "dcf_op_tcn: bad arguments");
  if (scratch_begin(m, "dcf_op_tcn", st)) return -1;
  int rc = resolve_tcn(m, prefix, n_in, n_layers, st);
  float* buf = nullptr;
  if (rc == 0 && hipMalloc(&buf, (size_t)2 * B * T * TCN_HID * sizeof(float)) != hipSuccess) { set_error("dcf_op_tcn: out of memory"); rc = -1; }
  if (rc == 0) {
    LevelTable lt{};
    lt.n_levels = n_in; lt.B = B; lt.T[0] = T; lt.S = T;
    RefineArgs ra{};
    ra.stacked = x; ra.mask_all = mask;
    ra.w_in = m->tcn_in_w; ra.b_in = m->tcn_in_b;
    ra.host_w_dil = m->tcn_wd.data(); ra.host_b_dil = m->tcn_bd.data(); ra.host_w_pw = m->tcn_wp.data();
    ra.host_b_pw = m->tcn_bp.data(); ra.host_ln_w = m->tcn_lnw.data(); ra.host_ln_b = m->tcn_lnb.data();
    ra.w_out = m->tcn_out_w; ra.b_out = m->tcn_out_b;
    ra.host_frag = (!m->tcn_frag.empty() && dcf::debug_option("tcn_frag", 1) != 0) ? m->tcn_frag.data() : nullptr;
    ra.stack_layers = dcf::debug_option("tcn_stack", tcn_stack_env());
    ra.bufA = buf; ra.bufB = buf + (size_t)B * T * TCN_HID; ra.F = Y; ra.ldf = TCN_HID; ra.E = 0;
    ra.B = B; ra.T0 = T; ra.n_levels = n_in; ra.n_layers = n_layers;
    ra.f16 = m->gemm_terms == GEMM_F16X3; ra.status = m->status;
    rc = launch_refine(ra, lt, st);
  }
  rc = scratch_end(m, st, rc);
  if (buf) (void)hipFree(buf);
  return rc;
}

}
```

### include/decafnet_hip.h

```cpp
#ifndef DECAFNET_HIP_H
#define DECAFNET_HIP_H

#include <stdint.h>

#ifdef __cplusplus
extern "C" {
#endif

const char* dcf_last_error(void);
int dcf_abi_version(void);

typedef struct dcf_model dcf_model;

typedef struct dcf_config {
  int32_t D;
  int32_t E;
  int32_t TE;
  int32_t vid_heads;
  int32_t fusion_heads;
  int32_t fusion_layers;
  int32_t n_embd_convs;
  int32_t n_stem;
  int32_t n_levels;
  int32_t win;
  int32_t head_layers;
  int32_t sn;
  float sratio;
  int32_t msf;
  int32_t norm;
  int32_t use_abs_pe;
  int32_t max_batch;
  int32_t gemm_mode;
  int32_t model_kind;
  int32_t second_fusion;
  int32_t text_in;
  int32_t text_layers;
  int32_t text_heads;
  int32_t text_abs_pe;
  int32_t text_bkgd;
  int32_t scat;
  int32_t sfonly;
  int32_t text_kind;
  int32_t xattn_affine;
  int32_t vid_stride;
  int32_t pool_only;
  int32_t attn_mode;
} dcf_config;

int dcf_model_create(const dcf_config* cfg, dcf_model** out);
void dcf_model_destroy(dcf_model* m);

int dcf_model_bind(dcf_model* m, const char* name, const float* data, const int64_t* shape, int32_t ndim);

int dcf_numerics_status(dcf_model* m, int32_t reset, void* stream);
int dcf_numerics_status_async(dcf_model* m, int32_t* host_dst, void* stream);
int dcf_model_set_ln_carry(dcf_model* m, int32_t on);

int dcf_model_set_pe(dcf_model* m, const float* pe_tokens, int64_t T);

int dcf_model_set_text_pe(dcf_model* m, const float* pe_tokens, int64_t L);

int dcf_text_encode(dcf_model* m, const float* tokens, const uint8_t* token_mask, int32_t Lq, float* text_out,
                    uint8_t* mask_out, void* stream);

int dcf_model_finalize(dcf_model* m, void* stream);

int64_t dcf_points_per_query(const dcf_model* m, int64_t T);

int dcf_forward_eval(dcf_model* m, const float* vid, const float* shallow_vid, const uint8_t* vid_mask, int64_t T,
                     int32_t nq, const float* const* text, const uint8_t* const* text_mask, const int32_t* text_len,
                     const float* text_cls, float* logits_out, float* offsets_out, uint8_t* masks_out, void* stream);

int dcf_forward_eval_gated(dcf_model* m, const float* vid, const float* shallow_vid, const uint8_t* vid_mask, int64_t T,
                           int32_t nq, const float* const* text, const uint8_t* const* text_mask, const int32_t* text_len,
                           const float* gate, float* logits_out, float* offsets_out, uint8_t* masks_out, void* stream);

int dcf_forward_train_videos(dcf_model* m, int32_t nvid, const float* const* vid, const float* const* shallow_vid,
                             const uint8_t* const* vid_mask, int64_t T, const int32_t* nq_per_video, const float* const* text,
                             const uint8_t* const* text_mask, const int32_t* text_len, const float* const* text_cls,
                             float* logits1_out, float* logits2_out, float* offsets_out, uint8_t* masks_out, void* stream);

int dcf_model_set_dropout(dcf_model* m, float vid_proj_p, float vid_path_p, float fus_proj_p, float fus_path_p, float refine_p,
                          int64_t seed);
int dcf_debug_dropout_keep(int64_t seed, int32_t site, int64_t e0, int64_t n, float p, uint8_t* out, void* stream);

int dcf_sigmoid_focal_loss(const float* inputs, const float* targets, const uint8_t* select, int64_t n, float alpha, float gamma,
                           int32_t smoothing, float* elem_out, float* sum_out, int32_t* count_out, void* stream);
int dcf_ctr_iou_loss(const float* input_offsets, const float* target_offsets, const uint8_t* select, int64_t n, int32_t kind,
                     float eps, float* elem_out, float* sum_out, int32_t* count_out, void* stream);

int dcf_annotate_points(const float* targets, int32_t nrows, int64_t T, int32_t L, double regression_range, double sigma, int32_t use_offset,
                        int64_t max_seq_len, int32_t center_sampling, double radius, uint8_t* labels_out, float* offsets_out,
                        uint8_t* in_window_out, uint8_t* in_range_out, void* stream);
int dcf_point_objective(const float* logits1, const float* logits2, const float* offsets, const uint8_t* masks, const float* targets,
                        int32_t nrows, int64_t T, int32_t L, double regression_range, double sigma, int32_t use_offset, int64_t max_seq_len,
                        int32_t center_sampling, double radius, float alpha, double smoothing, int32_t iou_kind, float eps,
                        const float* loss_norm_dev, float world_size, float loss_weight, float* rows_out, float* out4, void* stream);

int dcf_sigmoid_focal_loss_grad(const float* inputs, const float* targets, const uint8_t* select, int64_t n, float alpha, float gamma,
                                int32_t smoothing, const float* grad_elem, const float* grad_scalar, const int32_t* count_dev,
                                float* grad_out, void* stream);
int dcf_ctr_iou_loss_grad(const float* input_offsets, const float* target_offsets, const uint8_t* select, int64_t n, int32_t kind,
                          float eps, const float* grad_elem, const float* grad_scalar, const int32_t* count_dev, float* grad_out,
                          void* stream);
int dcf_point_objective_grad(const float* logits1, const float* logits2, const float* offsets, const uint8_t* masks, const float* targets,
                             int32_t nrows, int64_t T, int32_t L, double regression_range, double sigma, int32_t use_offset, int64_t max_seq_len,
                             int32_t center_sampling, double radius, float alpha, double smoothing, int32_t iou_kind, float eps,
                             const float* loss_norm_dev, float world_size, float loss_weight, const float* grad_total_dev,
                             const float* grad_parts_dev, float* g_logits1, float* g_logits2, float* g_offsets, int32_t accumulate,
                             float* rows_out, float* out4, void* stream);

int dcf_forward_eval_videos(dcf_model* m, int32_t nvid, const float* const* vid, const float* const* shallow_vid,
                            const uint8_t* const* vid_mask, int64_t T, const int32_t* nq_per_video, const float* const* text,
                            const uint8_t* const* text_mask, const int32_t* text_len, const float* const* text_cls,
                            float* logits_out, float* offsets_out, uint8_t* masks_out, void* stream);

int dcf_debug_copy(dcf_model* m, int32_t what, float* dst, int64_t max_floats, void* stream);

int dcf_hybrid_phase1(dcf_model* m, int32_t k, const float* vid_w, const float* shallow_w, const uint8_t* mask_w, int64_t Tn, int64_t Tc,
                      int32_t nq, const float* const* text, const uint8_t* const* text_mask, const int32_t* text_len, const float* gate_w,
                      float* featk_out, void* stream);
int dcf_hybrid_phase2(dcf_model* m, const float* featk_c, const uint8_t* maskk_c, int64_t off_k, float* refk_out, void* stream);
int dcf_hybrid_phase3(dcf_model* m, const float* refk_c, float* logits_n, float* offsets_n, uint8_t* masks_n, float* logits_c,
                      float* offsets_c, uint8_t* masks_c, void* stream);

int dcf_graph_active(const dcf_model* m);
int dcf_model_set_graph_mode(dcf_model* m, int32_t mode);
int dcf_debug_set_option(const char* name, int32_t value);
int dcf_calib_mfma_rate(int32_t shape, int32_t mfmas_per_wave, int32_t* n_cus, float* ns_per_mfma);

int dcf_collect_segments(const float* logits, const float* offsets, const uint8_t* masks, int32_t nq, int64_t T,
                         int32_t n_levels, float pre_nms_thresh, int32_t pre_nms_topk, float seg_len_thresh,
                         float* segs_out, float* scores_out, int32_t* counts_out, void* stream);

int dcf_collect_segments_ext(const float* logits, const float* offsets, const uint8_t* masks, const float* ext_scores,
                             int32_t nq, int64_t T, int32_t n_levels, float pre_nms_thresh, int32_t pre_nms_topk,
                             float seg_len_thresh, float* segs_out, float* scores_out, int32_t* counts_out, void* stream);

int dcf_nms_1d(const float* segs, const float* scores, const int32_t* counts, int32_t nq, int32_t n_max,
               int32_t stride, float iou_thresh, int64_t* keep_out, int32_t* keep_counts_out, void* stream);
int dcf_softnms_1d(const float* segs, const float* scores, const int32_t* counts, int32_t nq, int32_t n_max,
                   int32_t stride, float iou_thresh, float sigma, float min_score, int32_t method,
                   int32_t max_iters, float* dets_out, int64_t* inds_out, int32_t* out_counts, void* stream);
int dcf_segment_voting(const float* nms_segs, int32_t nms_ld, const int32_t* n1_counts, int32_t n1_max,
                       int32_t n1_stride, const float* all_segs, const float* all_scores,
                       const int32_t* n2_counts, int32_t n2_max, int32_t n2_stride, float iou_thresh,
                       int32_t nq, float* out, void* stream);

int dcf_profile_enable(int32_t on);
int64_t dcf_profile_report(char* buf, int64_t cap);

int dcf_op_linear(const float* A, const float* W, const float* bias, float* C, int32_t M, int32_t N, int32_t K,
                  int32_t act, void* stream);
int dcf_op_linear_split(const float* A, const float* W, const float* bias, float* C, int32_t M, int32_t N, int32_t K,
                        int32_t act, int32_t nterms, void* stream);
int dcf_op_linear_cm(const float* A_cm, const float* W, const float* bias, float* C, int32_t M, int32_t N, int32_t K,
                     void* stream);
int dcf_op_linear_ln(const float* A, const float* W, const float* bias, const float* ln_w, const float* ln_b, float* C, float* Y,
                     int32_t M, int32_t N, int32_t K, int32_t relu, int32_t nterms, void* stream);

int dcf_op_linear_ln_carry(const float* A, const float* W1, const float* b1, const float* R, const float* ln_w, const float* ln_b,
                           const float* W2, const float* b2, float* X, float* Y, int32_t M, int32_t N1, int32_t K1, int32_t N2,
                           int32_t gelu, int32_t nterms, void* stream);

int dcf_op_ffn(const float* X, const float* ln_w, const float* ln_b, const float* W1, const float* b1, const float* W2, const float* b2,
               const float* ls, const uint8_t* mask, float* C, float* stats_out, int32_t M, int32_t E, int32_t chain, void* stream);

int dcf_op_linear_cm_split(const float* A_cm, const float* W, const float* bias, float* C, int32_t M, int32_t N, int32_t K,
                           int32_t nterms, void* stream);
int dcf_op_head(const float* X, const uint8_t* mask, const float* W1, const float* ln1_w, const float* ln1_b, const float* W2,
                const float* ln2_w, const float* ln2_b, const float* Wout, const float* bout, float* out, int32_t B, int32_t T,
                int32_t C, int32_t NO, float scale, int32_t chain, void* stream);

int dcf_op_conv3(const float* X, const uint8_t* mask, const float* W_ock, float* Y, int32_t B, int32_t T, int32_t Cin,
                 int32_t N, void* stream);
int dcf_op_conv3_split(const float* X, const uint8_t* mask, const float* W_ock, float* Y, int32_t B, int32_t T, int32_t Cin,
                       int32_t N, int32_t nterms, void* stream);
int dcf_op_layernorm(const float* X, const float* w, const float* b, float* Y, int32_t rows, int32_t C, int32_t relu,
                     void* stream);
int dcf_op_xattn(const float* Q, const float* K, const float* V, const uint8_t* kvmask, float* O, int32_t B, int32_t T,
                 int32_t Lk, int32_t C, int32_t heads, void* stream);
int dcf_op_local_attn(const float* Q, const float* K, const float* V, const uint8_t* mask, float* O, int32_t B, int32_t T,
                      int32_t C, int32_t heads, int32_t window, void* stream);
int dcf_op_sidekick(const float* shallow, const float* text_cls, float* correl, int32_t D, int32_t T, int32_t nq,
                    int32_t norm, void* stream);
int dcf_op_gate(const float* correl, const uint8_t* vid_mask, float* gate, uint8_t* mask_out, int32_t T, int32_t nq,
                int32_t sn, double sratio, int32_t msf, void* stream);

int dcf_op_encoder(dcf_model* m, const char* prefix, const float* X, const uint8_t* mask, int32_t B, int32_t T, int32_t stride,
                   float* Y, uint8_t* mask_out, void* stream);
int dcf_op_enc_pre(dcf_model* m, const char* prefix, const float* X, const uint8_t* mask, int32_t B, int32_t T, int32_t stride,
                   float* Qc, float* Kc, float* Vc, float* Skip, void* stream);
int dcf_op_decoder(dcf_model* m, const char* prefix, float* X, const uint8_t* mask, int32_t B, int32_t T,
                   const float* const* text, const uint8_t* const* text_mask, const int32_t* text_len, void* stream);
int dcf_op_tcn(dcf_model* m, const char* prefix, const float* x, const uint8_t* mask, int32_t B, int32_t T, int32_t n_in,
               int32_t n_layers, float* Y, void* stream);

#ifdef __cplusplus
}
#endif
#endif
```

Baseline: 21.64 million clips/s.

## Fold query and output projections into per-video key/value images for decoder cross-attention

Precomputes per-batch matrices M = Wq^T K (scaled) and N = Wp V per head, plus a bias-times-key mask term, in a new fold-image kernel. The fused decoder chain then computes attention scores directly from the normalized input against M and applies N to the softmax probabilities, skipping the separate Q projection and output projection GEMMs. It also skips N pieces for key slots beyond Lk. This trades E×E per-row GEMMs for work proportional to Lk (32 here), at the cost of an extra per-video precompute kernel and an overflow check on the split-f16 images.

```diff
diff --git a/cvpr2025-decafnet_amd/_lib.py b/cvpr2025-decafnet_amd/_lib.py
--- a/cvpr2025-decafnet_amd/_lib.py
+++ b/cvpr2025-decafnet_amd/_lib.py
@@ -84,6 +84,7 @@
     'dcf_op_conv3_split': (i32, [c_f32p, c_u8p, c_f32p, c_f32p, i32, i32, i32, i32, i32, vp]),
     'dcf_op_layernorm': (i32, [c_f32p, c_f32p, c_f32p, c_f32p, i32, i32, i32, vp]),
     'dcf_op_xattn': (i32, [c_f32p, c_f32p, c_f32p, c_u8p, c_f32p, i32, i32, i32, i32, i32, vp]),
+    'dcf_op_dec_fold_image': (i32, [c_f32p, c_f32p, c_u8p, c_f32p, c_f32p, c_f32p, i32, i32, vp, vp, c_f32p, vp, vp]),
     'dcf_op_local_attn': (i32, [c_f32p, c_f32p, c_f32p, c_u8p, c_f32p, i32, i32, i32, i32, i32, vp]),
     'dcf_op_sidekick': (i32, [c_f32p, c_f32p, c_f32p, i32, i32, i32, i32, vp]),
     'dcf_op_gate': (i32, [c_f32p, c_u8p, c_f32p, c_u8p, i32, i32, i32, f64, i32, vp]),
diff --git a/cvpr2025-decafnet_amd/csrc/dec_chain.h b/cvpr2025-decafnet_amd/csrc/dec_chain.h
--- a/cvpr2025-decafnet_amd/csrc/dec_chain.h
+++ b/cvpr2025-decafnet_amd/csrc/dec_chain.h
@@ -11,11 +11,9 @@
   const float* ln_q_w; const float* ln_q_b;
   const float* dw;
   const float* qn_w; const float* qn_b;
-  const unsigned short* Wq;
-  const float* bq;
-  const unsigned short* KV;
-  const float* kmask;
-  const unsigned short* Wp;
+  const unsigned short* Mimg;
+  const unsigned short* Nimg;
+  const float* cmask;
   const float* bp;
   float* Q3;
   int64_t ldq;
@@ -24,6 +22,7 @@
   int B, T;
   int affine;
   int lk2;
+  int Lk;
   unsigned* status;
   int attn_single;
 };
@@ -34,8 +33,8 @@
 size_t chain1_image_halfs(int N, int K);
 int launch_split_chain1(const float* W, unsigned short* img, int N, int K, hipStream_t stream, unsigned* overflow = nullptr);
 
-size_t kv_image_halfs(int lk2);
-int launch_kv_image(const float* K, const float* V, const uint8_t* kvmask, int B, int Lk, int lk2, unsigned short* img, float* kmask,
-                    hipStream_t stream);
+size_t fold_image_halfs(int lk2, bool n);
+int launch_fold_image(const float* K, const float* V, const uint8_t* kvmask, const float* Wq, const float* bq, const float* Wp, int B, int Lk,
+                      int lk2, unsigned short* Mimg, unsigned short* Nimg, float* cmask, hipStream_t stream, unsigned* overflow = nullptr);
 
 }
diff --git a/cvpr2025-decafnet_amd/csrc/dec_chain.hip b/cvpr2025-decafnet_amd/csrc/dec_chain.hip
--- a/cvpr2025-decafnet_amd/csrc/dec_chain.hip
+++ b/cvpr2025-decafnet_amd/csrc/dec_chain.hip
@@ -14,7 +14,7 @@
 constexpr int DE = 256, DHEADS = 4, DHD = 64;
 constexpr int STAGE = 65536;
 constexpr int WGROWS = 128;
-constexpr int P_LNW = 0, P_LNB = 256, P_QNW = 512, P_QNB = 768, P_DW = 1024, P_BQ = 1792, P_BP = 2048, P_MS = 2560, P_END = 2624;
+constexpr int P_LNW = 0, P_LNB = 256, P_QNW = 512, P_QNB = 768, P_DW = 1024, P_MS = 1792, P_BP = 2048, P_END = 2560;
 constexpr int X_LAST = P_END;
 constexpr int X_FIRST = X_LAST + 5 * 256;
 constexpr int LDS_FLOATS = X_FIRST + 5 * 256;
@@ -41,36 +41,84 @@
   *reinterpret_cast<unsigned*>(img + o + 512) = lo;
 }
 
-__global__ void k_kv_image(const float* __restrict__ K, const float* __restrict__ V, const uint8_t* __restrict__ kvmask, int B, int Lk,
-                           int lk2, unsigned short* __restrict__ img, float* __restrict__ kmask) {
-  const int per_head = 16 * lk2 * 256;
-  const int i = blockIdx.x * blockDim.x + threadIdx.x;
-  if (i < B * 64) {
-    const int b = i / 64, key = i % 64;
-    kmask[i] = (key < Lk && kvmask[(size_t)b * Lk + key]) ? 0.f : -INFINITY;
-  }
-  if (i >= B * DHEADS * per_head) return;
-  const int b = i / (DHEADS * per_head), rem = i - b * (DHEADS * per_head);
-  const int hd = rem / per_head, rem2 = rem - hd * per_head;
-  const int piece = rem2 >> 8, lane = (rem2 >> 2) & 63, jp = rem2 & 3;
-  const int h = lane >> 5, r = lane & 31, plane = piece & 1, j = 2 * jp;
-  const float scale = 1.0f / sqrtf(sqrtf((float)DHD));
+__global__ __launch_bounds__(256) void k_fold_image(const float* __restrict__ K, const float* __restrict__ V, const uint8_t* __restrict__ kvmask,
+                                                    const float* __restrict__ Wq, const float* __restrict__ bq, const float* __restrict__ Wp,
+                                                    int B, int Lk, int lk2, unsigned short* __restrict__ Mimg, unsigned short* __restrict__ Nimg,
+                                                    float* __restrict__ cmask, unsigned* __restrict__ overflow) {
+  const int ppm = DHEADS * 16 * lk2, ppn = 8 * 16 * lk2;
+  const int units = ppm + ppn + 1;
+  const int b = (int)blockIdx.x / units, u = (int)blockIdx.x - b * units;
+  const int tid = threadIdx.x;
+  const float isd = 0.125f;
+  if (u == ppm + ppn) {
+    const int hd = tid >> 6, key = tid & 63;
+    float c = -INFINITY;
+    if (key < Lk && kvmask[(size_t)b * Lk + key]) {
+      const float* kr = K + ((size_t)b * Lk + key) * DE + DHD * hd;
+      float s = 0.f;
+      for (int ch = 0; ch < DHD; ch += 4) {
+        const f32x4 k4 = *reinterpret_cast<const f32x4*>(kr + ch);
+#pragma unroll
+        for (int e = 0; e < 4; ++e) s = __builtin_fmaf(k4[e], bq[DHD * hd + ch + e], s);
+      }
+      c = s * isd;
+    }
+    cmask[(size_t)b * 256 + tid] = c;
+    return;
+  }
+  __shared__ float sA[32][DHD + 1];
+  __shared__ float sB[DHD][16 + 1];
+  const bool ism = u < ppm;
+  const int un = u - ppm;
+  float scale = 1.f;
+  unsigned short* dst;
+  {
+    const int ar = tid >> 3, ac = (tid & 7) * 8;
+    const float* arow = nullptr;
+    if (ism) {
+      const int hd = u / (16 * lk2), kk = (u / lk2) % 16, kt = u % lk2;
+      const int key = 32 * kt + ar;
+      if (key < Lk) arow = K + ((size_t)b * Lk + key) * DE + DHD * hd + ac;
+      const int ch = tid >> 2, c4 = (tid & 3) * 4;
+      const f32x4 w4 = *reinterpret_cast<const f32x4*>(Wq + (size_t)(DHD * hd + ch) * DE + 16 * kk + c4);
+#pragma unroll
+      for (int e = 0; e < 4; ++e) sB[ch][c4 + e] = w4[e];
+      scale = isd;
+      dst = Mimg + ((size_t)b * ppm + u) * 1024;
+    } else {
+      const int jb = un / (16 * lk2), kk = (un >> 1) % (8 * lk2), t2 = un & 1;
+      const int hd = kk / (2 * lk2), ks = kk % (2 * lk2);
+      arow = Wp + (size_t)(64 * jb + 32 * t2 + ar) * DE + DHD * hd + ac;
+      const int kc = tid >> 4, ch4 = (tid & 15) * 4, key = 16 * ks + kc;
+      f32x4 v4 = f32x4{0.f, 0.f, 0.f, 0.f};
+      if (key < Lk) v4 = *reinterpret_cast<const f32x4*>(V + ((size_t)b * Lk + key) * DE + DHD * hd + ch4);
+#pragma unroll
+      for (int e = 0; e < 4; ++e) sB[ch4 + e][kc] = v4[e];
+      dst = Nimg + ((size_t)b * ppn + un) * 1024;
+    }
+    f32x4 a0 = f32x4{0.f, 0.f, 0.f, 0.f}, a1 = a0;
+    if (arow) { a0 = *reinterpret_cast<const f32x4*>(arow); a1 = *reinterpret_cast<const f32x4*>(arow + 4); }
+#pragma unroll
+    for (int e = 0; e < 4; ++e) { sA[ar][ac + e] = a0[e]; sA[ar][ac + 4 + e] = a1[e]; }
+  }
+  __syncthreads();
+  const int lane = tid >> 2, jp = tid & 3, h = lane >> 5, r = lane & 31, j = 2 * jp;
+  const int in16 = 8 * (j >> 2) + 4 * h + (j & 3);
   float v0 = 0.f, v1 = 0.f;
-  if (piece < 8 * lk2) {
-    const int ks = (piece >> 1) & 3, kt = piece >> 3;
-    const int key = 32 * kt + r, ch = DHD * hd + 16 * ks + 8 * (j >> 2) + 4 * h + (j & 3);
-    if (key < Lk) { v0 = K[((size_t)b * Lk + key) * DE + ch] * scale; v1 = K[((size_t)b * Lk + key) * DE + ch + 1] * scale; }
-  } else {
-    const int pv = piece - 8 * lk2;
-    const int q = (pv >> 1) & 1, kt = (pv >> 2) % lk2, ct = (pv >> 2) / lk2;
-    const int ch = DHD * hd + 32 * ct + r, key = 32 * kt + 16 * q + 8 * (j >> 2) + 4 * h + (j & 3);
-    if (key < Lk) v0 = V[((size_t)b * Lk + key) * DE + ch];
-    if (key + 1 < Lk) v1 = V[((size_t)b * Lk + key + 1) * DE + ch];
-  }
-  const f16x2 hh = __builtin_convertvector(f32x2{v0, v1}, f16x2);
-  const f16x2 ll = __builtin_convertvector(f32x2{v0 - (float)hh[0], v1 - (float)hh[1]}, f16x2);
-  const size_t o = (((size_t)b * DHEADS + hd) * 16 * lk2 + piece) * 512 + (size_t)lane * 8 + j;
-  *reinterpret_cast<unsigned*>(img + o) = __builtin_bit_cast(unsigned, plane == 0 ? hh : ll);
+#pragma unroll 8
+  for (int ch = 0; ch < DHD; ++ch) {
+    const float av = sA[r][ch];
+    v0 = __builtin_fmaf(av, sB[ch][in16], v0);
+    v1 = __builtin_fmaf(av, sB[ch][in16 + 1], v1);
+  }
+  v0 *= scale; v1 *= scale;
+  unsigned hi, lo;
+  split2_f16(v0, v1, SW, hi, lo);
+  if (!(__builtin_fabsf(v0) * SW <= 65504.f) || !(__builtin_fabsf(v1) * SW <= 65504.f)) {
+    if (overflow) atomicOr(overflow, 1u);
+  }
+  *reinterpret_cast<unsigned*>(dst + lane * 8 + j) = hi;
+  *reinterpret_cast<unsigned*>(dst + 512 + lane * 8 + j) = lo;
 }
 
 template <int LK2, bool SINGLE = false>
@@ -85,15 +133,18 @@
   const int t = t0 + w * 32 + r;
   const bool inseq = t < p.T;
   const int64_t row = (int64_t)b * p.T + (inseq ? t : p.T - 1);
-  constexpr int KVP = 16 * LK2;
-
-  const unsigned short* kv_b = p.KV + (size_t)b * DHEADS * KVP * 512;
+  constexpr int NP = 32 * LK2;
+  constexpr int KS2 = 2 * LK2;
+  constexpr int KSN = DHEADS * KS2;
+  const int Lk = p.Lk;
+  auto live = [&](int kk) __attribute__((always_inline)) { return 16 * (kk % KS2) < Lk; };
+
+  const unsigned short* m_b = p.Mimg + (size_t)b * DHEADS * NP * 512;
+  const unsigned short* n_b = p.Nimg + (size_t)b * 8 * NP * 512;
   auto issue_piece = [&](int s, int i) __attribute__((always_inline)) {
-    const bool kv = s < 8 && (s & 1);
-    const int np = kv ? KVP : 64;
-    int pc = w + 4 * i;
-    pc = pc < np ? pc : np - 1;
-    const unsigned short* src = s >= 8 ? p.Wp + (size_t)(s - 8) * 64 * 512 : (kv ? kv_b + (size_t)(s >> 1) * KVP * 512 : p.Wq + (size_t)(s >> 1) * 64 * 512);
+    if (s >= DHEADS && !live(i)) return;
+    const int pc = w + 4 * i;
+    const unsigned short* src = s >= DHEADS ? n_b + (size_t)(s - DHEADS) * NP * 512 : m_b + (size_t)s * NP * 512;
     glds16(src + (size_t)pc * 512, lane16, (unsigned)(s & 1) * STAGE + (unsigned)pc * 1024u);
   };
 #ifdef DCF_DC_STAMP
@@ -111,15 +162,14 @@
   f32x4 ev = f32x4{0.f, 0.f, 0.f, 0.f};
   if (evalid) ev = *reinterpret_cast<const f32x4*>(p.X + ((int64_t)b * p.T + te) * p.ldx + 4 * lane);
 #pragma unroll
-  for (int i = 0; i < 16; ++i) issue_piece(0, i);
+  for (int i = 0; i < 8 * LK2; ++i) issue_piece(0, i);
 
   {
     ldf[P_LNW + tid] = p.ln_q_w[tid]; ldf[P_LNB + tid] = p.ln_q_b[tid];
     ldf[P_QNW + tid] = p.qn_w[tid]; ldf[P_QNB + tid] = p.qn_b[tid];
     ldf[P_DW + tid] = p.dw[tid]; ldf[P_DW + 256 + tid] = p.dw[256 + tid]; ldf[P_DW + 512 + tid] = p.dw[512 + tid];
-    ldf[P_BQ + tid] = p.bq[tid];
+    ldf[P_MS + tid] = p.cmask[(size_t)b * 256 + tid];
     ldf[P_BP + tid] = p.bp[tid]; ldf[P_BP + 256 + tid] = p.bp[256 + tid];
-    if (tid < 64) ldf[P_MS + tid] = p.kmask[(size_t)b * 64 + tid];
   }
 
 
@@ -198,182 +248,111 @@
   }
 
   STAMP(3);
-  f16x8 cth[16], ctl[16];
-  const float qscale = 1.0f / sqrtf(sqrtf((float)DHD));
+  f16x8 ph[DHEADS][KS2], pl[DHEADS][KS2];
   auto stage_begin = [&](int s) __attribute__((always_inline)) {
     asm volatile("s_waitcnt vmcnt(0)" ::: "memory");
     STAMP(4);
     __syncthreads();
     STAMP(5);
   };
-  auto gemm2 = [&](const unsigned char* buf, const f16x8 (&bh)[16], const f16x8 (&bl)[16], f32x16 (&acc)[2], auto&& dma, auto&& side)
-                   __attribute__((always_inline)) {
-    f16x8 fr[2][4];
+  auto gemm_nt = [&](const unsigned char* buf, auto nt_, auto ks_, auto&& acc, auto&& on, auto&& bop, auto&& dma, auto&& side)
+                     __attribute__((always_inline)) {
+    constexpr int NT = decltype(nt_)::value, KS = decltype(ks_)::value;
+    f16x8 fr[2][NT][2];
     auto frags = [&](int kk, int set) __attribute__((always_inline)) {
-      fr[set][0] = *reinterpret_cast<const f16x8*>(buf + ((0 * 16 + kk) * 2) * 1024);
-      fr[set][1] = *reinterpret_cast<const f16x8*>(buf + ((0 * 16 + kk) * 2 + 1) * 1024);
-      fr[set][2] = *reinterpret_cast<const f16x8*>(buf + ((1 * 16 + kk) * 2) * 1024);
-      fr[set][3] = *reinterpret_cast<const f16x8*>(buf + ((1 * 16 + kk) * 2 + 1) * 1024);
+#pragma unroll
+      for (int t2 = 0; t2 < NT; ++t2) {
+        fr[set][t2][0] = *reinterpret_cast<const f16x8*>(buf + ((kk * NT + t2) * 2) * 1024);
+        fr[set][t2][1] = *reinterpret_cast<const f16x8*>(buf + ((kk * NT + t2) * 2 + 1) * 1024);
+      }
     };
     frags(0, 0);
 #pragma unroll
-    for (int kk = 0; kk < 16; ++kk) {
+    for (int kk = 0; kk < KS; ++kk) {
       const int set = kk & 1;
-      if (kk + 1 < 16) frags(kk + 1, set ^ 1);
-      acc[0] = mma(fr[set][1], bh[kk], acc[0]);
-      acc[1] = mma(fr[set][3], bh[kk], acc[1]);
+      const bool go = on(kk);
+      if (kk + 1 < KS) frags(kk + 1, set ^ 1);
+      if constexpr (!SINGLE) {
+        if (go) {
+#pragma unroll
+          for (int t2 = 0; t2 < NT; ++t2) acc(t2) = mma(fr[set][t2][1], bop(kk, 0), acc(t2));
+        }
+      }
       __builtin_amdgcn_sched_barrier(0);
       side(kk, 0);
       __builtin_amdgcn_sched_barrier(0);
-      acc[0] = mma(fr[set][0], bl[kk], acc[0]);
-      acc[1] = mma(fr[set][2], bl[kk], acc[1]);
+      if constexpr (!SINGLE) {
+        if (go) {
+#pragma unroll
+          for (int t2 = 0; t2 < NT; ++t2) acc(t2) = mma(fr[set][t2][0], bop(kk, 1), acc(t2));
+        }
+      }
       __builtin_amdgcn_sched_barrier(0);
       side(kk, 1);
       dma(kk);
       __builtin_amdgcn_sched_barrier(0);
-      acc[0] = mma(fr[set][0], bh[kk], acc[0]);
-      acc[1] = mma(fr[set][2], bh[kk], acc[1]);
+      if (go) {
+#pragma unroll
+        for (int t2 = 0; t2 < NT; ++t2) acc(t2) = mma(fr[set][t2][0], bop(kk, 0), acc(t2));
+      }
       __builtin_amdgcn_sched_barrier(0);
     }
   };
-  f32x16 O[2];
-  u32x4 cx_h, cx_l;
-  auto ctx_piece = [&](int hd, int u) __attribute__((always_inline)) {
-    const int ct = u >> 3, q = (u >> 2) & 1, i = u & 3;
-    unsigned hi, lo;
-    split2_f16(O[ct][8 * q + 2 * i], O[ct][8 * q + 2 * i + 1], SA, hi, lo);
-    cx_h[i] = hi; cx_l[i] = lo;
-    if (i == 3) {
-      cth[2 * (2 * hd + ct) + q] = __builtin_bit_cast(f16x8, cx_h);
-      ctl[2 * (2 * hd + ct) + q] = __builtin_bit_cast(f16x8, cx_l);
+  f32x16 S[2][LK2];
+  float sm_mx = 0.f, sm_sum = 0.f, sm_inv = 0.f;
+  auto sm_step = [&](int hd, int step) __attribute__((always_inline)) {
+    f32x16 (&Sh)[LK2] = S[hd & 1];
+    if (step < 2) {
+      if (step == 0) sm_mx = -INFINITY;
+      if (step < LK2) {
+        const int kt = step;
+#pragma unroll
+        for (int g = 0; g < 4; ++g) {
+          const f32x4 mk = *reinterpret_cast<const f32x4*>(ldf + P_MS + 64 * hd + 32 * kt + 8 * g + 4 * h);
+#pragma unroll
+          for (int e = 0; e < 4; ++e) {
+            Sh[kt][4 * g + e] = __builtin_fmaf(Sh[kt][4 * g + e], UNSCALE, mk[e]);
+            sm_mx = fmaxf(sm_mx, Sh[kt][4 * g + e]);
+          }
+        }
+      }
+    } else if (step == 2) {
+      sm_mx = xor32_max(sm_mx);
+      sm_sum = 0.f;
+    } else if (step < 11) {
+      const int u = step - 3;
+#pragma unroll
+      for (int kt = 0; kt < LK2; ++kt)
+#pragma unroll
+        for (int e = 2 * u; e < 2 * u + 2; ++e) { Sh[kt][e] = fast_exp(Sh[kt][e] - sm_mx); sm_sum += Sh[kt][e]; }
+    } else if (step == 11) {
+      sm_inv = 1.0f / xor32_sum(sm_sum);
+    } else {
+      const int ks = step - 12;
+      if (ks < KS2) {
+        const int kt = ks >> 1, q = ks & 1;
+        float v8[8];
+#pragma unroll
+        for (int e = 0; e < 8; ++e) v8[e] = Sh[kt][8 * q + e] * sm_inv;
+        split8(v8, SA, ph[hd][ks], pl[hd][ks]);
+      }
     }
   };
 #pragma unroll
   for (int hd = 0; hd < DHEADS; ++hd) {
-    f32x16 QA[2];
-    {
-      stage_begin(2 * hd);
-      const unsigned char* buf = lds + ((2 * hd) & 1) * STAGE + lane16;
-#pragma unroll
-      for (int t2 = 0; t2 < 2; ++t2)
-#pragma unroll
-        for (int e = 0; e < 16; ++e) QA[t2][e] = 0.f;
-      gemm2(buf, qh, ql, QA,
-            [&](int kk) __attribute__((always_inline)) {
-              if (kk < KVP / 4) issue_piece(2 * hd + 1, kk);
-            },
-            [&](int kk, int slot) __attribute__((always_inline)) { if (hd > 0 && slot == 0) ctx_piece(hd - 1, kk); });
-    }
+    stage_begin(hd);
+    const unsigned char* buf = lds + (hd & 1) * STAGE + lane16;
+#pragma unroll
+    for (int kt = 0; kt < LK2; ++kt)
+#pragma unroll
+      for (int e = 0; e < 16; ++e) S[hd & 1][kt][e] = 0.f;
+    gemm_nt(buf, std::integral_constant<int, LK2>{}, std::integral_constant<int, 16>{},
+            [&](int t2) __attribute__((always_inline)) -> f32x16& { return S[hd & 1][t2]; },
+            [&](int) __attribute__((always_inline)) { return true; },
+            [&](int kk, int plane) __attribute__((always_inline)) -> const f16x8& { return plane ? ql[kk] : qh[kk]; },
+            [&](int kk) __attribute__((always_inline)) { if (kk < 8 * LK2) issue_piece(hd + 1, kk); },
+            [&](int kk, int slot) __attribute__((always_inline)) { if (hd > 0 && slot == 0) sm_step(hd - 1, kk); });
     STAMP(6);
-    f16x8 sh_[4], sl_[4];
-#pragma unroll
-    for (int t2 = 0; t2 < 2; ++t2)
-#pragma unroll
-      for (int q = 0; q < 2; ++q) {
-        float v8[8];
-#pragma unroll
-        for (int u = 0; u < 2; ++u) {
-          const int g = 2 * q + u;
-          const f32x4 bq = *reinterpret_cast<const f32x4*>(ldf + P_BQ + DHD * hd + 32 * t2 + 8 * g + 4 * h);
-#pragma unroll
-          for (int e = 0; e < 4; ++e) v8[4 * u + e] = __builtin_fmaf(QA[t2][4 * g + e], UNSCALE, bq[e]) * qscale;
-        }
-        split8(v8, 1.f, sh_[2 * t2 + q], sl_[2 * t2 + q]);
-      }
-    STAMP(7);
-    {
-      stage_begin(2 * hd + 1);
-      const unsigned char* buf = lds + ((2 * hd + 1) & 1) * STAGE + lane16;
-      f32x16 S[LK2];
-#pragma unroll
-      for (int kt = 0; kt < LK2; ++kt)
-#pragma unroll
-        for (int e = 0; e < 16; ++e) S[kt][e] = 0.f;
-      f16x8 kf[2][LK2][2];
-      auto kfrags = [&](int ks, int set) __attribute__((always_inline)) {
-#pragma unroll
-        for (int kt = 0; kt < LK2; ++kt) {
-          kf[set][kt][0] = *reinterpret_cast<const f16x8*>(buf + ((kt * 4 + ks) * 2) * 1024);
-          kf[set][kt][1] = *reinterpret_cast<const f16x8*>(buf + ((kt * 4 + ks) * 2 + 1) * 1024);
-        }
-      };
-      kfrags(0, 0);
-#pragma unroll
-      for (int ks = 0; ks < 4; ++ks) {
-        const int set = ks & 1;
-        if (ks + 1 < 4) kfrags(ks + 1, set ^ 1);
-        issue_piece(2 * hd + 2, 2 * ks);
-        issue_piece(2 * hd + 2, 2 * ks + 1);
-        if constexpr (!SINGLE) {
-#pragma unroll
-          for (int kt = 0; kt < LK2; ++kt) S[kt] = mma(kf[set][kt][0], sl_[ks], S[kt]);
-#pragma unroll
-          for (int kt = 0; kt < LK2; ++kt) S[kt] = mma(kf[set][kt][1], sh_[ks], S[kt]);
-        }
-#pragma unroll
-        for (int kt = 0; kt < LK2; ++kt) S[kt] = mma(kf[set][kt][0], sh_[ks], S[kt]);
-        __builtin_amdgcn_sched_barrier(0);
-      }
-      STAMP(8);
-      f16x8 vf[2][2][2];
-      auto vfrags = [&](int st_, int set) __attribute__((always_inline)) {
-#pragma unroll
-        for (int ct = 0; ct < 2; ++ct) {
-          const int pc = 8 * LK2 + ((ct * LK2 + (st_ >> 1)) * 2 + (st_ & 1)) * 2;
-          vf[set][ct][0] = *reinterpret_cast<const f16x8*>(buf + pc * 1024);
-          vf[set][ct][1] = *reinterpret_cast<const f16x8*>(buf + (pc + 1) * 1024);
-        }
-      };
-      vfrags(0, 0);
-      float mx = -INFINITY;
-#pragma unroll
-      for (int kt = 0; kt < LK2; ++kt)
-#pragma unroll
-        for (int g = 0; g < 4; ++g) {
-          const f32x4 mk = *reinterpret_cast<const f32x4*>(ldf + P_MS + 32 * kt + 8 * g + 4 * h);
-#pragma unroll
-          for (int e = 0; e < 4; ++e) { S[kt][4 * g + e] += mk[e]; mx = fmaxf(mx, S[kt][4 * g + e]); }
-        }
-      mx = xor32_max(mx);
-      float sum = 0.f;
-#pragma unroll
-      for (int kt = 0; kt < LK2; ++kt)
-#pragma unroll
-        for (int e = 0; e < 16; ++e) { S[kt][e] = fast_exp(S[kt][e] - mx); sum += S[kt][e]; }
-      const float inv = 1.0f / xor32_sum(sum);
-      f16x8 ph[LK2][2], pl[LK2][2];
-#pragma unroll
-      for (int kt = 0; kt < LK2; ++kt)
-#pragma unroll
-        for (int q = 0; q < 2; ++q) {
-          float v8[8];
-#pragma unroll
-          for (int e = 0; e < 8; ++e) v8[e] = S[kt][8 * q + e] * inv;
-          split8(v8, 1.f, ph[kt][q], pl[kt][q]);
-        }
-      STAMP(9);
-#pragma unroll
-      for (int ct = 0; ct < 2; ++ct)
-#pragma unroll
-        for (int e = 0; e < 16; ++e) O[ct][e] = 0.f;
-#pragma unroll
-      for (int st_ = 0; st_ < 2 * LK2; ++st_) {
-        const int set = st_ & 1, kt = st_ >> 1, q = st_ & 1;
-        if (st_ + 1 < 2 * LK2) vfrags(st_ + 1, set ^ 1);
-#pragma unroll
-        for (int i = 0; i < 8 / (2 * LK2); ++i) issue_piece(2 * hd + 2, 8 + st_ * (8 / (2 * LK2)) + i);
-        if constexpr (!SINGLE) {
-#pragma unroll
-          for (int ct = 0; ct < 2; ++ct) O[ct] = mma(vf[set][ct][0], pl[kt][q], O[ct]);
-#pragma unroll
-          for (int ct = 0; ct < 2; ++ct) O[ct] = mma(vf[set][ct][1], ph[kt][q], O[ct]);
-        }
-#pragma unroll
-        for (int ct = 0; ct < 2; ++ct) O[ct] = mma(vf[set][ct][0], ph[kt][q], O[ct]);
-        __builtin_amdgcn_sched_barrier(0);
-      }
-      STAMP(10);
-    }
   }
 
   float ps = 0.f, pss = 0.f;
@@ -405,7 +384,7 @@
   };
 #pragma unroll
   for (int j = 0; j < 8; ++j) {
-    stage_begin(8 + j);
+    stage_begin(DHEADS + j);
     const unsigned char* buf = lds + (j & 1) * STAGE + lane16;
     if (j > 0) asm volatile("" : "+v"(xr[(j - 1) & 1][0]), "+v"(xr[(j - 1) & 1][1]), "+v"(xr[(j - 1) & 1][2]), "+v"(xr[(j - 1) & 1][3]));
     load_xr(j);
@@ -413,19 +392,22 @@
     for (int t2 = 0; t2 < 2; ++t2)
 #pragma unroll
       for (int e = 0; e < 16; ++e) A2[j & 1][t2][e] = 0.f;
-    if (j == 0) {
-      gemm2(buf, cth, ctl, A2[0],
-            [&](int kk) __attribute__((always_inline)) {
-              issue_piece(9, kk);
-            },
-            [&](int kk, int slot) __attribute__((always_inline)) { if (kk < 8) ctx_piece(DHEADS - 1, 2 * kk + slot); });
-    } else {
-      gemm2(buf, cth, ctl, A2[j & 1],
-            [&](int kk) __attribute__((always_inline)) {
-              if (j + 1 < 8) issue_piece(8 + j + 1, kk);
-            },
-            [&](int kk, int slot) __attribute__((always_inline)) { if ((kk & 3) == 0) epilogue(j - 1, kk >> 2, slot); });
-    }
+    gemm_nt(buf, std::integral_constant<int, 2>{}, std::integral_constant<int, KSN>{},
+            [&](int t2) __attribute__((always_inline)) -> f32x16& { return A2[j & 1][t2]; },
+            [&](int kk) __attribute__((always_inline)) { return live(kk); },
+            [&](int kk, int plane) __attribute__((always_inline)) -> const f16x8& { return plane ? pl[kk / KS2][kk % KS2] : ph[kk / KS2][kk % KS2]; },
+            [&](int kk) __attribute__((always_inline)) { if (j + 1 < 8) issue_piece(DHEADS + j + 1, kk); },
+            [&](int kk, int slot) __attribute__((always_inline)) {
+              if (j == 0) {
+                constexpr int PER = (16 + 6 * KS2 - 1) / (6 * KS2);
+                const int sl = 2 * kk + slot;
+#pragma unroll
+                for (int i = 0; i < PER; ++i)
+                  if (sl * PER + i < 16) sm_step(DHEADS - 1, sl * PER + i);
+              } else if (kk % KS2 == 0) {
+                epilogue(j - 1, kk / KS2, slot);
+              }
+            });
     STAMP(11);
   }
   asm volatile("s_waitcnt vmcnt(0)" ::: "memory");
@@ -444,7 +426,7 @@
   if (bad && p.status) {
     bool anykey = false;
 #pragma unroll
-    for (int k = 0; k < 64; ++k) anykey = anykey || ldf[P_MS + k] == 0.f;
+    for (int k = 0; k < 64; ++k) anykey = anykey || ldf[P_MS + k] > -INFINITY;
     if (anykey) atomicOr(p.status, 1u);
   }
 #ifdef DCF_DC_STAMP
@@ -474,23 +456,26 @@
   return 0;
 }
 
-size_t kv_image_halfs(int lk2) { return (size_t)DHEADS * 16 * lk2 * 512; }
-
-int launch_kv_image(const float* K, const float* V, const uint8_t* kvmask, int B, int Lk, int lk2, unsigned short* img, float* kmask,
-                    hipStream_t stream) {
-  DCF_CHECK(B > 0 && Lk >= 1 && Lk <= 32 * lk2 && (lk2 == 1 || lk2 == 2), "launch_kv_image: Lk = %d, lk2 = %d", Lk, lk2);
-  const int n = B * DHEADS * 16 * lk2 * 256;
-  hipLaunchKernelGGL(k_kv_image, dim3((n + 255) / 256), dim3(256), 0, stream, K, V, kvmask, B, Lk, lk2, img, kmask);
+size_t fold_image_halfs(int lk2, bool n) { return (size_t)(n ? 8 : DHEADS) * 32 * lk2 * 512; }
+
+int launch_fold_image(const float* K, const float* V, const uint8_t* kvmask, const float* Wq, const float* bq, const float* Wp, int B, int Lk,
+                      int lk2, unsigned short* Mimg, unsigned short* Nimg, float* cmask, hipStream_t stream, unsigned* overflow) {
+  DCF_CHECK(B > 0 && Lk >= 1 && Lk <= 32 * lk2 && (lk2 == 1 || lk2 == 2), "launch_fold_image: Lk = %d, lk2 = %d", Lk, lk2);
+  auto al16 = [](const void* q) { return (reinterpret_cast<uintptr_t>(q) & 15) == 0; };
+  DCF_CHECK(al16(K) && al16(V) && al16(Wq) && al16(Wp) && al16(Mimg) && al16(Nimg), "launch_fold_image: operands must be 16-byte aligned");
+  const int units = DHEADS * 16 * lk2 + 8 * 16 * lk2 + 1;
+  hipLaunchKernelGGL(k_fold_image, dim3((unsigned)(B * units)), dim3(256), 0, stream, K, V, kvmask, Wq, bq, Wp, B, Lk, lk2, Mimg, Nimg, cmask,
+                     overflow);
   DCF_HIP(hipGetLastError());
   return 0;
 }
 
 int launch_dec_chain(const DecChainArgs& a, hipStream_t stream) {
-  DCF_CHECK(a.B > 0 && a.T > 0 && a.X && a.mask && a.Wq && a.KV && a.kmask && a.Wp && a.Q3, "launch_dec_chain: null argument");
-  DCF_CHECK(a.lk2 == 1 || a.lk2 == 2, "launch_dec_chain: lk2 = %d", a.lk2);
+  DCF_CHECK(a.B > 0 && a.T > 0 && a.X && a.mask && a.Mimg && a.Nimg && a.cmask && a.Q3, "launch_dec_chain: null argument");
+  DCF_CHECK((a.lk2 == 1 || a.lk2 == 2) && a.Lk >= 1 && a.Lk <= 32 * a.lk2, "launch_dec_chain: lk2 = %d, Lk = %d", a.lk2, a.Lk);
   DCF_CHECK(!a.stats_out || (a.stats_w > 0 && DE % a.stats_w == 0), "launch_dec_chain: stats_out needs a slot width dividing %d", DE);
   auto al16 = [](const void* q) { return (reinterpret_cast<uintptr_t>(q) & 15) == 0; };
-  DCF_CHECK(al16(a.X) && al16(a.Q3) && al16(a.Wq) && al16(a.Wp) && al16(a.KV) && a.ldx % 4 == 0 && a.ldq % 4 == 0,
+  DCF_CHECK(al16(a.X) && al16(a.Q3) && al16(a.Mimg) && al16(a.Nimg) && a.ldx % 4 == 0 && a.ldq % 4 == 0,
             "launch_dec_chain: operands must be 16-byte aligned with row pitches that are multiples of 4");
   static bool attr_set[64] = {};
   int dev = 0;
diff --git a/cvpr2025-decafnet_amd/csrc/engine.hip b/cvpr2025-decafnet_amd/csrc/engine.hip
--- a/cvpr2025-decafnet_amd/csrc/engine.hip
+++ b/cvpr2025-decafnet_amd/csrc/engine.hip
@@ -160,7 +160,7 @@
   const float *wp_il, *bp_il;
   const float *ln_ffn_w, *ln_ffn_b, *fc_w, *fc_b, *pj_w, *pj_b, *ls_ffn;
   const float *fc_wf, *fc_s, *fc_c;
-  const unsigned short *wq_chain, *wp_chain;
+  bool chain;
 };
 struct TextEncW {
   const float *ln_attn_w, *ln_attn_b, *wq, *bq, *wk, *bk, *wv, *bv, *wp, *bp, *ls_attn;
@@ -422,17 +422,7 @@
     if (pack3(m, w.bp, 2, E / 32, 32, 1, 0, 2, st, &w.bp_il)) return -1;
     SPLIT(w.wp_il, 2 * E, E);
   }
-  w.wq_chain = w.wp_chain = nullptr;
-  if (m->gemm_terms == GEMM_F16X3 && w.wp_il && dec_chain_supports(E, m->cfg.fusion_heads, 1)) {
-    unsigned short *iq = nullptr, *ip = nullptr;
-    DCF_HIP(hipMalloc(&iq, chain1_image_halfs(E, E) * sizeof(unsigned short)));
-    m->owned.push_back(reinterpret_cast<float*>(iq));
-    DCF_HIP(hipMalloc(&ip, chain1_image_halfs(2 * E, E) * sizeof(unsigned short)));
-    m->owned.push_back(reinterpret_cast<float*>(ip));
-    if (launch_split_chain1(w.wq, iq, E, E, st, nullptr)) return -1;
-    if (launch_split_chain1(w.wp_il, ip, 2 * E, E, st, nullptr)) return -1;
-    w.wq_chain = iq; w.wp_chain = ip;
-  }
+  w.chain = m->gemm_terms == GEMM_F16X3 && w.wp_il && dec_chain_supports(E, m->cfg.fusion_heads, 1);
   return 0;
 }
 
@@ -699,7 +689,7 @@
   uint8_t *mask_pre, *nbr_pre;
   float* col5;
   float *X, *R[7], *H2, *HID, *F, *HA, *HB, *HC, *HD, *logits1, *tcnA, *tcnB, *kvn, *Kt, *Vt;
-  unsigned short* kvimg;
+  unsigned short *mimg, *nimg;
   float* kmadd;
   float* stats;
   float* hstats[2];
@@ -741,8 +731,9 @@
   b.kvn = a.take<float>((size_t)B * Lk * c.TE);
   b.Kt = a.take<float>((size_t)B * Lk * E);
   b.Vt = a.take<float>((size_t)B * Lk * E);
-  b.kvimg = a.take<unsigned short>((size_t)B * kv_image_halfs(2));
-  b.kmadd = a.take<float>((size_t)B * 64);
+  b.mimg = a.take<unsigned short>((size_t)B * fold_image_halfs(2, false));
+  b.nimg = a.take<unsigned short>((size_t)B * fold_image_halfs(2, true));
+  b.kmadd = a.take<float>((size_t)B * 256);
 }
 
 static int get_plan(dcf_model* m, int T0, int B, int L, hipStream_t st, Plan** out) {
@@ -1112,7 +1103,7 @@
 static bool can_chain_dec(dcf_model* m, const DecW& w, const LevelTable* lt, int rows, int64_t ldx, int Lk) {
   static const bool off = getenv("DCF_NO_DEC_CHAIN") != nullptr;
   const dcf_config& c = m->cfg;
-  return !off && !lt && m->gemm_terms == GEMM_F16X3 && w.wq_chain && w.wp_chain && dec_chain_supports(c.E, c.fusion_heads, Lk) &&
+  return !off && !lt && m->gemm_terms == GEMM_F16X3 && w.chain && dec_chain_supports(c.E, c.fusion_heads, Lk) &&
          c.TE % 32 == 0 && rows >= dec_chain_min_rows() && ldx % 4 == 0;
 }
 
@@ -1133,16 +1124,17 @@
     TRY(run_gemm(m, gkv, 2, A_ROWS, st));
     if (chain) {
       const int lk2 = Lk <= 32 ? 1 : 2;
-      TRY(launch_kv_image(b.Kt, b.Vt, b.kvmask, B, Lk, lk2, b.kvimg, b.kmadd, st));
+      TRY(launch_fold_image(b.Kt, b.Vt, b.kvmask, w.wq, w.bq, w.wp_il, B, Lk, lk2, b.mimg, b.nimg, b.kmadd, st, m->status));
       carry = !g_no_carry() && w.fc_wf && m->wsplit.count(w.fc_wf) &&
               (can_chain_ffn_rows(m, rows, E) || gemm_can_carry_stats(rows, 4 * E, E, 1, m->wsplit_terms[w.fc_wf]));
       DecChainArgs da{};
       da.X = X; da.ldx = ldx; da.mask = mask; da.ln_q_w = w.ln_q_w; da.ln_q_b = w.ln_q_b; da.dw = w.dw; da.qn_w = w.qn_w; da.qn_b = w.qn_b;
-      da.Wq = w.wq_chain; da.bq = w.bq; da.KV = b.kvimg; da.kmask = b.kmadd; da.Wp = w.wp_chain; da.bp = w.bp_il;
+      da.Mimg = b.mimg; da.Nimg = b.nimg; da.cmask = b.kmadd; da.bp = w.bp_il;
       da.Q3 = b.R[2]; da.ldq = E; da.stats_out = carry ? b.stats : nullptr; da.stats_w = STATS_W;
-      da.B = B; da.T = T; da.affine = c.xattn_affine; da.lk2 = lk2; da.status = m->status; da.attn_single = c.attn_mode == 1;
+      da.B = B; da.T = T; da.affine = c.xattn_affine; da.lk2 = lk2; da.Lk = Lk; da.status = m->status; da.attn_single = c.attn_mode == 1;
       {
-        ProfScope prof("gemm_f16x3<dec_chain>", st, 2.0 * rows * E * 3.0 * E + 4.0 * rows * E * Lk, (double)rows * E * 4.0 * 2.0);
+        ProfScope prof("gemm_f16x3<dec_chain>", st, 2.0 * rows * c.fusion_heads * (32.0 * lk2 * E + 2.0 * E * 16.0 * ((Lk + 15) / 16)),
+                       (double)rows * E * 4.0 * 2.0);
         TRY(launch_dec_chain(da, st));
       }
       if (!carry) {
@@ -2675,6 +2667,12 @@
   return dcf::launch_xattn(a, (hipStream_t)stream);
 }
 
+int dcf_op_dec_fold_image(const float* K, const float* V, const uint8_t* kvmask, const float* Wq, const float* bq, const float* Wp,
+                          int32_t B, int32_t Lk, uint16_t* Mimg, uint16_t* Nimg, float* cmask, uint32_t* status, void* stream) {
+  DCF_CHECK(K && V && kvmask && Wq && bq && Wp && Mimg && Nimg && cmask && B >= 1 && Lk >= 1 && Lk <= 64, "dcf_op_dec_fold_image: bad arguments");
+  return dcf::launch_fold_image(K, V, kvmask, Wq, bq, Wp, B, Lk, Lk <= 32 ? 1 : 2, Mimg, Nimg, cmask, (hipStream_t)stream, status);
+}
+
 int dcf_op_local_attn(const float* Q, const float* K, const float* V, const uint8_t* mask, float* O, int32_t B, int32_t T,
                       int32_t C, int32_t heads, int32_t window, void* stream) {
   if (window == 0) {
diff --git a/include/decafnet_hip.h b/include/decafnet_hip.h
--- a/include/decafnet_hip.h
+++ b/include/decafnet_hip.h
@@ -180,6 +180,8 @@
                      void* stream);
 int dcf_op_xattn(const float* Q, const float* K, const float* V, const uint8_t* kvmask, float* O, int32_t B, int32_t T,
                  int32_t Lk, int32_t C, int32_t heads, void* stream);
+int dcf_op_dec_fold_image(const float* K, const float* V, const uint8_t* kvmask, const float* Wq, const float* bq, const float* Wp,
+                          int32_t B, int32_t Lk, uint16_t* Mimg, uint16_t* Nimg, float* cmask, uint32_t* status, void* stream);
 int dcf_op_local_attn(const float* Q, const float* K, const float* V, const uint8_t* mask, float* O, int32_t B, int32_t T,
                       int32_t C, int32_t heads, int32_t window, void* stream);
 int dcf_op_sidekick(const float* shallow, const float* text_cls, float* correl, int32_t D, int32_t T, int32_t nq,
```

New measurement: 21.84 million clips/s, median of 6. Within noise of the previous version (+0.9%).
